# JanBeh/radiorust

Measured on NVIDIA B200. Metric: complex MS/s via FreqShift->Filter->Downsampler, higher is better.
Workload: dtype f32

## Files before the change

radiorust_b200/csrc/rr_chain.cu:

```cuda
#include <cuda_runtime.h>

#include <atomic>
#include <cmath>
#include <complex>
#include <algorithm>
#include <cstdio>
#include <cstdlib>
#include <cstring>
#include <deque>
#include <memory>
#include <mutex>
#include <numeric>
#include <string>
#include <unordered_map>
#include <vector>

#include "../../include/radiorust_b200.h"
#include "rr_design.h"
#include "rr_kernels.h"

namespace {

thread_local std::string g_err;
std::atomic<uint64_t> g_launches{0};

int fail(int code, const std::string& msg) {
    g_err = msg;
    return code;
}
int fail_cuda(cudaError_t e, const char* what) {
    g_err = std::string(what) + ": " + cudaGetErrorString(e);
    return RR_ERR_CUDA;
}
#define RR_CUDA(expr)                                     \
    do {                                                  \
        cudaError_t e__ = (expr);                         \
        if (e__ != cudaSuccess) return fail_cuda(e__, #expr); \
    } while (0)
#define RR_TRY(expr)              \
    do {                          \
        int r__ = (expr);         \
        if (r__ != RR_OK) return r__; \
    } while (0)
#define RR_LAUNCH(n_kernels, expr)                        \
    do {                                                  \
        cudaError_t e__ = (expr);                         \
        if (e__ != cudaSuccess) return fail_cuda(e__, #expr); \
        g_launches.fetch_add((n_kernels));                \
    } while (0)

struct DevBuf {
    void* p = nullptr;
    size_t bytes = 0;
    int ensure(size_t need, bool zero = false, cudaStream_t st = nullptr) {
        if (need <= bytes && p) {
            return RR_OK;
        }
        if (p) cudaFree(p);
        p = nullptr;
        bytes = 0;
        if (need == 0) need = 16;
        cudaError_t e = cudaMalloc(&p, need);
        if (e != cudaSuccess) {
            p = nullptr;
            g_err = std::string("cudaMalloc: ") + cudaGetErrorString(e);
            return e == cudaErrorMemoryAllocation ? RR_ERR_NOMEM : RR_ERR_CUDA;
        }
        bytes = need;
        if (zero) {
            e = cudaMemsetAsync(p, 0, need, st);
            if (e != cudaSuccess) return fail_cuda(e, "cudaMemsetAsync");
        }
        return RR_OK;
    }
    void release() {
        if (p) cudaFree(p);
        p = nullptr;
        bytes = 0;
    }
};

struct Shape {
    size_t chunk_len = 0, n_chunks = 0;
    double rate = 0.0;
    size_t len() const { return chunk_len * n_chunks; }
};

struct View {
    const void* p = nullptr;
    long long stride = 0;
    Shape sh;
};

struct NcoHost {
    int64_t numer = 0, denom = 1;
    uint64_t idx = 0;
    double start_phase = 0.0;
    bool has_table = false;
};

struct StageHost {
    double f_sr = NAN;
    size_t f_n = 0;
    int f_seg = 0;
    bool f_dirty = true;
    double r_in_rate = NAN;
    bool r_valid = false;
    int r_L = 0;
    long long P = 1, Q = 1, j0 = 0, m0 = 0;
    size_t r_pending = 0;
    bool r_indexed = false;
    double r_pos = 0.0;
    bool fm_has_prev = false;
    double n_sr = NAN;
    size_t rc_pending = 0;
    double rc_rate = NAN;
    size_t ov_hist = 0, ov_len = 0;
    double ov_rate = NAN;
};

struct StageAct {
    bool active = false;
    bool redesign = false;
    bool first_is_history = false;
    size_t n_new = 0;
    size_t pending_before = 0;
    long long j0 = 0, m0 = 0;
    double pos0 = 0.0;
    bool nco_recalc = false;
    int seg_before = 0;
    bool lost = false;
    Shape out;
};

inline long long floordiv128(long long a, long long b, long long c) { return (long long)(((__int128)a * b) / c); }
inline long long ceildiv128(long long a, long long b, long long c) { return (long long)(((__int128)a * b + (c - 1)) / c); }

bool integer_valued(double x) { return std::isfinite(x) && x >= 0.0 && x < 9.0e15 && std::floor(x) == x; }

}

struct rr_ctx {
    int device = 0;
    int sm_count = 0;
};


struct rr_pool {
    rr_ctx* ctx = nullptr;
    std::mutex mu;
    struct Buf {
        void* p;
        size_t cap;
    };
    std::deque<Buf> idle;
    std::unordered_map<void*, size_t> live;
    uint64_t n_alloc = 0, n_reuse = 0;
};

namespace {

struct Stage {
    rr_stage_desc d{};
    StageHost h;
    std::vector<double> shift;
    std::vector<uint8_t> shift_dirty;
    bool any_shift_dirty = true;
    std::vector<NcoHost> nco_h;
    std::vector<rr::NcoStream> nco_stage;
    DevBuf nco_d;
    DevBuf hperm, tw;
    DevBuf hist2[2];
    int hist_cur = 0;
    long long hist_fused_jlo = -1, hist_fused_jfirst = 0;
    DevBuf ztmp;
    size_t f_np = 0;
    DevBuf stg_in, stg_out, zero_chunk;
    DevBuf idx_a, idx_b;
    std::vector<std::complex<double>> taps;
    bool taps_valid = false;
    DevBuf big_h, big_twA, big_twB, big_twC, big_scratch;
    DevBuf ir, tail[2], obuf[2];
    int tail_cur = 0, obuf_cur = 0;
    std::vector<double> ir_host_flt;
    bool ztail_stale = false;
    DevBuf gtab, twK;
    bool poly_valid = false, poly_tried = false;
    int poly_K = 0, poly_G = 0, poly_Lmax = 0, poly_V = 0;
    DevBuf gtab2, twK2;
    bool poly2_tw_own = false;
    DevBuf acoef, gtab3, ubuf[2];
    long long ubuf_stride[2] = {-1, -1};
    int ubuf_cur = 0;
    bool ucache_valid = false;
    long long ucache_rows = 0;
    const void* ucache_ptr = nullptr;
    long long ucache_stride = 0;
    DevBuf ukeep[2];
    int ukeep_cur = 0;
    int fused_slot = -1;
    bool fused_valid = false;
    bool front_valid = false;
    int front_rank = 0;
    double front_discarded = 0.0;
    bool frontq_valid = false;
    bool frontq_wide = false;
    int frontq_cols = 0;
    int frontq_rank = 0;
    double frontq_discarded = 0.0;
    DevBuf acoef_q, gtab_q;
    bool poly2_valid = false;
    int poly2_G = 0, poly2_V = 0;
    size_t obuf_cap = 0;
    std::vector<double> ir_host;
    DevBuf fm_prev, fm_last;
    DevBuf fm_phase;
    size_t tail_cap = 0;
    DevBuf fwin, ftw;
    size_t fwin_n = 0;
    DevBuf out;
    size_t out_cap = 0;
};

}

struct rr_chain {
    rr_ctx* ctx = nullptr;
    int dtype = RR_C32;
    size_t esz = 8;
    int S = 1;
    std::vector<Stage> st;
    cudaStream_t stream = nullptr;
    cudaStream_t h2d_stream = nullptr, d2h_stream = nullptr;
    DevBuf stage_in[2], stage_out[2];
    cudaEvent_t ev_h2d[2] = {nullptr, nullptr}, ev_comp[2] = {nullptr, nullptr}, ev_d2h[2] = {nullptr, nullptr};
    cudaEvent_t ev_copy = nullptr;
    int slot = 0;
    std::string plan;
    uint64_t samples_lost = 0;
    bool push_mutated = false;
    bool allow_poly = true;
    bool allow_poly2 = true;
    size_t big_os_scratch_bytes = (size_t)2 << 30;
    bool allow_sab = true;
    bool allow_ucache = true;
    bool allow_front = true;
    bool allow_fused = true;
    int fused_min_streams = -1;
    long long fused_min_rows = 1;
    bool timing = false;
    std::vector<cudaEvent_t> evs;
    size_t ev_used = 0;
    std::vector<std::string> ev_names;
    std::string timed_kernel, breakdown;
    int timing_begin() {
        if (!timing) return 0;
        if (ev_used + 2 > evs.size()) {
            cudaEvent_t a = nullptr, b = nullptr;
            if (cudaEventCreate(&a) != cudaSuccess || cudaEventCreate(&b) != cudaSuccess) return 0;
            evs.push_back(a);
            evs.push_back(b);
        }
        cudaEventRecord(evs[ev_used], stream);
        return 1;
    }
    void timing_end(const char* name) {
        cudaEventRecord(evs[ev_used + 1], stream);
        ev_used += 2;
        if (ev_names.size() < ev_used / 2) ev_names.resize(ev_used / 2);
        ev_names[ev_used / 2 - 1] = name;
    }
};

namespace {
void chain_restart(rr_chain* c);
}

#define RR_TIMED_LAUNCH(c, name, n_kernels, expr)                        \
    do {                                                                 \
        const int t__ = (c)->timing_begin();                             \
        RR_LAUNCH(n_kernels, expr);                                      \
        if (t__) (c)->timing_end(name);                                  \
    } while (0)

namespace {

int advance_stage(const rr_stage_desc& d, StageHost& h, const Shape& in, StageAct* act) {
    StageAct a;
    a.out = in;
    if (in.n_chunks == 0 || in.chunk_len == 0) {
        a.out.n_chunks = 0;
        *act = a;
        return RR_OK;
    }
    a.active = true;
    switch (d.kind) {
        case RR_STAGE_FREQSHIFT:
            a.nco_recalc = !(h.n_sr == in.rate);
            h.n_sr = in.rate;
            break;
        case RR_STAGE_GAIN:
        case RR_STAGE_FOURIER:
        case RR_STAGE_FMMOD:
            break;
        case RR_STAGE_RECHUNK: {
            if (h.rc_pending > 0 && !(h.rc_rate == in.rate)) {
                h.rc_pending = 0;
                a.lost = true;
            }
            h.rc_rate = in.rate;
            const size_t ocl = (size_t)d.output_chunk_len;
            a.pending_before = h.rc_pending;
            a.n_new = in.len();
            const size_t total = h.rc_pending + a.n_new;
            a.out.chunk_len = ocl;
            a.out.n_chunks = total / ocl;
            h.rc_pending = total - a.out.n_chunks * ocl;
            break;
        }
        case RR_STAGE_OVERLAP: {
            const size_t k = (size_t)d.chunk_count;
            if (h.ov_hist > 0 && (h.ov_len != in.chunk_len || !(h.ov_rate == in.rate)))
                return fail(RR_ERR_UNSUPPORTED, "Overlapper: the chunks of one history must share length and sample rate");
            a.pending_before = h.ov_hist;
            const size_t tot = h.ov_hist + in.n_chunks;
            a.out.chunk_len = k * in.chunk_len;
            a.out.n_chunks = tot >= k ? tot - (k - 1) : 0;
            double acc = 0.0;
            for (size_t i = 0; i < k; ++i) acc += in.rate * (double)in.chunk_len;
            a.out.rate = acc / (double)(k * in.chunk_len);
            h.ov_hist = std::min(k - 1, tot);
            h.ov_len = in.chunk_len;
            h.ov_rate = in.rate;
            break;
        }
        case RR_STAGE_FMDEMOD:
            a.first_is_history = !h.fm_has_prev;
            h.fm_has_prev = true;
            break;
        case RR_STAGE_FILTER: {
            a.redesign = h.f_dirty || !(h.f_sr == in.rate) || h.f_n != in.chunk_len;
            if (a.redesign) {
                h.f_dirty = false;
                h.f_sr = in.rate;
                h.f_n = in.chunk_len;
                h.f_seg = 0;
            }
            a.seg_before = h.f_seg;
            a.first_is_history = (h.f_seg == 0);
            a.out.n_chunks = in.n_chunks - (a.first_is_history ? 1 : 0);
            h.f_seg = (int)std::min<size_t>(2, (size_t)h.f_seg + in.n_chunks);
            break;
        }
        case RR_STAGE_DOWNSAMPLE:
        case RR_STAGE_UPSAMPLE: {
            const bool down = d.kind == RR_STAGE_DOWNSAMPLE;
            if (!h.r_valid || !(h.r_in_rate == in.rate)) {
                const double in_rate = in.rate, out_rate = d.output_rate;
                if (!(in_rate >= 0.0)) return fail(RR_ERR_INVALID, "input sample rate must be positive");
                if (down && !(in_rate >= out_rate))
                    return fail(RR_ERR_INVALID, "input sample rate must be greater than or equal to output sample rate");
                if (!down && !(in_rate <= out_rate))
                    return fail(RR_ERR_INVALID, "input sample rate must be smaller than or equal to output sample rate");
                if (!down && !(d.bandwidth < in_rate))
                    return fail(RR_ERR_INVALID, "bandwidth must be smaller than input sample rate");
                const double margin = down ? (out_rate - d.bandwidth) / 2.0 : (in_rate - d.bandwidth) / 2.0;
                const double lf = std::ceil((down ? in_rate : out_rate) / margin * d.quality);
                if (!(lf > 0.0) || lf > 1.0e8) return fail(RR_ERR_INVALID, "resampler impulse response length out of range");
                if (in_rate == 0.0 || out_rate == 0.0) return fail(RR_ERR_INVALID, "resampler sample rates must be non-zero");
                h.r_indexed = !integer_valued(in_rate) || !integer_valued(out_rate);
                h.r_pos = 0.0;
                if (!h.r_indexed) {
                    long long Pn = (long long)in_rate, Qn = (long long)out_rate;
                    const long long g = std::gcd(Pn, Qn);
                    h.P = Pn / g;
                    h.Q = Qn / g;
                } else {
                    h.P = h.Q = 1;
                }
                h.j0 = 0;
                h.m0 = 0;
                h.r_L = (int)lf;
                h.r_in_rate = in_rate;
                h.r_valid = true;
                a.redesign = true;
            }
            const long long len = (long long)in.len();
            a.j0 = h.j0;
            a.m0 = h.m0;
            a.pos0 = h.r_pos;
            if (h.r_indexed) {
                const double in_rate = in.rate, out_rate = d.output_rate;
                double pos = h.r_pos;
                size_t cnt = 0;
                if (down) {
                    for (long long j = 0; j < len; ++j) {
                        pos += out_rate;
                        if (pos >= in_rate) {
                            pos -= in_rate;
                            ++cnt;
                        }
                    }
                } else {
                    for (long long p = 0; p < len; ++p) {
                        while (pos < out_rate) {
                            ++cnt;
                            pos += in_rate;
                        }
                        pos -= out_rate;
                    }
                }
                h.r_pos = pos;
                a.n_new = cnt;
            } else {
                long long total_after;
                if (down) total_after = floordiv128(h.j0 + len, h.Q, h.P);
                else total_after = ceildiv128(h.j0 + len, h.Q, h.P);
                a.n_new = (size_t)(total_after - h.m0);
                const long long j1 = (h.j0 + len) % h.P;
                h.j0 = j1;
                h.m0 = down ? floordiv128(j1, h.Q, h.P) : ceildiv128(j1, h.Q, h.P);
            }
            a.pending_before = h.r_pending;
            const size_t ocl = d.output_chunk_len ? (size_t)d.output_chunk_len : 1;
            const size_t total = h.r_pending + a.n_new;
            a.out.chunk_len = ocl;
            a.out.n_chunks = total / ocl;
            a.out.rate = d.output_rate;
            h.r_pending = total - a.out.n_chunks * ocl;
            break;
        }
        default:
            return fail(RR_ERR_INVALID, "unknown stage kind");
    }
    *act = a;
    return RR_OK;
}

int stage_event(const rr_stage_desc& d, StageHost& h, bool* interrupt) {
    int lost = 0;
    switch (d.kind) {
        case RR_STAGE_RECHUNK:
            if (h.rc_pending > 0) {
                h.rc_pending = 0;
                lost = 1;
                *interrupt = true;
            }
            break;
        case RR_STAGE_OVERLAP:
            h.ov_hist = 0;
            lost = 1;
            *interrupt = true;
            break;
        case RR_STAGE_FILTER:
            if (*interrupt) h.f_seg = 0;
            break;
        case RR_STAGE_FMDEMOD:
            if (*interrupt) h.fm_has_prev = false;
            break;
        default:
            break;
    }
    return lost;
}

inline size_t filter_padded_len(size_t n) {
    size_t np = 32;
    while (np < n) np <<= 1;
    return np;
}
template <typename T> bool filter_len_supported(size_t n) {
    if (n < 1 || n > ((size_t)1 << 23)) return false;
    const size_t np = filter_padded_len(n);
    return rr::chain_os_supported<T>((int)np, 0, 0) || rr::big_os_supported<T>((int)np);
}
inline bool is_pow2(size_t n) { return n >= 2 && (n & (n - 1)) == 0; }

int stage_supported(const rr_chain* c, const rr_stage_desc& d, const Shape& in) {
    if (in.n_chunks == 0 || in.chunk_len == 0) return RR_OK;
    const bool f32 = c->dtype == RR_C32;
    if (d.kind == RR_STAGE_FILTER) {
        const size_t n = in.chunk_len;
        if (!(f32 ? filter_len_supported<float>(n) : filter_len_supported<double>(n)))
            return fail(RR_ERR_UNSUPPORTED, "Filter: chunk length not supported by the device path");
    } else if (d.kind == RR_STAGE_FOURIER) {
        const int n = (int)std::min<size_t>(in.chunk_len, (size_t)1 << 30);
        const bool fft = f32 ? rr::fourier_fft_supported<float>(n) : rr::fourier_fft_supported<double>(n);
        if (!fft && in.chunk_len > (size_t)rr::kFourierDirectMax)
            return fail(RR_ERR_UNSUPPORTED, "Fourier: chunk lengths outside the FFT plans are limited to 4096 samples");
    }
    return RR_OK;
}

int dry_shape(const rr_chain* c, const Shape& in, Shape* out) {
    std::vector<StageHost> hs;
    hs.reserve(c->st.size());
    for (const auto& s : c->st) hs.push_back(s.h);
    Shape sh = in;
    for (size_t i = 0; i < hs.size(); ++i) {
        StageAct a;
        RR_TRY(stage_supported(c, c->st[i].d, sh));
        RR_TRY(advance_stage(c->st[i].d, hs[i], sh, &a));
        if (a.lost) {
            bool intr = true;
            for (size_t j = i + 1; j < hs.size(); ++j) stage_event(c->st[j].d, hs[j], &intr);
        }
        sh = a.out;
    }
    *out = sh;
    return RR_OK;
}

template <typename T> struct TypeTag { using type = T; };
#define RR_DISPATCH(chain, T, ...)                     \
    do {                                               \
        if ((chain)->dtype == RR_C32) {                \
            using T = float;                           \
            __VA_ARGS__;                               \
        } else {                                       \
            using T = double;                          \
            __VA_ARGS__;                               \
        }                                              \
    } while (0)

rr::WindowFn make_window(int kind, double beta, rr_window_fn fn, void* user) {
    switch (kind) {
        case RR_WINDOW_RECTANGULAR:
            return [](double) { return 1.0; };
        case RR_WINDOW_CUSTOM:
            return [fn, user](double x) { return fn ? fn(user, x) : 1.0; };
        default:
            return [beta](double x) { return rr::kaiser_rel_with_beta(beta, x); };
    }
}

template <typename T> int upload_complex(DevBuf& buf, const std::vector<std::complex<double>>& v, cudaStream_t st) {
    RR_TRY(buf.ensure(v.size() * 2 * sizeof(T)));
    std::vector<T> tmp(v.size() * 2);
    for (size_t i = 0; i < v.size(); ++i) {
        tmp[2 * i] = (T)v[i].real();
        tmp[2 * i + 1] = (T)v[i].imag();
    }
    RR_CUDA(cudaMemcpyAsync(buf.p, tmp.data(), tmp.size() * sizeof(T), cudaMemcpyHostToDevice, st));
    RR_CUDA(cudaStreamSynchronize(st));
    return RR_OK;
}
template <typename T> int upload_real(DevBuf& buf, const std::vector<double>& v, cudaStream_t st) {
    RR_TRY(buf.ensure(v.size() * sizeof(T)));
    std::vector<T> tmp(v.size());
    for (size_t i = 0; i < v.size(); ++i) tmp[i] = (T)v[i];
    RR_CUDA(cudaMemcpyAsync(buf.p, tmp.data(), tmp.size() * sizeof(T), cudaMemcpyHostToDevice, st));
    RR_CUDA(cudaStreamSynchronize(st));
// ... 421 lines not shown
    const size_t tab_bytes = (size_t)(Q * P) * (size_t)bestK * 2 * sizeof(T);
    if (tab_bytes > ((size_t)512 << 20)) return RR_OK;
    const double e8 = (double)P / (8.0 * (double)((P + 7) / 8)), e10 = (double)P / (10.0 * (double)((P + 9) / 10));
    int G = e10 > e8 + 1e-9 ? 10 : 8;
    if (const char* e = std::getenv("RR_POLY_G")) G = std::atoi(e) == 8 ? 8 : 10;
    if (!rr::poly_supported<T>(bestK, (int)Q, G)) return RR_OK;
    if (rr::poly_smem_bytes<T>(bestK, (int)Q, G, 1) > (size_t)220 * 1024) return RR_OK;
    std::vector<std::complex<double>> tab, perm;
    const int lm = rr::design_poly_tables(f.taps, ds.ir_host_flt, P, Q, bestK, &tab);
    if (lm != (int)Lmax) return fail(RR_ERR_INVALID, "internal: polyphase reach mismatch");
    const double scale = 2.0 * (double)n / (double)bestK;
    const long long NR = (P + G - 1) / G;
    perm.assign((size_t)(Q * NR) * (size_t)bestK * (size_t)G, std::complex<double>(0.0, 0.0));
    for (long long q = 0; q < Q; ++q)
        for (long long p = 0; p < P; ++p) {
            const long long r = p / G, gg = p % G;
            for (int k = 0; k < bestK; ++k) {
                const size_t pos = (size_t)rr::poly_hperm_index<T>(bestK, k);
                perm[(((size_t)(q * NR + r)) * bestK + pos) * G + gg] = tab[(size_t)(q * P + p) * bestK + k] * scale;
            }
        }
    RR_TRY(upload_complex<T>(ds.gtab, perm, c->stream));
    std::vector<std::complex<double>> tw;
    rr::make_twiddles((size_t)bestK, &tw);
    RR_TRY(upload_complex<T>(ds.twK, tw, c->stream));
    ds.poly_K = bestK;
    ds.poly_G = G;
    ds.poly_Lmax = (int)Lmax;
    ds.poly_V = (int)(bestK - 1 - Lmax);
    ds.poly_valid = true;

    if (std::is_same<T, float>::value && Q > 1 && c->allow_front && P > 2 * kFrontQRank && rr::poly_supported<T>(bestK, (int)Q, 8) &&
        Lmax + 2 <= bestK) {
        constexpr int RMAX = 2 * kFrontQRank;
        std::vector<double> acf;
        std::vector<std::complex<double>> bq;
        int rank = 0;
        double disc = 0.0;
        const int lmq = rr::design_rank_tables_q(f.taps, ds.ir_host_flt, P, Q, bestK, 2.0e-8, RMAX, &rank, &acf, &bq, &disc);
        const int cols = rank <= kFrontQRank ? kFrontQRank : RMAX;
        const bool narrow = cols == kFrontQRank && rr::front_supported(kFrontQRank, P);
        if (rank > 0 && lmq == (int)Lmax && (narrow || rr::front_wide_supported(cols, P))) {
            std::vector<float> ac((size_t)P * cols);
            for (long long p = 0; p < P; ++p)
                for (int cc = 0; cc < cols; ++cc) ac[(size_t)p * cols + cc] = (float)acf[(size_t)p * RMAX + cc];
            RR_TRY(ds.acoef_q.ensure(ac.size() * sizeof(float)));
            RR_CUDA(cudaMemcpyAsync(ds.acoef_q.p, ac.data(), ac.size() * sizeof(float), cudaMemcpyHostToDevice, c->stream));
            RR_CUDA(cudaStreamSynchronize(c->stream));
            constexpr int GQ = 8;
            const long long NRq = cols / GQ;
            perm.assign((size_t)(Q * NRq) * (size_t)bestK * (size_t)GQ, std::complex<double>(0.0, 0.0));
            for (long long q = 0; q < Q; ++q)
                for (int cc = 0; cc < cols; ++cc) {
                    const long long r = cc / GQ, gg = cc % GQ;
                    for (int k = 0; k < bestK; ++k) {
                        const size_t pos = (size_t)rr::poly_hperm_index<T>(bestK, k);
                        perm[(((size_t)(q * NRq + r)) * bestK + pos) * GQ + gg] = bq[((size_t)q * RMAX + cc) * bestK + k] * scale;
                    }
                }
            RR_TRY(upload_complex<T>(ds.gtab_q, perm, c->stream));
            ds.frontq_rank = rank;
            ds.frontq_cols = cols;
            ds.frontq_wide = !narrow;
            ds.frontq_discarded = disc;
            ds.frontq_valid = true;
        }
    }

    if (std::is_same<T, float>::value && c->allow_poly2 && rr::poly2_supported(512, P, Q) && 511 - Lmax >= 128) {
        const int K2 = 512, G2 = rr::poly2_pick_G(P);
        if (bestK != K2) rr::design_poly_tables(f.taps, ds.ir_host_flt, P, Q, K2, &tab);
        const double scale2 = 2.0 * (double)n / (double)K2;
        const long long NR2 = (P + G2 - 1) / G2;
        perm.assign((size_t)NR2 * (size_t)K2 * (size_t)G2, std::complex<double>(0.0, 0.0));
        for (long long p = 0; p < P; ++p)
            for (int k = 0; k < K2; ++k)
                perm[(size_t)rr::poly2_table_index(G2, (int)(p / G2), (int)(p % G2), k)] = tab[(size_t)p * K2 + k] * scale2;
        RR_TRY(upload_complex<T>(ds.gtab2, perm, c->stream));
        if (bestK != K2) {
            rr::make_twiddles((size_t)K2, &tw);
            RR_TRY(upload_complex<T>(ds.twK2, tw, c->stream));
        }
        ds.poly2_tw_own = bestK != K2;
        ds.poly2_G = G2;
        ds.poly2_V = (int)(K2 - 1 - Lmax);
        ds.poly2_valid = true;

        constexpr int RK = 10;
        if (c->allow_front && rr::front_supported(RK, P) && rr::poly2_supported(K2, RK, 1)) {
            std::vector<double> acf;
            std::vector<std::complex<double>> bfft;
            int rank = 0;
            double disc = 0.0;
            const int lm2 = rr::design_rank_tables(f.taps, ds.ir_host_flt, P, K2, 2.0e-8, RK, &rank, &acf, &bfft, &disc);
            if (rank > 0 && lm2 == (int)Lmax) {
                std::vector<float> ac((size_t)P * RK);
                for (long long p = 0; p < P; ++p)
                    for (int cc = 0; cc < RK; ++cc) ac[(size_t)(((p / 2) * 2 + (p & 1)) * RK + cc)] = (float)acf[(size_t)p * RK + cc];
                RR_TRY(ds.acoef.ensure(ac.size() * sizeof(float)));
                RR_CUDA(cudaMemcpyAsync(ds.acoef.p, ac.data(), ac.size() * sizeof(float), cudaMemcpyHostToDevice, c->stream));
                RR_CUDA(cudaStreamSynchronize(c->stream));
                perm.assign((size_t)K2 * (size_t)RK, std::complex<double>(0.0, 0.0));
                for (int cc = 0; cc < RK; ++cc)
                    for (int k = 0; k < K2; ++k) perm[(size_t)rr::poly2_table_index(RK, 0, cc, k)] = bfft[(size_t)cc * K2 + k] * scale2;
                RR_TRY(upload_complex<T>(ds.gtab3, perm, c->stream));
                ds.front_rank = rank;
                ds.front_discarded = disc;
                ds.front_valid = true;
                if (c->allow_fused && rr::fused_supported(RK, P, (int)Lmax)) {
                    const int slot = fused_slot_acquire(c->ctx->device, &ds);
                    if (slot >= 0) {
                        RR_CUDA(rr::fused_upload_coef(slot, ac.data(), (int)P, c->stream));
                        RR_CUDA(cudaStreamSynchronize(c->stream));
                        ds.fused_slot = slot;
                        ds.fused_valid = true;
                    }
                }
            }
        }
    }
    return RR_OK;
}

template <typename T>
int downsample_indexed(rr_chain* c, Stage& ds, const StageAct& a, const void* in, long long in_stride, long long len, void* out,
                       long long out_stride) {
    const double in_rate = ds.h.r_in_rate, out_rate = ds.d.output_rate;
    std::vector<int> fire;
    fire.reserve(a.n_new);
    double pos = a.pos0;
    for (long long j = 0; j < len; ++j) {
        pos += out_rate;
        if (pos >= in_rate) {
            pos -= in_rate;
            fire.push_back((int)j);
        }
    }
    if (fire.size() != a.n_new) return fail(RR_ERR_INVALID, "internal: indexed downsampler count mismatch");
    RR_TRY(ds.idx_a.ensure(std::max<size_t>(fire.size(), 1) * sizeof(int)));
    if (!fire.empty()) RR_CUDA(cudaMemcpyAsync(ds.idx_a.p, fire.data(), fire.size() * sizeof(int), cudaMemcpyHostToDevice, c->stream));
    RR_CUDA(cudaStreamSynchronize(c->stream));
    RR_LAUNCH(2, rr::launch_downsample_indexed<T>(in, in_stride, len, ds.tail[ds.tail_cur].p, ds.tail[ds.tail_cur ^ 1].p, (const T*)ds.ir.p,
                                                  ds.h.r_L, (const int*)ds.idx_a.p, (long long)fire.size(), out, out_stride, c->S, c->stream));
    ds.tail_cur ^= 1;
    return RR_OK;
}
template <typename T>
int upsample_indexed(rr_chain* c, Stage& us, const StageAct& a, const void* in, long long in_stride, long long len, void* out,
                     long long out_stride) {
    const double in_rate = us.h.r_in_rate, out_rate = us.d.output_rate;
    const int L = us.h.r_L;
    std::vector<int> qpos((size_t)len);
    double pos = a.pos0;
    long long q = 0;
    for (long long p = 0; p < len; ++p) {
        qpos[(size_t)p] = (int)q;
        while (pos < out_rate) {
            ++q;
            pos += in_rate;
        }
        pos -= out_rate;
    }
    if ((size_t)q != a.n_new) return fail(RR_ERR_INVALID, "internal: indexed upsampler count mismatch");
    std::vector<int> cnt((size_t)q + (size_t)L);
    {
        size_t p = 0;
        for (size_t i = 0; i < cnt.size(); ++i) {
            while (p < qpos.size() && (size_t)qpos[p] <= i) ++p;
            cnt[i] = (int)p;
        }
    }
    RR_TRY(us.idx_a.ensure(std::max<size_t>(qpos.size(), 1) * sizeof(int)));
    RR_TRY(us.idx_b.ensure(std::max<size_t>(cnt.size(), 1) * sizeof(int)));
    if (!qpos.empty()) RR_CUDA(cudaMemcpyAsync(us.idx_a.p, qpos.data(), qpos.size() * sizeof(int), cudaMemcpyHostToDevice, c->stream));
    if (!cnt.empty()) RR_CUDA(cudaMemcpyAsync(us.idx_b.p, cnt.data(), cnt.size() * sizeof(int), cudaMemcpyHostToDevice, c->stream));
    RR_CUDA(cudaStreamSynchronize(c->stream));
    RR_LAUNCH(1, rr::launch_upsample_indexed<T>(in, in_stride, len, us.tail[us.tail_cur].p, us.tail[us.tail_cur ^ 1].p, (const T*)us.ir.p, L,
                                                (const int*)us.idx_a.p, (const int*)us.idx_b.p, q, out, out_stride, c->S, c->stream));
    us.tail_cur ^= 1;
    return RR_OK;
}

struct DirectOut {
    void* user_out = nullptr;
    long long user_stride = 0;
    bool done = false;
};
template <typename T>
int run_filter_down(rr_chain* c, Stage& f, Stage& ds, const FilterIo& io, const StageAct& fa, const StageAct& da, std::string* plan,
                    DirectOut* direct = nullptr) {
    const size_t n = io.n;
    const int S = c->S;
    cudaStream_t st = c->stream;
    const int L = ds.h.r_L;
    void* obase = (char*)ds.obuf[ds.obuf_cur].p + da.pending_before * 2 * sizeof(T);
    const long long ostride = (long long)ds.obuf_cap;

    const bool rational = !ds.h.r_indexed && is_pow2(n);
    if (c->allow_poly && rational) RR_TRY(poly_prepare<T>(c, f, ds));
    const bool was_ucache_valid = ds.ucache_valid;
    ds.ucache_valid = false;
    size_t ca = io.n_chunks;
    if (c->allow_poly && rational && ds.poly_valid) {
        const size_t need = (size_t)(2 - std::min(2, fa.seg_before));
        ca = std::min(need, io.n_chunks);
    }
    const size_t fih = fa.first_is_history ? 1 : 0;

    long long j0 = da.j0, m0 = da.m0;
    if (ca > fih) {
        const long long zlen = (long long)((ca - fih) * n);
        if (ds.h.r_indexed) {
            RR_TRY(f.ztmp.ensure((size_t)S * (size_t)zlen * 2 * sizeof(T)));
            RR_TRY(run_os<T>(c, f, io, ca, fih != 0, f.ztmp.p, zlen));
            RR_TRY(downsample_indexed<T>(c, ds, da, f.ztmp.p, zlen, zlen, obase, ostride));
            *plan += "os|downsample(indexed)";
            return RR_OK;
        }
        const long long tot = floordiv128(j0 + zlen, ds.h.Q, ds.h.P);
        const long long n_out = tot - m0;
        if (rational && rr::chain_os_supported<T>((int)n, 1, L)) {
            rr::ChainOsArgs<T> a{};
            a.in = io.in;
            a.in_stride = io.in_stride;
            a.n_chunks = (int)ca;
            a.first_is_history = (int)fih;
            a.emit = 1;
            a.hist_in = (const char*)f.hist2[f.hist_cur].p + n * 2 * sizeof(T);
            a.hist_stride = (long long)(2 * n);
            a.hist_out = nullptr;
            a.hperm = f.hperm.p;
            a.twN = f.tw.p;
            a.nco = io.nco ? (const rr::NcoStream*)io.nco->nco_d.p : nullptr;
            a.nco_offset = 0;
            a.out = obase;
            a.out_stride = ostride;
            a.ir = (const T*)ds.ir.p;
            a.L = L;
            a.ztail_in = ds.tail[ds.tail_cur].p;
            a.ztail_out = ds.tail[ds.tail_cur ^ 1].p;
            a.rate.P = ds.h.P;
            a.rate.Q = ds.h.Q;
            a.rate.j0 = j0;
            a.rate.m0 = m0;
            RR_TIMED_LAUNCH(c, "k_chain_os<epi=down>", 1, rr::launch_chain_os<T>((int)n, 1, S, 1, a, st));
            ds.tail_cur ^= 1;
            *plan += "fused_os[filter+down]";
        } else {
            RR_TRY(f.ztmp.ensure((size_t)S * (size_t)zlen * 2 * sizeof(T)));
            RR_TRY(run_os<T>(c, f, io, ca, fih != 0, f.ztmp.p, zlen));
            rr::RateState rs;
            rs.P = ds.h.P;
            rs.Q = ds.h.Q;
            rs.j0 = j0;
            rs.m0 = m0;
            RR_LAUNCH(2, rr::launch_downsample<T>(f.ztmp.p, zlen, zlen, ds.tail[ds.tail_cur].p, ds.tail[ds.tail_cur ^ 1].p, (const T*)ds.ir.p,
                                                  L, rs, n_out, obase, ostride, S, st));
            ds.tail_cur ^= 1;
            *plan += !is_pow2(n) ? "padded_os[filter]|downsample" : (rr::chain_os_supported<T>((int)n, 0, 0) ? "fused_os[filter]|downsample" : "big_os|downsample");
        }
        obase = (char*)obase + (size_t)n_out * 2 * sizeof(T);
        j0 = (j0 + zlen) % ds.h.P;
        m0 = floordiv128(j0, ds.h.Q, ds.h.P);
    }

    if (ca < io.n_chunks) {
        const long long Pq = ds.h.P, Qq = ds.h.Q;
        const long long zlen = (long long)((io.n_chunks - ca) * n);
        const long long m_lo = m0 + 1;
        const long long m_hi = floordiv128(j0 + zlen, Qq, Pq);
        bool used_poly2 = false, used_front = false, used_fused = false, used_frontq = false;
        if (m_hi >= m_lo) {
            rr::PolyArgs<T> a{};
            a.in = io.in;
            a.in_stride = io.in_stride;
            a.len = (long long)(io.n_chunks * n);
            a.n = (long long)n;
            a.nco = io.nco ? (const rr::NcoStream*)io.nco->nco_d.p : nullptr;
            a.gtab = ds.gtab.p;
            a.twK = ds.twK.p;
            a.P = Pq;
            a.Q = Qq;
            a.Lmax = ds.poly_Lmax;
            a.V = ds.poly_V;
            a.J0 = j0 - (long long)(ca * n);
            a.m0 = m0;
            a.m_lo = m_lo;
            a.m_hi = m_hi;
            a.I_lo = m_lo / Qq;
            const long long I_hi = m_hi / Qq;
            bool done = false;
            if constexpr (std::is_same<T, float>::value) {
                const bool tma_ok = ((uintptr_t)a.in % 16 == 0) && (S == 1 || a.in_stride % 2 == 0) && a.len < (1LL << 31);
                if (ds.poly2_valid && ds.front_valid && ds.fused_valid && c->allow_fused && tma_ok && ca == 0 && was_ucache_valid &&
                    c->allow_ucache && ds.ucache_ptr && Qq == 1 && m0 == 0 && a.J0 >= 0 && a.J0 < Pq && S >= c->fused_min_streams &&
                    m_hi - m_lo + 1 >= c->fused_min_rows && a.len >= 33 * Pq) {
                    constexpr int RK = 10;
                    const long long n_out = m_hi - m_lo + 1;
                    const long long Lh = ds.poly_Lmax;
                    const size_t kbytes = (size_t)S * (size_t)Lh * RK * 2 * sizeof(float);
                    DevBuf& kb = ds.ukeep[ds.ukeep_cur];
                    RR_TRY(kb.ensure(kbytes));
                    rr::FusedArgs fu{};
                    fu.in = a.in;
                    fu.in_stride = a.in_stride;
                    fu.len = a.len;
                    fu.hist2 = f.hist2[f.hist_cur].p;
                    fu.n = a.n;
                    fu.nco = a.nco;
                    fu.P = (int)Pq;
                    fu.coef_slot = ds.fused_slot;
                    fu.J0 = a.J0;
                    fu.n_out = (int)n_out;
                    fu.Lmax = (int)Lh;
                    fu.V = ds.poly2_V;
                    fu.ukeep_in = ds.ucache_ptr;
                    fu.ukeep_in_stride = ds.ucache_stride;
                    fu.ukeep_out = kb.p;
                    fu.ukeep_out_stride = Lh * RK;
                    fu.gtab = ds.gtab3.p;
                    fu.twK = ds.poly2_tw_own ? ds.twK2.p : ds.twK.p;
                    fu.out = obase;
                    fu.out_stride = ostride;
                    const long long emit = (long long)da.out.len();
                    if (direct && direct->user_out && emit >= (long long)da.pending_before && emit > 0) {
                        fu.out = (char*)direct->user_out + da.pending_before * 2 * sizeof(T);
                        fu.out_stride = direct->user_stride;
                        fu.out2 = ds.obuf[ds.obuf_cur ^ 1].p;
                        fu.out2_stride = ostride;
                        fu.out_split = emit - (long long)da.pending_before;
                        direct->done = true;
                    }
                    const long long cover_hi = m_hi * Pq - a.J0;
                    f.hist_fused_jlo = -1;
                    f.hist_fused_jfirst = 0;
                    const long long hfrom = a.len - 2 * a.n, hstart = std::max<long long>(hfrom, 0);
                    if (cover_hi > hstart) {
                        fu.hist_out = f.hist2[f.hist_cur ^ 1].p;
                        fu.hist_from = hfrom;
                        fu.hist_stride = 2 * a.n;
                        f.hist_fused_jlo = cover_hi - hfrom;
                        f.hist_fused_jfirst = hstart - hfrom;
                    }
                    RR_TIMED_LAUNCH(c, "k_fused", 1, rr::launch_fused(S, fu, c->ctx->sm_count, st));
                    ds.ucache_valid = true;
                    ds.ucache_rows = n_out + Lh;
                    ds.ucache_ptr = kb.p;
                    ds.ucache_stride = Lh * RK;
                    ds.ukeep_cur ^= 1;
                    done = true;
                    used_fused = true;
                }
                if (!done && ds.poly2_valid && ds.front_valid && tma_ok) {
                    constexpr int RK = 10;
                    const int G2 = RK;
                    const long long n_out = m_hi - m_lo + 1;
                    const long long n_rows = n_out + ds.poly_Lmax;
                    const long long pad_rows = 512;
                    const long long u_stride = (((n_rows + 127) / 128 * 128 + pad_rows) * RK + 1) / 2 * 2;
                    if (n_rows < (1LL << 27)) {
                        const int n_blocks1 = (int)((n_out - 1) / ds.poly2_V + 1);
                        const int halves_total = 2 * c->ctx->sm_count;
                        const int sab_run = (c->allow_sab && n_blocks1 <= 3 && S > halves_total) ? (S + halves_total - 1) / halves_total : 0;
                        const int sab_nb = sab_run * n_blocks1;
                        const size_t S_alloc = sab_run ? (size_t)((S + sab_run - 1) / sab_run) * sab_run : (size_t)S;
                        const size_t ubytes = S_alloc * (size_t)u_stride * 2 * sizeof(float);
                        DevBuf& ub = ds.ubuf[ds.ubuf_cur];
                        if (ub.bytes < ubytes || ds.ubuf_stride[ds.ubuf_cur] != u_stride) {
                            RR_TRY(ub.ensure(ubytes));
                            RR_CUDA(cudaMemsetAsync(ub.p, 0, ubytes, st));
                            ds.ubuf_stride[ds.ubuf_cur] = u_stride;
                        }
                        const long long Lh = ds.poly_Lmax;
                        const bool cached = was_ucache_valid && c->allow_ucache && ca == 0 && ds.ucache_rows >= Lh && n_out > 0;
                        rr::FrontArgs fa{};
                        if (cached) {
                            fa.kept_src = ds.ucache_ptr;
                            fa.kept_stride = ds.ucache_stride;
                            fa.kept_rows = (int)Lh;
                        }
                        fa.in = a.in;
                        fa.in_stride = a.in_stride;
                        fa.len = a.len;
                        fa.hist2 = f.hist2[f.hist_cur].p;
                        fa.n = a.n;
                        fa.nco = a.nco;
                        fa.acoef = (const float*)ds.acoef.p;
                        fa.P = (int)Pq;
                        fa.J0 = a.J0;
                        fa.row_first = m_lo - 1 - (cached ? 0 : Lh);
                        fa.n_rows = (int)(cached ? n_out : n_rows);
                        fa.u = (char*)ub.p + (cached ? (size_t)Lh * RK * 2 * sizeof(float) : 0);
                        fa.u_stride = u_stride;
                        const long long cover_lo = fa.row_first * Pq - a.J0, cover_hi = m_hi * Pq - a.J0;
                        f.hist_fused_jlo = -1;
                        f.hist_fused_jfirst = 0;
                        const long long hfrom = a.len - 2 * a.n, hstart = std::max<long long>(hfrom, 0);
                        if (cover_lo <= hstart && cover_hi > hstart) {
                            fa.hist_out = f.hist2[f.hist_cur ^ 1].p;
                            fa.hist_from = hfrom;
                            fa.hist_stride = 2 * a.n;
                            fa.hist_staged = a.len < 4 * a.n ? 1 : 0;
                            f.hist_fused_jlo = cover_hi - hfrom;
                            f.hist_fused_jfirst = hstart - hfrom;
                        }
                        RR_TIMED_LAUNCH(c, "k_front", 1, rr::launch_front(RK, S, fa, st));
                        rr::PolyArgs<float> b{};
                        b.in = ub.p;
                        b.in_stride = u_stride;
                        b.len = (n_rows + pad_rows) * RK;
                        b.hist2 = ub.p;
                        b.n = 0;
                        b.nco = nullptr;
                        b.gtab = ds.gtab3.p;
                        b.twK = ds.poly2_tw_own ? ds.twK2.p : ds.twK.p;
                        b.P = RK;
                        b.Q = 1;
                        b.Lmax = ds.poly_Lmax;
                        b.V = ds.poly2_V;
                        b.J0 = 0;
                        b.m0 = ds.poly_Lmax;
                        b.m_lo = ds.poly_Lmax + 1;
                        b.m_hi = ds.poly_Lmax + n_out;
                        b.I_lo = b.m_lo;
                        b.n_blocks = (int)((b.m_hi - b.I_lo) / b.V + 1);
                        int nbpc = std::min(G2, b.n_blocks);
                        while (nbpc > 1 && rr::poly2_smem_bytes(G2, nbpc) > (size_t)226 * 1024) --nbpc;
                        const long long ctas_y = (S + 1) / 2;
                        while (nbpc > 1 && ctas_y * ((b.n_blocks + nbpc - 1) / nbpc) < 2LL * c->ctx->sm_count) --nbpc;
                        const int ngroups = (b.n_blocks + nbpc - 1) / nbpc;
                        nbpc = (b.n_blocks + ngroups - 1) / ngroups;
                        int ngrp = ngroups;
                        while (ngrp > 1 && ctas_y * ((ngroups + ngrp - 1) / ngrp) < 2LL * c->ctx->sm_count) --ngrp;
                        b.nbpc = nbpc;
                        b.ngrp = ngrp;
                        b.out = obase;
                        b.out_stride = ostride;
                        int S2 = S;
                        if (sab_nb) {
                            int nb2 = std::min(G2, sab_nb);
                            while (nb2 > 1 && rr::poly2_smem_bytes(G2, nb2) > (size_t)226 * 1024) --nb2;
                            const int groups2 = (sab_nb + nb2 - 1) / nb2;
                            b.n_blocks = sab_nb;
                            b.nbpc = (sab_nb + groups2 - 1) / groups2;
                            b.ngrp = groups2;
                            b.sab_blocks = sab_nb;
                            b.sab_rb = n_blocks1;
                            b.sab_streams = S;
                            b.sab_in_step = u_stride;
                            b.in_stride = (long long)sab_run * u_stride;
                            b.len = (long long)sab_run * u_stride;
                            S2 = (S + sab_run - 1) / sab_run;
                        }
                        const long long emit = (long long)da.out.len();
                        if (direct && direct->user_out && ca == 0 && emit >= (long long)da.pending_before && emit > 0) {
                            b.out = (char*)direct->user_out + da.pending_before * 2 * sizeof(T);
                            b.out_stride = direct->user_stride;
                            b.out2 = ds.obuf[ds.obuf_cur ^ 1].p;
                            b.out2_stride = ostride;
                            b.out_split = emit - (long long)da.pending_before;
                            direct->done = true;
                        }
                        if (sab_nb) {
                            b.sab_out_step = b.out_stride;
                            b.sab_out2_step = b.out2_stride;
                            b.out_stride *= sab_run;
                            b.out2_stride *= sab_run;
                        }
                        RR_TIMED_LAUNCH(c, "k_poly2", 1, rr::launch_poly2(G2, S2, b, st));
                        ds.ucache_valid = true;
                        ds.ucache_rows = n_rows;
                        ds.ucache_ptr = (const char*)ub.p + (size_t)(n_rows - Lh) * RK * 2 * sizeof(float);
                        ds.ucache_stride = u_stride;
                        ds.ubuf_cur ^= 1;
                        done = true;
                        used_front = true;
                    }
                }
                if (!done && ds.frontq_valid && (tma_ok || ds.frontq_wide) && Qq > 1) {
                    const int RQ = ds.frontq_cols;
                    constexpr int GQ = 8;
                    const long long Lh = ds.poly_Lmax;
                    const long long I_first = a.I_lo, I_last = I_hi;
                    const long long row_first = I_first - 1 - Lh;
                    const long long n_rows = I_last - I_first + 2 + Lh;
                    const long long u_stride = n_rows * RQ;
                    if (n_rows * Pq < (1LL << 31)) {
                        DevBuf& ub = ds.ubuf[0];
                        RR_TRY(ub.ensure((size_t)S * (size_t)u_stride * 2 * sizeof(float)));
                        ds.ubuf_stride[0] = -1;
                        rr::FrontArgs fa{};
                        fa.in = a.in;
                        fa.in_stride = a.in_stride;
                        fa.len = a.len;
                        fa.hist2 = f.hist2[f.hist_cur].p;
                        fa.n = a.n;
                        fa.nco = a.nco;
                        fa.acoef = (const float*)ds.acoef_q.p;
                        fa.P = (int)Pq;
                        fa.J0 = a.J0;
                        fa.row_first = row_first;
                        fa.n_rows = (int)n_rows;
                        fa.u = ub.p;
                        fa.u_stride = u_stride;
                        const long long cover_lo = row_first * Pq - a.J0, cover_hi = std::min<long long>((I_last + 1) * Pq - a.J0, a.len);
                        f.hist_fused_jlo = -1;
                        f.hist_fused_jfirst = 0;
                        const long long hfrom = a.len - 2 * a.n, hstart = std::max<long long>(hfrom, 0);
                        if (cover_lo <= hstart && cover_hi > hstart) {
                            fa.hist_out = f.hist2[f.hist_cur ^ 1].p;
                            fa.hist_from = hfrom;
                            fa.hist_stride = 2 * a.n;
                            fa.hist_staged = a.len < 4 * a.n ? 1 : 0;
                            f.hist_fused_jlo = cover_hi - hfrom;
                            f.hist_fused_jfirst = hstart - hfrom;
                        }
                        if (ds.frontq_wide) RR_TIMED_LAUNCH(c, "k_front_wide", 1, rr::launch_front_wide(RQ, S, fa, st));
                        else RR_TIMED_LAUNCH(c, "k_front", 1, rr::launch_front(RQ, S, fa, st));
                        rr::PolyArgs<float> b{};
                        b.in = ub.p;
                        b.in_stride = u_stride;
                        b.len = n_rows * RQ;
                        b.hist2 = ub.p;
                        b.n = 0;
                        b.nco = nullptr;
                        b.gtab = ds.gtab_q.p;
                        b.twK = ds.twK.p;
                        b.P = RQ;
                        b.Q = Qq;
                        b.Lmax = (int)Lh;
                        b.V = ds.poly_V;
                        b.J0 = row_first * RQ;
                        b.m0 = a.m0;
                        b.m_lo = a.m_lo;
                        b.m_hi = a.m_hi;
                        b.I_lo = I_first;
                        b.n_blocks = (int)((I_last - I_first) / b.V + 1);
                        int nbpc = b.n_blocks;
                        while (nbpc > 1 && rr::poly_smem_bytes<float>(ds.poly_K, (int)Qq, GQ, nbpc) > (size_t)200 * 1024) --nbpc;
                        while (nbpc > 1 && (long long)S * ((b.n_blocks + nbpc - 1) / nbpc) < 2LL * c->ctx->sm_count) --nbpc;
                        const int nsb = (b.n_blocks + nbpc - 1) / nbpc;
                        b.nbpc = (b.n_blocks + nsb - 1) / nsb;
                        b.out = obase;
                        b.out_stride = ostride;
                        RR_TIMED_LAUNCH(c, "k_poly(u)", 1, rr::launch_poly<float>(ds.poly_K, (int)Qq, GQ, S, b, st));
                        done = true;
                        used_frontq = true;
                    }
                }
                if (!done && ds.poly2_valid && tma_ok) {
                    a.gtab = ds.gtab2.p;
                    if (ds.poly2_tw_own) a.twK = ds.twK2.p;
                    a.V = ds.poly2_V;
                    a.n_blocks = (int)((I_hi - a.I_lo) / a.V + 1);
                    const int G2 = ds.poly2_G;
                    int nbpc = std::min(G2, a.n_blocks);
                    while (nbpc > 1 && rr::poly2_smem_bytes(G2, nbpc) > (size_t)226 * 1024) --nbpc;
                    const long long ctas_y = (S + 1) / 2;
                    while (nbpc > 1 && ctas_y * ((a.n_blocks + nbpc - 1) / nbpc) < 2LL * c->ctx->sm_count) --nbpc;
                    const int ngroups = (a.n_blocks + nbpc - 1) / nbpc;
                    nbpc = (a.n_blocks + ngroups - 1) / ngroups;
                    int ngrp = ngroups;
                    while (ngrp > 1 && ctas_y * ((ngroups + ngrp - 1) / ngrp) < 2LL * c->ctx->sm_count) --ngrp;
                    a.nbpc = nbpc;
                    a.ngrp = ngrp;
                    a.out = obase;
                    a.out_stride = ostride;
                    a.hist2 = f.hist2[f.hist_cur].p;
                    RR_TIMED_LAUNCH(c, "k_poly2", 1, rr::launch_poly2(G2, S, a, st));
                    done = true;
                    used_poly2 = true;
                }
            }
            if (!done) {
                a.n_blocks = (int)((I_hi - a.I_lo) / a.V + 1);
                int nbpc = std::max(1, ds.poly_G / (int)Qq);
                while (nbpc > 1 && rr::poly_smem_bytes<T>(ds.poly_K, (int)Qq, ds.poly_G, nbpc) > (size_t)200 * 1024) --nbpc;
                while (nbpc > 1 && (long long)S * ((a.n_blocks + nbpc - 1) / nbpc) < 2LL * c->ctx->sm_count) --nbpc;
                const int nsb = (a.n_blocks + nbpc - 1) / nbpc;
                nbpc = (a.n_blocks + nsb - 1) / nsb;
                a.nbpc = nbpc;
                a.out = obase;
                a.out_stride = ostride;
                a.hist2 = f.hist2[f.hist_cur].p;
                RR_TIMED_LAUNCH(c, "k_poly", 1, rr::launch_poly<T>(ds.poly_K, (int)Qq, ds.poly_G, S, a, st));
            }
        }
        ds.ztail_stale = true;
        if (!plan->empty() && plan->back() != '+' && plan->back() != '|' && ca > 0) *plan += "|";
        *plan += used_frontq ? "front+poly[filter+down]" : used_fused ? "fused[filter+down]" : (used_front ? "front+poly2[filter+down]" : (used_poly2 ? "poly2[filter+down]" : "poly[filter+down]"));
    }
    return RR_OK;
}

template <typename T>
int run_push(rr_chain* c, double sample_rate, size_t chunk_len, size_t n_chunks, const void* dev_in, size_t in_stride, void* dev_out,
             size_t out_capacity, size_t out_stride, size_t* out_count, double* out_rate) {
    const int S = c->S;
    const int ns = (int)c->st.size();
    cudaStream_t st = c->stream;
    Shape in;
    in.chunk_len = chunk_len;
    in.n_chunks = n_chunks;
    in.rate = sample_rate;
    if (chunk_len * n_chunks > in_stride && S > 1) return fail(RR_ERR_INVALID, "in_stride smaller than the pushed samples");

    {
        Shape sh;
        RR_TRY(dry_shape(c, in, &sh));
        if (sh.len() > out_capacity) return fail(RR_ERR_CAPACITY, "output buffer too small for this push");
        if (sh.len() > out_stride && S > 1) return fail(RR_ERR_INVALID, "out_stride smaller than the produced samples");
    }

    c->push_mutated = true;
    std::string plan;
    View cur;
    cur.p = dev_in;
    cur.stride = (long long)in_stride;
    cur.sh = in;
    Stage* pending_nco = nullptr;

    for (int i = 0; i < ns; ++i) {
        Stage& s = c->st[i];
        const bool last = (i == ns - 1);
        if (s.d.kind == RR_STAGE_FILTER && !last && c->st[i + 1].d.kind == RR_STAGE_DOWNSAMPLE && c->st[i + 1].ztail_stale &&
            cur.sh.n_chunks > 0) {
            StageHost probe = s.h;
            StageAct pa;
            RR_TRY(advance_stage(s.d, probe, cur.sh, &pa));
            StageHost dprobe = c->st[i + 1].h;
            StageAct dpa;
            int r = advance_stage(c->st[i + 1].d, dprobe, pa.out, &dpa);
            const bool ds_redesign = (r == RR_OK) && dpa.redesign;
            if (ds_redesign) c->st[i + 1].ztail_stale = false;
            else if (pa.redesign || pa.first_is_history || !c->allow_poly) RR_TRY(regen_ztail<T>(c, s, c->st[i + 1]));
        }
        StageAct a;
        RR_TRY(advance_stage(s.d, s.h, cur.sh, &a));
        if (a.lost) {
            ++c->samples_lost;
            bool intr = true;
            for (int j = i + 1; j < ns; ++j) c->samples_lost += (uint64_t)stage_event(c->st[j].d, c->st[j].h, &intr);
        }
        if (!a.active) {
            cur.sh = a.out;
            continue;
        }
// ... 445 lines not shown
    RR_CUDA(e);
    return RR_OK;
}
int rr_device_free(rr_ctx* ctx, void* p) {
    if (!ctx) return fail(RR_ERR_INVALID, "rr_device_free: null context");
    RR_CUDA(cudaSetDevice(ctx->device));
    if (p) RR_CUDA(cudaFree(p));
    return RR_OK;
}
int rr_ipc_export(rr_ctx* ctx, void* dev_ptr, void* handle_out_64_bytes) {
    if (!ctx || !dev_ptr || !handle_out_64_bytes) return fail(RR_ERR_INVALID, "rr_ipc_export: null argument");
    static_assert(sizeof(cudaIpcMemHandle_t) == 64, "the header promises a 64-byte handle");
    RR_CUDA(cudaSetDevice(ctx->device));
    cudaIpcMemHandle_t h;
    RR_CUDA(cudaIpcGetMemHandle(&h, dev_ptr));
    std::memcpy(handle_out_64_bytes, &h, sizeof h);
    return RR_OK;
}
int rr_ipc_open(rr_ctx* ctx, const void* handle_64_bytes, void** dev_ptr) {
    if (!ctx || !handle_64_bytes || !dev_ptr) return fail(RR_ERR_INVALID, "rr_ipc_open: null argument");
    *dev_ptr = nullptr;
    RR_CUDA(cudaSetDevice(ctx->device));
    cudaIpcMemHandle_t h;
    std::memcpy(&h, handle_64_bytes, sizeof h);
    RR_CUDA(cudaIpcOpenMemHandle(dev_ptr, h, cudaIpcMemLazyEnablePeerAccess));
    return RR_OK;
}
int rr_ipc_close(rr_ctx* ctx, void* dev_ptr) {
    if (!ctx) return fail(RR_ERR_INVALID, "rr_ipc_close: null context");
    RR_CUDA(cudaSetDevice(ctx->device));
    if (dev_ptr) RR_CUDA(cudaIpcCloseMemHandle(dev_ptr));
    return RR_OK;
}
int rr_memcpy_h2d(rr_ctx* ctx, void* dst_dev, const void* src_host, size_t bytes) {
    if (!ctx) return fail(RR_ERR_INVALID, "rr_memcpy_h2d: null context");
    RR_CUDA(cudaSetDevice(ctx->device));
    RR_CUDA(cudaDeviceSynchronize());
    RR_CUDA(cudaMemcpy(dst_dev, src_host, bytes, cudaMemcpyHostToDevice));
    return RR_OK;
}
int rr_memcpy_d2h(rr_ctx* ctx, void* dst_host, const void* src_dev, size_t bytes) {
    if (!ctx) return fail(RR_ERR_INVALID, "rr_memcpy_d2h: null context");
    RR_CUDA(cudaSetDevice(ctx->device));
    RR_CUDA(cudaDeviceSynchronize());
    RR_CUDA(cudaMemcpy(dst_host, src_dev, bytes, cudaMemcpyDeviceToHost));
    return RR_OK;
}

int rr_metering_level(rr_ctx* ctx, int32_t dtype, const void* dev_in, size_t in_stride, size_t chunk_len, size_t n_chunks, int n_streams,
                      double* host_out) {
    if (!ctx || !host_out || (!dev_in && n_chunks)) return fail(RR_ERR_INVALID, "rr_metering_level: null argument");
    if (dtype != RR_C32 && dtype != RR_C64) return fail(RR_ERR_INVALID, "rr_metering_level: bad dtype");
    if (n_streams < 1 || chunk_len == 0) return fail(RR_ERR_INVALID, "rr_metering_level: empty chunk (the reference divides by zero)");
    if (n_streams > 65535) return fail(RR_ERR_INVALID, "rr_metering_level: at most 65535 streams per call");
    if (n_chunks == 0) return RR_OK;
    RR_CUDA(cudaSetDevice(ctx->device));
    (void)cudaGetLastError();
    RR_CUDA(cudaDeviceSynchronize());
    DevBuf out;
    RR_TRY(out.ensure(sizeof(double) * n_chunks * (size_t)n_streams));
    cudaError_t e = dtype == RR_C32 ? rr::launch_level<float>(dev_in, (long long)in_stride, (long long)chunk_len, (long long)n_chunks, n_streams,
                                                              (double*)out.p, nullptr)
                                    : rr::launch_level<double>(dev_in, (long long)in_stride, (long long)chunk_len, (long long)n_chunks, n_streams,
                                                               (double*)out.p, nullptr);
    if (e == cudaSuccess) {
        g_launches.fetch_add(1);
        e = cudaMemcpy(host_out, out.p, sizeof(double) * n_chunks * (size_t)n_streams, cudaMemcpyDeviceToHost);
    }
    out.release();
    if (e != cudaSuccess) return fail_cuda(e, "rr_metering_level");
    return RR_OK;
}

int rr_metering_bandwidth(rr_ctx* ctx, int32_t dtype, const void* dev_bins, size_t in_stride, size_t chunk_len, size_t n_chunks,
                          int n_streams, double double_percentile, double sample_rate, double* host_out) {
    if (!ctx || !host_out || (!dev_bins && n_chunks)) return fail(RR_ERR_INVALID, "rr_metering_bandwidth: null argument");
    if (dtype != RR_C32 && dtype != RR_C64) return fail(RR_ERR_INVALID, "rr_metering_bandwidth: bad dtype");
    if (n_streams < 1 || n_streams > 65535 || chunk_len == 0) return fail(RR_ERR_INVALID, "rr_metering_bandwidth: empty chunk or bad stream count");
    if (n_chunks == 0) return RR_OK;
    RR_CUDA(cudaSetDevice(ctx->device));
    (void)cudaGetLastError();
    RR_CUDA(cudaDeviceSynchronize());
    DevBuf out;
    RR_TRY(out.ensure(sizeof(double) * n_chunks * (size_t)n_streams));
    cudaError_t e = dtype == RR_C32 ? rr::launch_bandwidth<float>(dev_bins, (long long)in_stride, (long long)chunk_len, (long long)n_chunks, n_streams,
                                                                  double_percentile, sample_rate, (double*)out.p, nullptr)
                                    : rr::launch_bandwidth<double>(dev_bins, (long long)in_stride, (long long)chunk_len, (long long)n_chunks, n_streams,
                                                                   double_percentile, sample_rate, (double*)out.p, nullptr);
    if (e == cudaSuccess) {
        g_launches.fetch_add(1);
        e = cudaMemcpy(host_out, out.p, sizeof(double) * n_chunks * (size_t)n_streams, cudaMemcpyDeviceToHost);
    }
    out.release();
    if (e != cudaSuccess) return fail_cuda(e, "rr_metering_bandwidth");
    return RR_OK;
}

int rr_metering_rescale_energy(rr_ctx* ctx, int32_t dtype, const void* dev_bins, size_t in_stride, size_t chunk_len, size_t n_chunks,
                               int n_streams, size_t resolution, void* host_out) {
    if (!ctx || !host_out || (!dev_bins && n_chunks)) return fail(RR_ERR_INVALID, "rr_metering_rescale_energy: null argument");
    if (dtype != RR_C32 && dtype != RR_C64) return fail(RR_ERR_INVALID, "rr_metering_rescale_energy: bad dtype");
    if (chunk_len == 0) return fail(RR_ERR_INVALID, "rr_metering_rescale_energy: empty input (metering.rs:98 asserts n > 0)");
    if (n_streams < 1 || n_streams > 65535 || n_chunks > 65535) return fail(RR_ERR_INVALID, "rr_metering_rescale_energy: at most 65535 streams and chunks per call");
    if (n_chunks == 0 || resolution == 0) return RR_OK;
    RR_CUDA(cudaSetDevice(ctx->device));
    (void)cudaGetLastError();
    RR_CUDA(cudaDeviceSynchronize());
    const size_t fsz = dtype == RR_C32 ? sizeof(float) : sizeof(double);
    const size_t bytes = fsz * n_chunks * (size_t)n_streams * resolution;
    DevBuf out;
    RR_TRY(out.ensure(bytes));
    cudaError_t e = dtype == RR_C32 ? rr::launch_rescale_energy<float>(dev_bins, (long long)in_stride, (long long)chunk_len, (long long)n_chunks,
                                                                       n_streams, (long long)resolution, out.p, nullptr)
                                    : rr::launch_rescale_energy<double>(dev_bins, (long long)in_stride, (long long)chunk_len, (long long)n_chunks,
                                                                        n_streams, (long long)resolution, out.p, nullptr);
    if (e == cudaSuccess) {
        g_launches.fetch_add(1);
        e = cudaMemcpy(host_out, out.p, bytes, cudaMemcpyDeviceToHost);
    }
    out.release();
    if (e != cudaSuccess) return fail_cuda(e, "rr_metering_rescale_energy");
    return RR_OK;
}

double rr_bessel_i0(double x) { return rr::bessel_i0(x); }
double rr_sinc(double x) { return rr::sinc(x); }
double rr_kaiser_rel_with_beta(double beta, double x) { return rr::kaiser_rel_with_beta(beta, x); }
double rr_kaiser_null_at_bin_to_beta(double n) { return rr::kaiser_null_at_bin_to_beta(n); }
void rr_deemphasis_factor(double tau, double frequency, double* out_re, double* out_im) {
    const std::complex<double> v = rr::deemphasis_factor(tau, frequency);
    if (out_re) *out_re = v.real();
    if (out_im) *out_im = v.imag();
}
int rr_freq_to_ratio(double sample_rate, double precision, double frequency, int64_t* numer, int64_t* denom) {
    int64_t n = 0, d = 1;
    if (!rr::freq_to_ratio(sample_rate, precision, frequency, &n, &d))
        return fail(RR_ERR_INVALID, "denominator == 0 (Ratio::new panics in the reference)");
    if (numer) *numer = n;
    if (denom) *denom = d;
    return RR_OK;
}
int rr_design_filter_response(rr_freq_resp_fn f, void* f_user, int32_t window_kind, double window_beta, rr_window_fn w, void* w_user,
                              double sample_rate, size_t n, int32_t dtype, double* out_2n_complex) {
    if (!f || !out_2n_complex) return fail(RR_ERR_INVALID, "rr_design_filter_response: null argument");
    rr::FreqResp fr = [f, f_user](int64_t bin, double freq) {
        double re = 0.0, im = 0.0;
        f(f_user, bin, freq, &re, &im);
        return std::complex<double>(re, im);
    };
    std::vector<std::complex<double>> H;
    if (!rr::design_filter_response(fr, make_window(window_kind, window_beta, w, w_user), sample_rate, n, dtype == RR_C32, &H))
        return fail(RR_ERR_INVALID, "rr_design_filter_response: n must be >= 1");
    for (size_t i = 0; i < H.size(); ++i) {
        out_2n_complex[2 * i] = H[i].real();
        out_2n_complex[2 * i + 1] = H[i].imag();
    }
    return RR_OK;
}
static int design_taps(bool down, double input_rate, double output_rate, double bandwidth, double quality, size_t* ir_len, double* ir) {
    if (!ir_len) return fail(RR_ERR_INVALID, "ir_len is null");
    if (!(output_rate >= 0.0) || !(bandwidth >= 0.0) || !(input_rate >= 0.0)) return fail(RR_ERR_INVALID, "rates must be positive");
    if (down && !(bandwidth < output_rate)) return fail(RR_ERR_INVALID, "bandwidth must be smaller than output sample rate");
    if (down && !(input_rate >= output_rate)) return fail(RR_ERR_INVALID, "input sample rate must be >= output sample rate");
    if (!down && !(input_rate <= output_rate)) return fail(RR_ERR_INVALID, "input sample rate must be <= output sample rate");
    if (!down && !(bandwidth < input_rate)) return fail(RR_ERR_INVALID, "bandwidth must be smaller than input sample rate");
    const double margin = down ? (output_rate - bandwidth) / 2.0 : (input_rate - bandwidth) / 2.0;
    const double lf = std::ceil((down ? input_rate : output_rate) / margin * quality);
    if (!(lf > 0.0) || lf > 1.0e8) return fail(RR_ERR_INVALID, "impulse response length out of range");
    const size_t L = (size_t)lf;
    const size_t cap = *ir_len;
    *ir_len = L;
    if (!ir) return RR_OK;
    if (cap < L) return fail(RR_ERR_CAPACITY, "ir buffer too small");
    std::vector<double> taps;
    const double ratio = down ? output_rate / input_rate : input_rate / output_rate;
    const double null_bin = (double)L * margin / (down ? input_rate : output_rate);
    rr::design_resampler_taps(L, ratio, null_bin, &taps);
    std::memcpy(ir, taps.data(), L * sizeof(double));
    return RR_OK;
}
int rr_design_downsampler_taps(double input_rate, double output_rate, double bandwidth, double quality, size_t* ir_len, double* ir) {
    return design_taps(true, input_rate, output_rate, bandwidth, quality, ir_len, ir);
}
int rr_design_upsampler_taps(double input_rate, double output_rate, double bandwidth, double quality, size_t* ir_len, double* ir) {
    return design_taps(false, input_rate, output_rate, bandwidth, quality, ir_len, ir);
}

int rr_design_fused_rank(rr_freq_resp_fn f, void* f_user, int32_t window_kind, double window_beta, rr_window_fn w, void* w_user,
                         double sample_rate, size_t n, double output_rate, double bandwidth, double quality, double tol, int max_rank,
                         int* rank, double* discarded, double* table_error) {
    if (!f || !rank) return fail(RR_ERR_INVALID, "rr_design_fused_rank: null argument");
    if (max_rank < 1 || max_rank > 64) return fail(RR_ERR_INVALID, "rr_design_fused_rank: max_rank out of range");
    rr::FreqResp fr = [f, f_user](int64_t bin, double freq) {
        double re = 0.0, im = 0.0;
        f(f_user, bin, freq, &re, &im);
        return std::complex<double>(re, im);
    };
    std::vector<std::complex<double>> resp, taps;
    if (!is_pow2(n)) return fail(RR_ERR_INVALID, "rr_design_fused_rank: the fused kernels run on power-of-two chunk lengths >= 2");
    if (!rr::design_filter_response(fr, make_window(window_kind, window_beta, w, w_user), sample_rate, n, true, &resp, &taps))
        return fail(RR_ERR_INVALID, "rr_design_fused_rank: filter design failed");
    if (!integer_valued(sample_rate) || !integer_valued(output_rate) || output_rate <= 0.0 || sample_rate < output_rate)
        return fail(RR_ERR_INVALID, "rr_design_fused_rank: rates must be integer valued, input >= output > 0");
    const long long g = std::gcd((long long)sample_rate, (long long)output_rate);
    const long long P = (long long)sample_rate / g, Q = (long long)output_rate / g;
    if (Q < 1 || Q > 4) return fail(RR_ERR_UNSUPPORTED, "rr_design_fused_rank: in/out = P/Q with Q <= 4 only");
    size_t L = 0;
    RR_TRY(design_taps(true, sample_rate, output_rate, bandwidth, quality, &L, nullptr));
    std::vector<double> ir(L);
    RR_TRY(design_taps(true, sample_rate, output_rate, bandwidth, quality, &L, ir.data()));
    for (auto& v : ir) v = (double)(float)v;
    const int K = 512;
    std::vector<double> a;
    std::vector<std::complex<double>> b, full;
    double disc = 0.0;
    const int lmax = Q == 1 ? rr::design_rank_tables(taps, ir, P, K, tol, max_rank, rank, &a, &b, &disc)
                            : rr::design_rank_tables_q(taps, ir, P, Q, K, tol, max_rank, rank, &a, &b, &disc);
    if (discarded) *discarded = disc;
    if (table_error) {
        *table_error = -1.0;
        if (*rank > 0 && lmax + 2 <= K) {
            rr::design_poly_tables(taps, ir, P, Q, K, &full);
            double num = 0.0, den = 0.0;
            for (long long q = 0; q < Q; ++q)
                for (long long p = 0; p < P; ++p)
                    for (int k = 0; k < K; ++k) {
                        std::complex<double> sum(0.0, 0.0);
                        for (int c = 0; c < *rank; ++c) sum += a[(size_t)p * max_rank + c] * b[((size_t)q * max_rank + c) * K + k];
                        const std::complex<double> want = full[(size_t)(q * P + p) * K + k];
                        num += std::norm(sum - want);
                        den += std::norm(want);
                    }
            *table_error = den > 0.0 ? std::sqrt(num / den) : 0.0;
        }
    }
    return RR_OK;
}

int rr_chain_create(rr_ctx* ctx, const rr_chain_desc* desc, rr_chain** out) {
    if (!ctx || !desc || !out) return fail(RR_ERR_INVALID, "rr_chain_create: null argument");
    *out = nullptr;
    if (desc->dtype != RR_C32 && desc->dtype != RR_C64) return fail(RR_ERR_INVALID, "rr_chain_create: bad dtype");
    if (desc->n_streams < 1) return fail(RR_ERR_INVALID, "rr_chain_create: n_streams must be >= 1");
    if (desc->n_streams > 65535) return fail(RR_ERR_INVALID, "rr_chain_create: at most 65535 streams per chain (streams map to a grid dimension)");
    if (desc->n_stages < 0 || (desc->n_stages > 0 && !desc->stages)) return fail(RR_ERR_INVALID, "rr_chain_create: bad stage list");
    for (int i = 0; i < desc->n_stages; ++i) {
        const rr_stage_desc& d = desc->stages[i];
        switch (d.kind) {
            case RR_STAGE_FREQSHIFT:
                if (!(d.precision > 0.0)) return fail(RR_ERR_INVALID, "FreqShifter: precision must be positive");
                break;
            case RR_STAGE_FILTER:
                if (!d.freq_resp) return fail(RR_ERR_INVALID, "Filter: freq_resp callback is null");
                break;
            case RR_STAGE_DOWNSAMPLE:
                if (!(d.output_rate >= 0.0)) return fail(RR_ERR_INVALID, "output sample rate must be positive");
                if (!(d.bandwidth >= 0.0)) return fail(RR_ERR_INVALID, "bandwidth must be positive");
                if (!(d.bandwidth < d.output_rate)) return fail(RR_ERR_INVALID, "bandwidth must be smaller than output sample rate");
                if (!(d.quality >= 1.0)) return fail(RR_ERR_INVALID, "quality must be >= 1.0");
                break;
            case RR_STAGE_UPSAMPLE:
                if (!(d.output_rate >= 0.0)) return fail(RR_ERR_INVALID, "output sample rate must be positive");
                if (!(d.bandwidth >= 0.0)) return fail(RR_ERR_INVALID, "bandwidth must be positive");
                if (!(d.quality >= 1.0)) return fail(RR_ERR_INVALID, "quality must be >= 1.0");
                break;
            case RR_STAGE_FMDEMOD:
            case RR_STAGE_FMMOD:
            case RR_STAGE_GAIN:
            case RR_STAGE_FOURIER:
                break;
            case RR_STAGE_RECHUNK:
                if (d.output_chunk_len == 0) return fail(RR_ERR_INVALID, "chunk length must be positive");
                break;
            case RR_STAGE_OVERLAP:
                if (d.chunk_count <= 0) return fail(RR_ERR_INVALID, "chunk count must be positive");
                break;
            default:
                return fail(RR_ERR_INVALID, "rr_chain_create: unknown stage kind");
        }
    }
    RR_CUDA(cudaSetDevice(ctx->device));
    std::unique_ptr<rr_chain> c(new rr_chain());
    c->ctx = ctx;
    c->dtype = desc->dtype;
    c->esz = desc->dtype == RR_C32 ? 8 : 16;
    c->S = desc->n_streams;
    c->st.resize((size_t)desc->n_stages);
    for (int i = 0; i < desc->n_stages; ++i) {
        Stage& s = c->st[(size_t)i];
        s.d = desc->stages[i];
        if (s.d.kind == RR_STAGE_FREQSHIFT) {
            s.shift.assign((size_t)c->S, s.d.shift);
            s.shift_dirty.assign((size_t)c->S, 1);
            s.any_shift_dirty = true;
        }
    }
    if (const char* e = std::getenv("RR_DISABLE_POLY")) c->allow_poly = !(e[0] == '1');
    if (const char* e = std::getenv("RR_DISABLE_POLY2")) c->allow_poly2 = !(e[0] == '1');
    if (const char* e = std::getenv("RR_DISABLE_FRONT")) c->allow_front = !(e[0] == '1');
    if (const char* e = std::getenv("RR_DISABLE_FUSED")) c->allow_fused = !(e[0] == '1');
    c->fused_min_streams = 2 * ctx->sm_count;
    if (const char* e = std::getenv("RR_FUSED_MIN_STREAMS")) c->fused_min_streams = std::max(1, std::atoi(e));
    if (const char* e = std::getenv("RR_FUSED_MIN_ROWS")) c->fused_min_rows = std::max(1, std::atoi(e));
    if (const char* e = std::getenv("RR_DISABLE_UCACHE")) c->allow_ucache = !(e[0] == '1');
    if (const char* e = std::getenv("RR_DISABLE_SAB")) c->allow_sab = !(e[0] == '1');
    if (const char* e = std::getenv("RR_BIG_OS_SCRATCH_MB")) c->big_os_scratch_bytes = (size_t)std::max(1, std::atoi(e)) << 20;
    RR_CUDA(cudaStreamCreateWithFlags(&c->stream, cudaStreamNonBlocking));
    *out = c.release();
    return RR_OK;
}

int rr_chain_destroy(rr_chain* c) {
    if (!c) return RR_OK;
    cudaSetDevice(c->ctx->device);
    if (c->stream) cudaStreamSynchronize(c->stream);
    for (auto& s : c->st) {
        DevBuf* bufs[] = {&s.nco_d, &s.hperm, &s.tw, &s.hist2[0], &s.hist2[1], &s.ztmp, &s.gtab, &s.twK, &s.big_h, &s.big_twA, &s.big_twB, &s.big_twC, &s.big_scratch,
                          &s.ir, &s.tail[0], &s.tail[1], &s.obuf[0], &s.obuf[1], &s.fm_prev, &s.fm_last, &s.out,
                          &s.gtab2, &s.twK2, &s.acoef, &s.gtab3, &s.acoef_q, &s.gtab_q, &s.ubuf[0], &s.ubuf[1], &s.fwin, &s.ftw, &s.fm_phase, &s.ukeep[0], &s.ukeep[1],
                          &s.stg_in, &s.stg_out, &s.zero_chunk, &s.idx_a, &s.idx_b};
        for (DevBuf* b : bufs) b->release();
        if (s.fused_slot >= 0) fused_slot_release(c->ctx->device, &s);
    }
    if (c->d2h_stream) cudaStreamSynchronize(c->d2h_stream);
    if (c->h2d_stream) cudaStreamSynchronize(c->h2d_stream);
    for (int k = 0; k < 2; ++k) {
        c->stage_in[k].release();
        c->stage_out[k].release();
        if (c->ev_h2d[k]) cudaEventDestroy(c->ev_h2d[k]);
        if (c->ev_comp[k]) cudaEventDestroy(c->ev_comp[k]);
        if (c->ev_d2h[k]) cudaEventDestroy(c->ev_d2h[k]);
    }
    for (cudaEvent_t e : c->evs) cudaEventDestroy(e);
    if (c->ev_copy) cudaEventDestroy(c->ev_copy);
    if (c->h2d_stream) cudaStreamDestroy(c->h2d_stream);
    if (c->d2h_stream) cudaStreamDestroy(c->d2h_stream);
    if (c->stream) cudaStreamDestroy(c->stream);
    delete c;
    return RR_OK;
}

static int stage_of(rr_chain* c, int stage, int kind, Stage** out) {
    if (!c) return fail(RR_ERR_INVALID, "null chain");
    if (stage < 0 || stage >= (int)c->st.size()) return fail(RR_ERR_INVALID, "stage index out of range");
    if (c->st[(size_t)stage].d.kind != kind) return fail(RR_ERR_INVALID, "stage is of a different kind");
    *out = &c->st[(size_t)stage];
    return RR_OK;
}

int rr_chain_set_shift(rr_chain* c, int stage, int stream, double shift_hz) {
    Stage* s = nullptr;
    RR_TRY(stage_of(c, stage, RR_STAGE_FREQSHIFT, &s));
    if (stream >= c->S) return fail(RR_ERR_INVALID, "stream index out of range");
    if (stream < 0) {
        for (int i = 0; i < c->S; ++i) {
            s->shift[(size_t)i] = shift_hz;
            s->shift_dirty[(size_t)i] = 1;
        }
    } else {
        s->shift[(size_t)stream] = shift_hz;
        s->shift_dirty[(size_t)stream] = 1;
    }
    s->any_shift_dirty = true;
    return RR_OK;
}
int rr_chain_set_shifts(rr_chain* c, int stage, const double* shifts_hz, int n) {
    Stage* s = nullptr;
    RR_TRY(stage_of(c, stage, RR_STAGE_FREQSHIFT, &s));
    if (!shifts_hz || n != c->S) return fail(RR_ERR_INVALID, "rr_chain_set_shifts: need one shift per stream");
    for (int i = 0; i < n; ++i) {
        s->shift[(size_t)i] = shifts_hz[i];
        s->shift_dirty[(size_t)i] = 1;
    }
    s->any_shift_dirty = true;
    return RR_OK;
}
int rr_chain_get_shift(rr_chain* c, int stage, int stream, double* shift_hz) {
    Stage* s = nullptr;
    RR_TRY(stage_of(c, stage, RR_STAGE_FREQSHIFT, &s));
    if (stream < 0 || stream >= c->S || !shift_hz) return fail(RR_ERR_INVALID, "bad stream index");
    *shift_hz = s->shift[(size_t)stream];
    return RR_OK;
}

int rr_chain_update_filter(rr_chain* c, int stage, rr_freq_resp_fn f, void* f_user, int32_t window_kind, double window_beta,
                           rr_window_fn w, void* w_user, int keep_window) {
    Stage* s = nullptr;
    RR_TRY(stage_of(c, stage, RR_STAGE_FILTER, &s));
    if (!f) return fail(RR_ERR_INVALID, "rr_chain_update_filter: freq_resp is null");
    s->d.freq_resp = f;
    s->d.freq_resp_user = f_user;
    if (!keep_window) {
        s->d.window_kind = window_kind;
        s->d.window_beta = window_beta;
        s->d.window_fn = w;
        s->d.window_user = w_user;
    }
    s->h.f_dirty = true;
    return RR_OK;
}
int rr_chain_set_deviation(rr_chain* c, int stage, double deviation) {
    Stage* s = nullptr;
    if (c && stage >= 0 && stage < (int)c->st.size() && c->st[(size_t)stage].d.kind == RR_STAGE_FMMOD) RR_TRY(stage_of(c, stage, RR_STAGE_FMMOD, &s));
    else RR_TRY(stage_of(c, stage, RR_STAGE_FMDEMOD, &s));
    s->d.deviation = deviation;
    return RR_OK;
}
int rr_chain_set_output_chunk_len(rr_chain* c, int stage, size_t output_chunk_len) {
    Stage* s = nullptr;
    RR_TRY(stage_of(c, stage, RR_STAGE_RECHUNK, &s));
    if (output_chunk_len == 0) return fail(RR_ERR_INVALID, "chunk length must be positive");
    s->d.output_chunk_len = output_chunk_len;
    return RR_OK;
}
int rr_chain_set_gain(rr_chain* c, int stage, double gain) {
    Stage* s = nullptr;
    RR_TRY(stage_of(c, stage, RR_STAGE_GAIN, &s));
    s->d.gain = gain;
    return RR_OK;
}

int rr_chain_event(rr_chain* c, int is_interrupt) {
    if (!c) return fail(RR_ERR_INVALID, "null chain");
    bool intr = is_interrupt != 0;
    for (auto& s : c->st) {
        c->samples_lost += (uint64_t)stage_event(s.d, s.h, &intr);
        if (intr) s.ucache_valid = false;
    }
    return RR_OK;
}
uint64_t rr_chain_samples_lost_count(rr_chain* c) { return c ? c->samples_lost : 0; }

size_t rr_chain_max_output(rr_chain* c, double sample_rate, size_t chunk_len, size_t n_chunks) {
    if (!c) return 0;
    Shape sh;
    sh.chunk_len = chunk_len;
    sh.n_chunks = n_chunks;
    sh.rate = sample_rate;
    Shape out;
    if (dry_shape(c, sh, &out) != RR_OK) return 0;
    return out.len();
}

int rr_chain_push_device(rr_chain* c, double sample_rate, size_t chunk_len, size_t n_chunks, const void* dev_in, size_t in_stride,
                         void* dev_out, size_t out_capacity, size_t out_stride, size_t* out_count, double* out_sample_rate) {
    if (!c) return fail(RR_ERR_INVALID, "null chain");
    if (out_count) *out_count = 0;
    if (n_chunks == 0 || chunk_len == 0) return RR_OK;
    if (!dev_in) return fail(RR_ERR_INVALID, "rr_chain_push_device: dev_in is null");
    if (chunk_len > (size_t)1 << 30 || n_chunks > (size_t)1 << 30) return fail(RR_ERR_INVALID, "push too large");
    RR_CUDA(cudaSetDevice(c->ctx->device));
    (void)cudaGetLastError();
    c->push_mutated = false;
    int r;
    if (c->dtype == RR_C32)
        r = run_push<float>(c, sample_rate, chunk_len, n_chunks, dev_in, in_stride, dev_out, out_capacity, out_stride, out_count,
                            out_sample_rate);
    else
        r = run_push<double>(c, sample_rate, chunk_len, n_chunks, dev_in, in_stride, dev_out, out_capacity, out_stride, out_count,
                             out_sample_rate);
    if (r != RR_OK && c->push_mutated) {
        const std::string msg = g_err;
        chain_restart(c);
        g_err = msg + " (the chain's streaming state was reset)";
        if (out_count) *out_count = 0;
    }
    c->push_mutated = false;
    return r;
}

int rr_chain_push(rr_chain* c, double sample_rate, size_t chunk_len, size_t n_chunks, const void* host_in, size_t in_stride,
                  void* host_out, size_t out_capacity, size_t out_stride, size_t* out_count, double* out_sample_rate) {
    if (!c) return fail(RR_ERR_INVALID, "null chain");
    if (out_count) *out_count = 0;
    if (n_chunks == 0 || chunk_len == 0) return RR_OK;
    if (!host_in) return fail(RR_ERR_INVALID, "rr_chain_push: host_in is null");
    RR_CUDA(cudaSetDevice(c->ctx->device));
    const size_t len = chunk_len * n_chunks;
    const size_t S = (size_t)c->S;
    if (S > 1 && in_stride < len) return fail(RR_ERR_INVALID, "in_stride smaller than the pushed samples");
    Shape sh_in, sh_out;
    sh_in.chunk_len = chunk_len;
    sh_in.n_chunks = n_chunks;
    sh_in.rate = sample_rate;
    RR_TRY(dry_shape(c, sh_in, &sh_out));
    const size_t max_out = sh_out.len();
    if (max_out > out_capacity) return fail(RR_ERR_CAPACITY, "output buffer too small for this push");
    if (max_out > 0 && !host_out) return fail(RR_ERR_INVALID, "rr_chain_push: host_out is null");
    if (max_out > out_stride && S > 1) return fail(RR_ERR_INVALID, "out_stride smaller than the produced samples");
    if (!c->h2d_stream) {
        RR_CUDA(cudaStreamCreateWithFlags(&c->h2d_stream, cudaStreamNonBlocking));
        RR_CUDA(cudaStreamCreateWithFlags(&c->d2h_stream, cudaStreamNonBlocking));
        for (int k = 0; k < 2; ++k) {
            RR_CUDA(cudaEventCreateWithFlags(&c->ev_h2d[k], cudaEventDisableTiming));
            RR_CUDA(cudaEventCreateWithFlags(&c->ev_comp[k], cudaEventDisableTiming));
            RR_CUDA(cudaEventCreateWithFlags(&c->ev_d2h[k], cudaEventDisableTiming));
        }
    }
    const int b = c->slot;
    const size_t ocap = max_out ? max_out : 1;
    RR_TRY(c->stage_in[b].ensure(S * len * c->esz));
    RR_TRY(c->stage_out[b].ensure(S * ocap * c->esz));
    RR_CUDA(cudaStreamWaitEvent(c->h2d_stream, c->ev_comp[b], 0));
    if (in_stride == len || S == 1)
        RR_CUDA(cudaMemcpyAsync(c->stage_in[b].p, host_in, S * len * c->esz, cudaMemcpyHostToDevice, c->h2d_stream));
    else
        RR_CUDA(cudaMemcpy2DAsync(c->stage_in[b].p, len * c->esz, host_in, in_stride * c->esz, len * c->esz, S, cudaMemcpyHostToDevice,
                                  c->h2d_stream));
    RR_CUDA(cudaEventRecord(c->ev_h2d[b], c->h2d_stream));
    RR_CUDA(cudaStreamWaitEvent(c->stream, c->ev_h2d[b], 0));
    RR_CUDA(cudaStreamWaitEvent(c->stream, c->ev_d2h[b], 0));
    size_t produced = 0;
    RR_TRY(rr_chain_push_device(c, sample_rate, chunk_len, n_chunks, c->stage_in[b].p, len, c->stage_out[b].p, max_out, ocap, &produced,
                                out_sample_rate));
    RR_CUDA(cudaEventRecord(c->ev_comp[b], c->stream));
    if (produced > 0) {
        RR_CUDA(cudaStreamWaitEvent(c->d2h_stream, c->ev_comp[b], 0));
        if ((out_stride == ocap && produced == ocap) || S == 1)
            RR_CUDA(cudaMemcpyAsync(host_out, c->stage_out[b].p, (S == 1 ? produced : S * ocap) * c->esz, cudaMemcpyDeviceToHost, c->d2h_stream));
        else
            RR_CUDA(cudaMemcpy2DAsync(host_out, out_stride * c->esz, c->stage_out[b].p, ocap * c->esz, produced * c->esz, S,
                                      cudaMemcpyDeviceToHost, c->d2h_stream));
        RR_CUDA(cudaEventRecord(c->ev_d2h[b], c->d2h_stream));
    }
    c->slot ^= 1;
    if (out_count) *out_count = produced;
    return RR_OK;
}

int rr_chain_copy_out_async(rr_chain* c, void* dst_dev, size_t dst_stride, const void* src_dev, size_t src_stride, size_t n_samples) {
    if (!c || (!dst_dev && n_samples) || (!src_dev && n_samples)) return fail(RR_ERR_INVALID, "rr_chain_copy_out_async: null argument");
    if (n_samples == 0) return RR_OK;
    RR_CUDA(cudaSetDevice(c->ctx->device));
    if (!c->d2h_stream) {
        RR_CUDA(cudaStreamCreateWithFlags(&c->h2d_stream, cudaStreamNonBlocking));
        RR_CUDA(cudaStreamCreateWithFlags(&c->d2h_stream, cudaStreamNonBlocking));
        for (int k = 0; k < 2; ++k) {
            RR_CUDA(cudaEventCreateWithFlags(&c->ev_h2d[k], cudaEventDisableTiming));
            RR_CUDA(cudaEventCreateWithFlags(&c->ev_comp[k], cudaEventDisableTiming));
            RR_CUDA(cudaEventCreateWithFlags(&c->ev_d2h[k], cudaEventDisableTiming));
        }
    }
    if (!c->ev_copy) RR_CUDA(cudaEventCreateWithFlags(&c->ev_copy, cudaEventDisableTiming));
    RR_CUDA(cudaEventRecord(c->ev_copy, c->stream));
    RR_CUDA(cudaStreamWaitEvent(c->d2h_stream, c->ev_copy, 0));
    RR_CUDA(cudaMemcpy2DAsync(dst_dev, dst_stride * c->esz, src_dev, src_stride * c->esz, n_samples * c->esz, (size_t)c->S, cudaMemcpyDeviceToDevice,
                              c->d2h_stream));
    return RR_OK;
}

int rr_chain_sync(rr_chain* c) {
    if (!c) return fail(RR_ERR_INVALID, "null chain");
    RR_CUDA(cudaSetDevice(c->ctx->device));
    RR_CUDA(cudaStreamSynchronize(c->stream));
    if (c->d2h_stream) RR_CUDA(cudaStreamSynchronize(c->d2h_stream));
    if (c->h2d_stream) RR_CUDA(cudaStreamSynchronize(c->h2d_stream));
    return RR_OK;
}
int rr_chain_set_fast_path(rr_chain* c, int enable) {
    if (!c) return fail(RR_ERR_INVALID, "null chain");
    c->allow_poly = enable != 0;
    return RR_OK;
}
int rr_chain_set_timing(rr_chain* c, int enable) {
    if (!c) return fail(RR_ERR_INVALID, "null chain");
    RR_CUDA(cudaSetDevice(c->ctx->device));
    c->timing = enable != 0;
    c->ev_used = 0;
    return RR_OK;
}
int rr_chain_kernel_time(rr_chain* c, double* total_ms, int* n_launches, const char** kernel_name) {
    if (!c || !total_ms) return fail(RR_ERR_INVALID, "null argument");
    RR_CUDA(cudaSetDevice(c->ctx->device));
    std::vector<std::string> names;
    std::vector<double> tot;
    std::vector<int> cnt;
    for (size_t i = 0; i + 1 < c->ev_used; i += 2) {
        float ms = 0.f;
        RR_CUDA(cudaEventSynchronize(c->evs[i + 1]));
        RR_CUDA(cudaEventElapsedTime(&ms, c->evs[i], c->evs[i + 1]));
        const std::string& nm = c->ev_names[i / 2];
        size_t k = 0;
        while (k < names.size() && names[k] != nm) ++k;
        if (k == names.size()) {
            names.push_back(nm);
            tot.push_back(0.0);
            cnt.push_back(0);
        }
        tot[k] += ms;
        cnt[k] += 1;
    }
    size_t best = 0;
    c->breakdown.clear();
    for (size_t k = 0; k < names.size(); ++k) {
        if (tot[k] > tot[best]) best = k;
        char buf[160];
        std::snprintf(buf, sizeof buf, "%s%s:%.6f:%d", k ? ";" : "", names[k].c_str(), tot[k], cnt[k]);
        c->breakdown += buf;
    }
    *total_ms = names.empty() ? 0.0 : tot[best];
    if (n_launches) *n_launches = names.empty() ? 0 : cnt[best];
    c->timed_kernel = names.empty() ? "" : names[best];
    if (kernel_name) *kernel_name = c->timed_kernel.c_str();
    return RR_OK;
}
const char* rr_chain_kernel_breakdown(rr_chain* c) { return c ? c->breakdown.c_str() : ""; }
// ... 5 lines not shown
```

radiorust_b200/csrc/rr_fused.cu:

```cuda
#include <cuda.h>
#include <cuda_runtime.h>

#include <algorithm>
#include <cstdio>
#include <cstdlib>
#include <mutex>

#include "rr_kernels.h"
#include "rr_poly.cuh"
#include "rr_pk.cuh"

namespace rr {

namespace {

constexpr int FK = 512;
constexpr int FRK = 10;
constexpr int T_WARPS = FRK / 2;
constexpr int T_THREADS = 32 * T_WARPS;
constexpr int F_ROWS = 32;
constexpr int PITCH = FRK * 8;
constexpr int STAGE_ROWS = 528;
constexpr int STAGE_BYTES = STAGE_ROWS * PITCH;
constexpr int TW_UNITS = 17;
constexpr int TW_BYTES = 16 * TW_UNITS * 16;
constexpr int YS_STRIDE = FK + 1;

constexpr int kFusedSlots = 6;
constexpr int kFusedSlotFloats = 2560;
__constant__ float4 c_fcoef[kFusedSlots * kFusedSlotFloats / 4];

__device__ __forceinline__ uint32_t s_u32(const void* p) { return (uint32_t)__cvta_generic_to_shared(p); }
__device__ __forceinline__ void mb_init(uint32_t bar, uint32_t count) {
    asm volatile("mbarrier.init.shared::cta.b64 [%0], %1;" ::"r"(bar), "r"(count) : "memory");
}
__device__ __forceinline__ void mb_expect_tx(uint32_t bar, uint32_t bytes) {
    asm volatile("mbarrier.arrive.expect_tx.shared::cta.b64 _, [%0], %1;" ::"r"(bar), "r"(bytes) : "memory");
}
__device__ __forceinline__ void mb_arrive(uint32_t bar) {
    asm volatile("mbarrier.arrive.release.cta.shared::cta.b64 _, [%0];" ::"r"(bar) : "memory");
}
__device__ __forceinline__ void mb_wait(uint32_t bar, uint32_t parity) {
    asm volatile(
        "{\n"
        ".reg .pred p;\n"
        "FWAIT_%=:\n"
        "mbarrier.try_wait.parity.acquire.cta.shared::cta.b64 p, [%0], %1;\n"
        "@p bra FDONE_%=;\n"
        "bra FWAIT_%=;\n"
        "FDONE_%=:\n"
        "}\n" ::"r"(bar),
        "r"(parity)
        : "memory");
}
__device__ __forceinline__ void mb_wait_long(uint32_t bar, uint32_t parity) {
    asm volatile(
        "{\n"
        ".reg .pred p;\n"
        "LWAIT_%=:\n"
        "mbarrier.try_wait.parity.acquire.cta.shared::cta.b64 p, [%0], %1, %2;\n"
        "@p bra LDONE_%=;\n"
        "bra LWAIT_%=;\n"
        "LDONE_%=:\n"
        "}\n" ::"r"(bar),
        "r"(parity), "r"(20000u)
        : "memory");
}
__device__ __forceinline__ pc f_lds(uint32_t addr) {
    pc r;
    asm volatile("ld.shared.v2.f32 {%0, %1}, [%2];" : "=f"(r.x), "=f"(r.y) : "r"(addr));
    return r;
}
__device__ __forceinline__ void f_lds2(uint32_t addr, pc& a, pc& b) {
    asm volatile("ld.shared.v4.f32 {%0, %1, %2, %3}, [%4];" : "=f"(a.x), "=f"(a.y), "=f"(b.x), "=f"(b.y) : "r"(addr));
}
__device__ __forceinline__ void f_sts(uint32_t addr, pc a) {
    asm volatile("st.shared.v2.f32 [%0], {%1, %2};" ::"r"(addr), "f"(a.x), "f"(a.y) : "memory");
}
__device__ __forceinline__ void f_sts2(uint32_t addr, pc a, pc b) {
    asm volatile("st.shared.v4.f32 [%0], {%1, %2, %3, %4};" ::"r"(addr), "f"(a.x), "f"(a.y), "f"(b.x), "f"(b.y) : "memory");
}
__device__ __forceinline__ void f_ldg2(const float4* p, pc& a, pc& b) {
    asm volatile("ld.global.nc.v4.f32 {%0, %1, %2, %3}, [%4];" : "=f"(a.x), "=f"(a.y), "=f"(b.x), "=f"(b.y) : "l"(p));
}

__device__ __forceinline__ pc f_rotation(uint32_t d, uint32_t numer_abs, uint32_t denom, double inv_m, int sign) {
    const uint32_t r = mulmod_fast(numer_abs, d % denom, denom, inv_m);
    double s, c;
    sincospi(2.0 * (double)r / (double)denom, &s, &c);
    return pc((float)c, (float)(sign < 0 ? -s : s));
}

__device__ __forceinline__ void f_pass1_store(pc (&v)[32], uint32_t tw_row, uint32_t xch_wr) {
    pdft_regs<32, +1>(v);
    pc w[3][2];
    f_lds2(tw_row, w[0][0], w[0][1]);
    f_lds2(tw_row + 16, w[1][0], w[1][1]);
#pragma unroll
    for (int m = 0; m < 16; ++m) {
        if (m + 2 < 16) f_lds2(tw_row + (m + 2) * 16, w[(m + 2) % 3][0], w[(m + 2) % 3][1]);
        f_sts(xch_wr + (2 * m) * PITCH, pcmul(v[2 * m], w[m % 3][0]));
        f_sts(xch_wr + (2 * m + 1) * PITCH, pcmul(v[2 * m + 1], w[m % 3][1]));
    }
}

#ifdef RR_FUSED_PROF
#define PROF(...) __VA_ARGS__
__device__ long long g_fused_prof[256 * 16];
#else
#define PROF(...)
#endif

struct FusedGeom {
    int steps, S0, hp, slot_bytes, slot_stride;
};
__host__ __device__ inline FusedGeom fused_geom(int P) {
    FusedGeom g;
    g.steps = P / 2;
    g.S0 = (g.steps + 1) / 2;
    g.hp = 2 * g.S0 + ((g.S0 & 1) ? 0 : 2);
    if (g.hp > P) g.hp = P;
    g.slot_bytes = F_ROWS * g.hp * 8;
    g.slot_stride = (g.slot_bytes + 127) / 128 * 128;
    return g;
}

template <int S_LO, int S_HI, bool HAS_NCO>
__device__ __forceinline__ void f_steps(pc (&acc)[FRK], const float4* __restrict__ xrow, const float4* __restrict__ crow, const float4* cf_base) {
#pragma unroll
    for (int st = S_LO; st < S_HI; ++st) {
        const float4 xv = xrow[st];
        pc x0(xv.x, xv.y), x1(xv.z, xv.w);
        if (HAS_NCO) {
            const float4 cv = crow[st];
            x0 = pcmul(x0, pc(cv.x, cv.y));
            x1 = pcmul(x1, pc(cv.z, cv.w));
        }
        const float4* cf = cf_base + st * 5;
        const float4 a0 = cf[0], a1 = cf[1], a2 = cf[2], a3 = cf[3], a4 = cf[4];
        const float k0[FRK] = {a0.x, a0.y, a0.z, a0.w, a1.x, a1.y, a1.z, a1.w, a2.x, a2.y};
        const float k1[FRK] = {a2.z, a2.w, a3.x, a3.y, a3.z, a3.w, a4.x, a4.y, a4.z, a4.w};
#pragma unroll
        for (int c = 0; c < FRK; ++c) {
            acc[c] = pfma_s(x0, k0[c], acc[c]);
            acc[c] = pfma_s(x1, k1[c], acc[c]);
        }
    }
}

}

template <int FW, int D, int NB, bool HAS_NCO, int PT>
__global__ void __launch_bounds__(T_THREADS + 32 * FW, 1)
k_fused(const __grid_constant__ CUtensorMap tmap, const FusedArgs a, const int n_streams) {
    extern __shared__ __align__(128) unsigned char smem[];
    const int warp = __shfl_sync(0xffffffffu, (int)(threadIdx.x >> 5), 0), lane = threadIdx.x & 31;
    const int P = PT > 0 ? PT : a.P;
    const FusedGeom geo = fused_geom(P);
    const int Lmax = a.Lmax, V = a.V, n_out = a.n_out;
    const int B = (n_out + V - 1) / V;
    const int n_tiles = (B * V + F_ROWS - 1) / F_ROWS;

    const int keep_bytes = ((Lmax * PITCH) + 127) / 128 * 128;
    unsigned char* const p_stage = smem;
    unsigned char* const p_tw = p_stage + 2 * STAGE_BYTES;
    unsigned char* const p_keep = p_tw + TW_BYTES;
    unsigned char* const p_ys = p_keep + keep_bytes;
    unsigned char* const p_ring = p_ys + (((size_t)NB * YS_STRIDE * 8 + 127) / 128 * 128);
    unsigned char* const p_colph = p_ring + (size_t)FW * D * geo.slot_stride;
    unsigned char* const p_bar = p_colph + (((size_t)FW * P * 8 + 127) / 128 * 128);
    const uint32_t bar_full = s_u32(p_bar), bar_empty = bar_full + 16, bar_ring = bar_full + 32;
    const uint32_t left_cnt = bar_ring + FW * D * 8;

    for (int e = threadIdx.x; e < 2 * STAGE_BYTES / 16; e += blockDim.x) reinterpret_cast<float4*>(p_stage)[e] = make_float4(0.f, 0.f, 0.f, 0.f);
    {
        const float2* __restrict__ twK = reinterpret_cast<const float2*>(a.twK);
        for (int e = threadIdx.x; e < FK; e += blockDim.x) {
            const int tr = e >> 5, k1 = e & 31;
            const float2 w = twK[(tr * k1) & (FK - 1)];
            const int off = (tr * TW_UNITS + (k1 >> 1)) * 16 + (k1 & 1) * 8;
            *reinterpret_cast<float2*>(p_tw + off) = w;
        }
    }
    if (threadIdx.x == 0) {
        asm volatile("prefetch.tensormap [%0];" ::"l"(&tmap) : "memory");
        mb_init(bar_full, FW);
        mb_init(bar_full + 8, FW);
        mb_init(bar_empty, T_WARPS);
        mb_init(bar_empty + 8, T_WARPS);
        for (int q = 0; q < FW * D; ++q) mb_init(bar_ring + q * 8, 1);
        asm volatile("st.shared.v2.u32 [%0], {%1, %1};" ::"r"(left_cnt), "r"(0u) : "memory");
        asm volatile("fence.mbarrier_init.release.cluster;" ::: "memory");
    }
    __syncthreads();

    const int n_my = (n_streams - (int)blockIdx.x + (int)gridDim.x - 1) / (int)gridDim.x;
    if (n_my <= 0) return;

    if (warp >= T_WARPS) {
        const int fw = warp - T_WARPS;
        const uint32_t ring_s = s_u32(p_ring) + fw * (D * geo.slot_stride);
        const uint32_t rbar = bar_ring + fw * (D * 8);
        float2* const colph = reinterpret_cast<float2*>(p_colph) + fw * P;
        const int steps = geo.steps, S0 = geo.S0, hp = geo.hp;
        const int half1_col0 = P - hp;
        const int J0 = (int)a.J0;
        const int hist_len = (int)(2 * a.n);
        const int hist_from = (int)a.hist_from;
        const int n_live = (n_out + F_ROWS - 1) / F_ROWS;
        const int rot_step = n_live % FW;
        auto tiles_from = [&](int j0) { return j0 < n_tiles ? (n_tiles - j0 + FW - 1) / FW : 0; };
        const int BV = B * V;
        const int tile_step = FW * F_ROWS;

        int i_so = 0, i_k = 0, i_half = 0, i_slot = 0;
        int i_j0 = fw, i_rot = 0, i_tw = tiles_from(fw);
        auto issue_next = [&]() {
            while (i_so < n_my) {
                if (i_k >= i_tw) {
                    ++i_so;
                    i_k = 0;
                    i_rot += rot_step;
                    if (i_rot >= FW) i_rot -= FW;
                    i_j0 = fw - i_rot + (fw < i_rot ? FW : 0);
                    i_tw = tiles_from(i_j0);
                    continue;
                }
                const int j = i_j0 + i_k * FW, half = i_half, so = i_so;
                i_half ^= 1;
                if (i_half == 0) ++i_k;
                const int rows_ok = min(F_ROWS, n_out - j * F_ROWS);
                if (rows_ok <= 0) continue;
                const int pos0 = j * (F_ROWS * P) - J0;
                const int coff = half ? half1_col0 : 0;
                const int sh = pos0 < 0 ? -1 : F_ROWS - rows_ok;
                if (lane == 0) {
                    mb_expect_tx(rbar + i_slot * 8, (uint32_t)geo.slot_bytes);
                    asm volatile("cp.async.bulk.tensor.3d.shared::cluster.global.mbarrier::complete_tx::bytes [%0], [%1, {%3, %4, %5}], [%2];" ::"r"(
                                     ring_s + i_slot * geo.slot_stride),
                                 "l"(&tmap), "r"(rbar + i_slot * 8), "r"(pos0 + coff - sh * P), "r"(sh), "r"((int)blockIdx.x + so * (int)gridDim.x)
                                 : "memory");
                }
                i_slot = (i_slot + 1 == D) ? 0 : i_slot + 1;
                return;
            }
        };
#pragma unroll 1
        for (int q = 0; q < D; ++q) issue_next();

        PROF(long long pr[8] = {0, 0, 0, 0, 0, 0, 0, 0}; const long long pr_t0 = clock64();)
        int c_slot = 0;
        uint32_t c_phase = 0;
        int gb_acq = -1;
        int gb_arr = -1;
        auto arrive_upto = [&](int gb_done) {
            for (int g2 = gb_arr + 1; g2 <= gb_done; ++g2) {
                while (gb_acq < g2) {
                    ++gb_acq;
                    mb_wait(bar_empty + (uint32_t)(gb_acq & 1) * 8, (uint32_t)(((gb_acq >> 1) & 1) ^ 1));
                }
                __syncwarp();
                if (lane == 0) mb_arrive(bar_full + (uint32_t)(g2 & 1) * 8);
            }
            if (gb_done > gb_arr) gb_arr = gb_done;
        };

        int rot = 0;
#pragma unroll 1
        for (int so = 0; so < n_my; ++so) {
            PROF(const long long pst0 = clock64();)
            const int s = (int)blockIdx.x + so * (int)gridDim.x;
            const int gb0 = so * B;
            const int j0 = fw - rot + (fw < rot ? FW : 0);
            const int tiles_w = tiles_from(j0);
            rot += rot_step;
            if (rot >= FW) rot -= FW;
            uint32_t denom = 1, numer_abs = 0, idx0 = 0;
            int sign = 0;
            float start = 0.f;
            pc rot_tile(1.f, 0.f);
            double inv_denom = 1.0;
            if (HAS_NCO && j0 < n_live) {
                const NcoStream ns = a.nco[s];
                denom = ns.denom;
                numer_abs = ns.numer_abs;
                sign = ns.sign;
                idx0 = ns.idx;
                start = (float)ns.start_phase;
                inv_denom = 1.0 / (double)denom;
                rot_tile = f_rotation((uint32_t)(tile_step * P), numer_abs, denom, inv_denom, sign);
                __syncwarp();
                for (int p = lane; p < P; p += 32) {
                    const pc c = f_rotation((uint32_t)p, numer_abs, denom, inv_denom, sign);
                    colph[p] = make_float2(c.x, c.y);
                }
                __syncwarp();
            }
            const float2* __restrict__ in = reinterpret_cast<const float2*>(a.in) + (long long)s * a.in_stride;
            const float2* __restrict__ hist_end = reinterpret_cast<const float2*>(a.hist2) + ((long long)s + 1) * hist_len;
            float2* __restrict__ hist_o = a.hist_out ? reinterpret_cast<float2*>(a.hist_out) + (long long)s * a.hist_stride : nullptr;
            float4* __restrict__ keep_o = reinterpret_cast<float4*>(reinterpret_cast<float2*>(a.ukeep_out) + (long long)s * a.ukeep_out_stride);
            const float4* cf_base = c_fcoef + a.coef_off4;
            const float4* __restrict__ crow = reinterpret_cast<const float4*>(colph);

            PROF(pr[7] += clock64() - pst0;)
            int blk = (j0 * F_ROWS) / V, off = (j0 * F_ROWS) - blk * V;
            pc rowph(1.f, 0.f);
#pragma unroll 1
            for (int k = 0; k < tiles_w; ++k) {
                const int r0 = (j0 + k * FW) * F_ROWS;
                const int row = r0 + lane;
                const int pos0 = r0 * P - J0;
                pc acc[FRK];
#pragma unroll
                for (int c = 0; c < FRK; ++c) acc[c] = pc(0.f, 0.f);
                PROF(long long pc0 = clock64();)
                if (r0 < n_out) {
                    if (HAS_NCO) {
                        if ((k & 15) == 0) {
                            const long long v = (long long)idx0 + pos0 + (long long)lane * P;
                            long long kk = v - (long long)floor((double)v * inv_denom) * (long long)denom;
                            if (kk < 0) kk += denom;
                            else if (kk >= (long long)denom) kk -= denom;
                            const cx<float> c = nco_phasor<float>(mulmod_fast(numer_abs, (uint32_t)kk, denom, inv_denom), denom, sign, start);
                            rowph = pc(c.x, c.y);
                        } else {
                            rowph = pcmul(rowph, rot_tile);
                        }
                    }
                    const int prow = pos0 + lane * P;
                    const bool to_hist = hist_o != nullptr && pos0 + F_ROWS * P > hist_from;
#pragma unroll 1
                    for (int half = 0; half < 2; ++half) {
                        const uint32_t slot_s = ring_s + c_slot * geo.slot_stride;
                        PROF(long long pw0 = clock64(); pr[0] += pw0 - pc0;)
                        mb_wait(rbar + c_slot * 8, c_phase);
                        PROF(long long pw1 = clock64(); pr[1] += pw1 - pw0;)
                        const int col0 = half ? half1_col0 : 0;
                        if (pos0 < 0) {
                            float2* dst = reinterpret_cast<float2*>(smem + (slot_s - s_u32(smem)));
                            const float r0x = __shfl_sync(0xffffffffu, rowph.x, 0), r0y = __shfl_sync(0xffffffffu, rowph.y, 0);
                            for (int cc = lane; cc < hp; cc += 32) {
                                const int p = col0 + cc;
                                const int pos = pos0 + p;
                                float2 q = make_float2(0.f, 0.f);
                                if (pos >= 0) {
                                    if (pos < (int)a.len) q = __ldg(in + pos);
                                } else if (pos >= -hist_len) {
                                    q = __ldg(hist_end + pos);
                                    if (HAS_NCO) {
                                        const float2 cph = colph[p];
                                        const pc y = pcmulc(pc(q.x, q.y), pcmul(pc(r0x, r0y), pc(cph.x, cph.y)));
                                        q = make_float2(y.x, y.y);
                                    }
                                }
                                dst[cc] = q;
                            }
                            __syncwarp();
                        }
                        const float4* __restrict__ xrow = reinterpret_cast<const float4*>(smem + (slot_s - s_u32(smem)) + lane * (hp * 8) - col0 * 8);
                        if (to_hist) {
                            const int st_lo = half ? S0 : 0, st_hi = half ? steps : S0;
#pragma unroll 2
                            for (int st = st_lo; st < st_hi; ++st) {
                                const float4 xv = xrow[st];
                                pc x0(xv.x, xv.y), x1(xv.z, xv.w);
                                if (HAS_NCO) {
                                    const float4 cv = crow[st];
                                    x0 = pcmul(x0, pc(cv.x, cv.y));
                                    x1 = pcmul(x1, pc(cv.z, cv.w));
                                }
                                const pc y0 = HAS_NCO ? pcmul(x0, rowph) : x0, y1 = HAS_NCO ? pcmul(x1, rowph) : x1;
                                const int jh = prow + 2 * st - hist_from;
                                if (row < n_out && jh >= -1) {
                                    if (jh >= 0) hist_o[jh] = make_float2(y0.x, y0.y);
                                    hist_o[jh + 1] = make_float2(y1.x, y1.y);
                                }
                                const float4* cf = cf_base + st * 5;
                                const float4 a0 = cf[0], a1 = cf[1], a2 = cf[2], a3 = cf[3], a4 = cf[4];
                                const float k0[FRK] = {a0.x, a0.y, a0.z, a0.w, a1.x, a1.y, a1.z, a1.w, a2.x, a2.y};
                                const float k1[FRK] = {a2.z, a2.w, a3.x, a3.y, a3.z, a3.w, a4.x, a4.y, a4.z, a4.w};
#pragma unroll
                                for (int c = 0; c < FRK; ++c) {
                                    acc[c] = pfma_s(x0, k0[c], acc[c]);
                                    acc[c] = pfma_s(x1, k1[c], acc[c]);
                                }
                            }
                        } else if constexpr (PT > 0) {
                            constexpr int STEPS_C = PT / 2, S0_C = (STEPS_C + 1) / 2;
                            if (half == 0) f_steps<0, S0_C, HAS_NCO>(acc, xrow, crow, cf_base);
                            else f_steps<S0_C, STEPS_C, HAS_NCO>(acc, xrow, crow, cf_base);
                        } else {
                            const int st_lo = half ? S0 : 0, st_hi = half ? steps : S0;
#pragma unroll 4
                            for (int st = st_lo; st < st_hi; ++st) {
                                const float4 xv = xrow[st];
                                pc x0(xv.x, xv.y), x1(xv.z, xv.w);
                                if (HAS_NCO) {
                                    const float4 cv = crow[st];
                                    x0 = pcmul(x0, pc(cv.x, cv.y));
                                    x1 = pcmul(x1, pc(cv.z, cv.w));
                                }
                                const float4* cf = cf_base + st * 5;
                                const float4 a0 = cf[0], a1 = cf[1], a2 = cf[2], a3 = cf[3], a4 = cf[4];
                                const float k0[FRK] = {a0.x, a0.y, a0.z, a0.w, a1.x, a1.y, a1.z, a1.w, a2.x, a2.y};
                                const float k1[FRK] = {a2.z, a2.w, a3.x, a3.y, a3.z, a3.w, a4.x, a4.y, a4.z, a4.w};
#pragma unroll
                                for (int c = 0; c < FRK; ++c) {
                                    acc[c] = pfma_s(x0, k0[c], acc[c]);
                                    acc[c] = pfma_s(x1, k1[c], acc[c]);
                                }
                            }
                        }
                        PROF(long long ps1 = clock64(); pr[2] += ps1 - pw1;)
                        asm volatile("fence.proxy.async.shared::cta;" ::: "memory");
                        __syncwarp();
                        PROF(long long ps2 = clock64(); pr[3] += ps2 - ps1;)
                        if (++c_slot == D) {
                            c_slot = 0;
                            c_phase ^= 1u;
                        }
                        issue_next();
                        PROF(pc0 = clock64(); pr[4] += pc0 - ps2;)
                    }
                }
                {
                    const int last_off = min(off + F_ROWS, BV - blk * V) - 1;
                    const int gb_hi = gb0 + blk + (last_off >= V ? 1 : 0);
                    PROF(long long pe0 = clock64(); pr[0] += pe0 - pc0;)
                    while (gb_acq < gb_hi) {
                        ++gb_acq;
                        mb_wait(bar_empty + (uint32_t)(gb_acq & 1) * 8, (uint32_t)(((gb_acq >> 1) & 1) ^ 1));
                    }
                    PROF(pc0 = clock64(); pr[5] += pc0 - pe0;)
                }
                if (row < BV) {
                    int b = blk, o = off + lane;
                    if (o >= V) {
                        o -= V;
                        ++b;
                    }
                    const uint32_t dst = s_u32(p_stage) + (uint32_t)((gb0 + b) & 1) * STAGE_BYTES + (Lmax + o) * PITCH;
                    const bool live = row < n_out;
                    const bool keep = live && row >= n_out - Lmax;
#pragma unroll
                    for (int c = 0; c < FRK; c += 2) {
                        pc y0 = acc[c], y1 = acc[c + 1];
                        if (HAS_NCO) {
                            y0 = pcmul(y0, rowph);
                            y1 = pcmul(y1, rowph);
                        }
                        if (!live) {
                            y0 = pc(0.f, 0.f);
                            y1 = pc(0.f, 0.f);
                        }
                        f_sts2(dst + c * 8, y0, y1);
                        if (keep) keep_o[((row - (n_out - Lmax)) * FRK + c) / 2] = make_float4(y0.x, y0.y, y1.x, y1.y);
                    }
                }
                __syncwarp();
                off += tile_step;
                while (off >= V) {
                    off -= V;
                    ++blk;
                }
                arrive_upto((k + 1 < tiles_w) ? gb0 + min(blk, B) - 1 : gb0 + B - 1);
                PROF(pr[6] += clock64() - pc0;)
            }
            if (tiles_w == 0) arrive_upto(gb0 + B - 1);
        }
        PROF(if (fw == 0 && lane == 0) {
            for (int q = 0; q < 7; ++q) g_fused_prof[blockIdx.x * 16 + q] = pr[q];
            g_fused_prof[blockIdx.x * 16 + 7] = pr[7];
            g_fused_prof[blockIdx.x * 16 + 8] = clock64() - pr_t0;
        })
        return;
    }

    const int tid = threadIdx.x;
    const int t = lane >> 1, gg = lane & 1;
    const int g = 2 * warp + gg;
    auto sync_t = [&]() { asm volatile("bar.sync 1, %0;" ::"n"(T_THREADS) : "memory"); };
    const uint32_t stage0 = s_u32(p_stage);
    const uint32_t tw_row = s_u32(p_tw) + t * (TW_UNITS * 16);
    const uint32_t tile_rd = t * PITCH + g * 8;
    const uint32_t xch_wr = 33 * t * PITCH + g * 8;
    const uint32_t xch_rd = t * PITCH + g * 8;
    const uint32_t keep_s = s_u32(p_keep) + warp * 16;
    float2* const ysave = reinterpret_cast<float2*>(p_ys);
    const float4* __restrict__ gtab = reinterpret_cast<const float4*>(a.gtab);
    const int hist_rows_per_lane = (Lmax + 31) / 32;

    const int n_blocks_total = n_my * B;
    auto copy_kept = [&](int so_k, int gb_k) {
        const uint32_t bytes = (uint32_t)(Lmax * PITCH), bar = bar_full + (uint32_t)(gb_k & 1) * 8;
        const float2* src = reinterpret_cast<const float2*>(a.ukeep_in) + (long long)((int)blockIdx.x + so_k * (int)gridDim.x) * a.ukeep_in_stride;
        asm volatile("fence.proxy.async.shared::cta;" ::: "memory");
        asm volatile("mbarrier.expect_tx.relaxed.cta.shared::cta.b64 [%0], %1;" ::"r"(bar), "r"(bytes) : "memory");
        asm volatile("cp.async.bulk.shared::cluster.global.mbarrier::complete_tx::bytes [%0], [%1], %2, [%3];" ::"r"(stage0 + (uint32_t)(gb_k & 1) * STAGE_BYTES),
                     "l"(src), "r"(bytes), "r"(bar)
                     : "memory");
    };
    if (tid == 0) {
        copy_kept(0, 0);
        if (B == 1 && n_my > 1) copy_kept(1, 1);
    }
    int parked = 0;
    int gb_first = 0;
    int so = 0, b = -1;
    PROF(long long tp[6] = {0, 0, 0, 0, 0, 0}; long long tc = clock64();)

#pragma unroll 1
    for (int gb = 0; gb < n_blocks_total; ++gb) {
        if (++b == B) {
            b = 0;
            ++so;
        }
        const int s = (int)blockIdx.x + so * (int)gridDim.x;
        const uint32_t stg = stage0 + (uint32_t)(gb & 1) * STAGE_BYTES;

        PROF({ long long n_ = clock64(); tp[0] += n_ - tc; tc = n_; })
        mb_wait_long(bar_full + (uint32_t)(gb & 1) * 8, (uint32_t)((gb >> 1) & 1));
        PROF({ long long n_ = clock64(); tp[1] += n_ - tc; tc = n_; })
#pragma unroll
        for (int q = 0; q < 12; ++q) {
            const int r = lane + 32 * q;
            if (q < hist_rows_per_lane && r < Lmax) {
                float4 nx;
                asm volatile("ld.shared.v4.f32 {%0, %1, %2, %3}, [%4];" : "=f"(nx.x), "=f"(nx.y), "=f"(nx.z), "=f"(nx.w) : "r"(stg + (V + r) * PITCH + warp * 16));
                if (b != 0) {
                    float4 h;
                    asm volatile("ld.shared.v4.f32 {%0, %1, %2, %3}, [%4];" : "=f"(h.x), "=f"(h.y), "=f"(h.z), "=f"(h.w) : "r"(keep_s + r * PITCH));
                    asm volatile("st.shared.v4.f32 [%0], {%1, %2, %3, %4};" ::"r"(stg + r * PITCH + warp * 16), "f"(h.x), "f"(h.y), "f"(h.z), "f"(h.w) : "memory");
                }
                asm volatile("st.shared.v4.f32 [%0], {%1, %2, %3, %4};" ::"r"(keep_s + r * PITCH), "f"(nx.x), "f"(nx.y), "f"(nx.z), "f"(nx.w) : "memory");
            }
        }
        if (b == 0 && n_out < Lmax) {
            float4* __restrict__ kout = reinterpret_cast<float4*>(reinterpret_cast<float2*>(a.ukeep_out) + (long long)s * a.ukeep_out_stride);
#pragma unroll 1
            for (int r = n_out + lane; r < Lmax; r += 32) {
                float4 h;
                asm volatile("ld.shared.v4.f32 {%0, %1, %2, %3}, [%4];" : "=f"(h.x), "=f"(h.y), "=f"(h.z), "=f"(h.w) : "r"(stg + r * PITCH + warp * 16));
                kout[((long long)(r - n_out) * FRK) / 2 + warp] = h;
            }
        }
        if (lane == 0) asm volatile("st.shared.v4.f32 [%0], {%1, %1, %1, %1};" ::"r"(stg + (FK - 1) * PITCH + warp * 16), "f"(0.f) : "memory");
        __syncwarp();

        pc acc[32];
        {
            pc v[32];
            const uint32_t src = stg + tile_rd;
#pragma unroll
            for (int m = 0; m < 32; ++m) v[m] = f_lds(src + m * (16 * PITCH));
            __syncwarp();
            f_pass1_store(v, tw_row, stg + xch_wr);
        }
        {
            const float4* gp = gtab + tid;
            pc h[16];
#pragma unroll
            for (int jj = 0; jj < 8; ++jj) f_ldg2(gp + jj * T_THREADS, h[2 * jj], h[2 * jj + 1]);
            __syncwarp();
#pragma unroll
            for (int which = 0; which < 2; ++which) {
                pc x[16];
#pragma unroll
                for (int tr = 0; tr < 16; ++tr) x[tr] = f_lds(stg + xch_rd + (33 * tr + 16 * which) * PITCH);
                pdft_regs<16, +1>(x);
#pragma unroll
                for (int k = 0; k < 16; ++k) acc[which * 16 + k] = pcmul(x[k], h[k]);
                if (which == 0) {
#pragma unroll
                    for (int jj = 0; jj < 8; ++jj) f_ldg2(gp + (8 + jj) * T_THREADS, h[2 * jj], h[2 * jj + 1]);
                }
            }
        }
        PROF({ long long n_ = clock64(); tp[2] += n_ - tc; tc = n_; })
        __syncwarp();
#pragma unroll
        for (int j = 0; j < 32; ++j) f_sts(stg + xch_rd + (16 * j) * PITCH, acc[j]);
        sync_t();
        if (parked == 0) gb_first = gb;
        {
            float2* ys = ysave + parked * YS_STRIDE;
            for (int o = tid; o < FK; o += T_THREADS) {
                const uint32_t src = stg + o * PITCH;
                pc sum(0.f, 0.f);
#pragma unroll
                for (int w = 0; w < T_WARPS; ++w) {
                    pc u0, u1;
                    f_lds2(src + w * 16, u0, u1);
                    sum = sum + u0;
                    sum = sum + u1;
                }
                const int j = o >> 4, tt = o & 15;
                ys[tt + 16 * (j >> 4) + 32 * (j & 15)] = make_float2(sum.x, sum.y);
            }
        }
        ++parked;
        PROF({ long long n_ = clock64(); tp[3] += n_ - tc; tc = n_; })

        if (parked == NB || gb + 1 == n_blocks_total) {
            sync_t();
#pragma unroll 1
            for (int j0 = 0; j0 < parked; j0 += FRK) {
                if (j0 + 2 * warp >= parked) continue;
                const int job = j0 + g;
                const bool active = job < parked;
                pc v[32];
                const float2* ys = ysave + (active ? job : 0) * YS_STRIDE;
#pragma unroll
                for (int i1 = 0; i1 < 32; ++i1) {
                    const float2 q = ys[t + 16 * i1];
                    v[i1] = active ? pc(q.x, -q.y) : pc(0.f, 0.f);
                }
                f_pass1_store(v, tw_row, stg + xch_wr);
                __syncwarp();
                const int gj = gb_first + (active ? job : 0);
                const int so_j = gj / B, b_j = gj - so_j * B;
                const int s_j = (int)blockIdx.x + so_j * (int)gridDim.x;
                float2* __restrict__ out = reinterpret_cast<float2*>(a.out) + (long long)s_j * a.out_stride;
                float2* __restrict__ out2 = a.out2 ? reinterpret_cast<float2*>(a.out2) + (long long)s_j * a.out2_stride : nullptr;
#pragma unroll
                for (int which = 0; which < 2; ++which) {
                    pc x[16];
#pragma unroll
                    for (int tr = 0; tr < 16; ++tr) x[tr] = f_lds(stg + xch_rd + (33 * tr + 16 * which) * PITCH);
                    pdft_regs<16, +1>(x);
                    if (active) {
#pragma unroll
                        for (int k2 = 0; k2 < 16; ++k2) {
                            const int i = t + 16 * which + 32 * k2;
                            if (i >= Lmax && i < Lmax + V) {
                                const long long o = (long long)b_j * V + (i - Lmax);
                                if (o < n_out) {
                                    float2* dst = (out2 != nullptr && o >= a.out_split) ? out2 + (o - a.out_split) : out + o;
                                    *dst = make_float2(x[k2].x, -x[k2].y);
                                }
                            }
                        }
                    }
                }
                __syncwarp();
            }
            parked = 0;
            sync_t();
        }
        PROF({ long long n_ = clock64(); tp[4] += n_ - tc; tc = n_; })
        __syncwarp();
        if (lane == 0) {
            uint32_t left;
            asm volatile("atom.acq_rel.cta.shared::cta.add.u32 %0, [%1], 1;" : "=r"(left) : "r"(left_cnt + (uint32_t)(gb & 1) * 4) : "memory");
            if (left % T_WARPS == T_WARPS - 1) {
                int b2 = b + 2, so2 = so;
                while (b2 >= B) {
                    b2 -= B;
                    ++so2;
                }
                if (b2 == 0 && so2 < n_my) copy_kept(so2, gb + 2);
            }
            mb_arrive(bar_empty + (uint32_t)(gb & 1) * 8);
        }
    }
    PROF(if (tid == 0) for (int q = 0; q < 5; ++q) g_fused_prof[blockIdx.x * 16 + 9 + q] = tp[q];)
}

namespace {

using EncodeFn = CUresult (*)(CUtensorMap*, CUtensorMapDataType, cuuint32_t, void*, const cuuint64_t*, const cuuint64_t*, const cuuint32_t*,
                              const cuuint32_t*, CUtensorMapInterleave, CUtensorMapSwizzle, CUtensorMapL2promotion, CUtensorMapFloatOOBfill);
EncodeFn fused_encode_fn() {
    static EncodeFn fn = nullptr;
    static std::once_flag once;
    std::call_once(once, [] {
        void* p = nullptr;
        cudaDriverEntryPointQueryResult q;
        if (cudaGetDriverEntryPoint("cuTensorMapEncodeTiled", &p, cudaEnableDefault, &q) == cudaSuccess && q == cudaDriverEntryPointSuccess)
            fn = reinterpret_cast<EncodeFn>(p);
    });
    return fn;
}

template <int FW, int D, int NB> size_t fused_smem(int P, int Lmax) {
    const FusedGeom geo = fused_geom(P);
    size_t b = 2 * (size_t)STAGE_BYTES + TW_BYTES;
    b += ((size_t)Lmax * PITCH + 127) / 128 * 128;
    b += ((size_t)NB * YS_STRIDE * 8 + 127) / 128 * 128;
    b += (size_t)FW * D * geo.slot_stride;
    b += ((size_t)FW * P * 8 + 127) / 128 * 128;
    b += 32 + (size_t)FW * D * 8 + 64;
    return b;
}

template <int FW, int D, int NB>
cudaError_t launch_cfg(int n_streams, const FusedArgs& a, const CUtensorMap& tm, int sm_count, cudaStream_t st) {
    const size_t smem = fused_smem<FW, D, NB>(a.P, a.Lmax);
    if (smem > (size_t)227 * 1024) return cudaErrorInvalidConfiguration;
    const int grid = std::min(n_streams, sm_count);
    void (*kern)(const CUtensorMap, const FusedArgs, const int);
    switch (a.P) {
        case 50: kern = a.nco ? k_fused<FW, D, NB, true, 50> : k_fused<FW, D, NB, false, 50>; break;
        case 40: kern = a.nco ? k_fused<FW, D, NB, true, 40> : k_fused<FW, D, NB, false, 40>; break;
        case 20: kern = a.nco ? k_fused<FW, D, NB, true, 20> : k_fused<FW, D, NB, false, 20>; break;
        default: return cudaErrorNotSupported;
    }
    const cudaError_t e = cudaFuncSetAttribute(kern, cudaFuncAttributeMaxDynamicSharedMemorySize, (int)smem);
    if (e != cudaSuccess) return e;
    kern<<<grid, T_THREADS + 32 * FW, smem, st>>>(tm, a, n_streams);
#ifdef RR_FUSED_PROF
    static int calls = 0;
    static int at = std::getenv("RR_FUSED_PROF_CALL") ? std::atoi(std::getenv("RR_FUSED_PROF_CALL")) : 12;
    if (++calls == at) {
        cudaDeviceSynchronize();
        long long h[256 * 16];
        cudaMemcpyFromSymbol(h, g_fused_prof, sizeof h);
        for (int c : {0, 100})
            fprintf(stderr,
                    "cta %d n_out %d F0: tile-head %lld ring-wait %lld steps %lld fence+sync %lld issue %lld empty-wait %lld finalize %lld stream-setup %lld | total %lld"
                    " || T0: pre %lld wait-full %lld fwd+prod %lld sum+park %lld inverse %lld\n",
                    c, a.n_out, h[c * 16], h[c * 16 + 1], h[c * 16 + 2], h[c * 16 + 3], h[c * 16 + 4], h[c * 16 + 5], h[c * 16 + 6], h[c * 16 + 7], h[c * 16 + 8], h[c * 16 + 9],
                    h[c * 16 + 10], h[c * 16 + 11], h[c * 16 + 12], h[c * 16 + 13]);
    }
#endif
    return cudaGetLastError();
}

}

int fused_coef_slots() { return kFusedSlots; }

bool fused_supported(int rank_pad, long long P, int Lmax) {
    if (rank_pad != FRK || !(P == 50 || P == 40 || P == 20) || fused_encode_fn() == nullptr) return false;
    if (Lmax < 1 || FK - 1 - Lmax < 128 || Lmax > 383) return false;
    if ((P / 2) * 2 * FRK > kFusedSlotFloats) return false;
    return fused_smem<7, 2, 5>((int)P, Lmax) <= (size_t)227 * 1024;
}

cudaError_t fused_upload_coef(int slot, const float* acoef, int P, cudaStream_t st) {
    if (slot < 0 || slot >= kFusedSlots) return cudaErrorInvalidValue;
    const size_t n = (size_t)(P / 2) * 2 * FRK;
    if (n > (size_t)kFusedSlotFloats) return cudaErrorInvalidValue;
    return cudaMemcpyToSymbolAsync(c_fcoef, acoef, n * sizeof(float), (size_t)slot * kFusedSlotFloats * sizeof(float), cudaMemcpyHostToDevice, st);
}

cudaError_t launch_fused(int n_streams, const FusedArgs& a0, int sm_count, cudaStream_t st) {
    EncodeFn enc = fused_encode_fn();
    if (!enc) return cudaErrorNotSupported;
    FusedArgs a = a0;
    a.coef_off4 = a.coef_slot * (kFusedSlotFloats / 4);
    if ((uintptr_t)a.ukeep_in % 16 != 0 || (n_streams > 1 && a.ukeep_in_stride % 2 != 0)) return cudaErrorInvalidValue;
    const FusedGeom geo = fused_geom(a.P);
    CUtensorMap tm;
    const cuuint64_t dims[3] = {(cuuint64_t)a.len, (cuuint64_t)F_ROWS, (cuuint64_t)n_streams};
    const cuuint64_t sstride = n_streams > 1 ? (cuuint64_t)a.in_stride * 8 : (((cuuint64_t)a.len * 8 + 15) / 16) * 16;
    const cuuint64_t strides[2] = {(cuuint64_t)a.P * 8, sstride};
    const cuuint32_t box[3] = {(cuuint32_t)geo.hp, (cuuint32_t)F_ROWS, 1};
    const cuuint32_t estr[3] = {1, 1, 1};
    const CUresult r = enc(&tm, CU_TENSOR_MAP_DATA_TYPE_UINT64, 3, const_cast<void*>(a.in), dims, strides, box, estr, CU_TENSOR_MAP_INTERLEAVE_NONE,
                           CU_TENSOR_MAP_SWIZZLE_NONE, CU_TENSOR_MAP_L2_PROMOTION_L2_128B, CU_TENSOR_MAP_FLOAT_OOB_FILL_NONE);
    if (r != CUDA_SUCCESS) return cudaErrorInvalidValue;
    static int cfg = -1;
    if (cfg < 0) {
        cfg = 0;
        if (const char* e = std::getenv("RR_FUSED_CFG")) cfg = std::atoi(e);
    }
    switch (cfg) {
        case 1: return launch_cfg<6, 2, 8>(n_streams, a, tm, sm_count, st);
        default: return launch_cfg<7, 2, 5>(n_streams, a, tm, sm_count, st);
    }
}

}
```

radiorust_b200/csrc/rr_kernels.h:

```cpp
#pragma once
#include <cuda_runtime.h>
#include <stdint.h>

namespace rr {

struct NcoStream {
    uint32_t numer_abs;
    uint32_t denom;
    uint32_t idx;
    int32_t sign;
    double start_phase;
};

struct RateState {
    long long P, Q, j0, m0;
};

template <typename T> struct ChainOsArgs {
    const void* in;
    long long in_stride;
    int n_chunks;
    int first_is_history;
    int emit;
    int reserved;
    const void* hist_in;
    long long hist_stride;
    void* hist_out;
    const void* hperm;
    const void* twN;
    const NcoStream* nco;
    long long nco_offset;
    void* out;
    long long out_stride;
    const T* ir;
    int L;
    const void* ztail_in;
    void* ztail_out;
    RateState rate;
};

template <typename T>
cudaError_t launch_chain_os(int n, int epi, int n_streams, int parts, const ChainOsArgs<T>& a, cudaStream_t st);
template <typename T> bool chain_os_supported(int n, int epi, int L);
template <typename T> int chain_os_threads(int n);
template <typename T> int chain_os_hperm_index(int n, int k);

template <typename T>
cudaError_t launch_freqshift(const void* in, long long in_stride, void* out, long long out_stride, long long len,
                             int n_streams, const NcoStream* nco, long long nco_offset, cudaStream_t st);

cudaError_t launch_nco_advance(NcoStream* nco, int n_streams, long long len, cudaStream_t st);

template <typename T>
cudaError_t launch_gain(const void* in, long long in_stride, void* out, long long out_stride, long long len,
                        int n_streams, double gain, cudaStream_t st);

template <typename T>
cudaError_t launch_downsample(const void* in, long long in_stride, long long len, const void* tail_in, void* tail_out,
                              const T* ir, int L, RateState rate, long long n_out, void* out, long long out_stride,
                              int n_streams, cudaStream_t st);

template <typename T>
cudaError_t launch_upsample(const void* in, long long in_stride, long long len, const void* acc_in, void* acc_out,
                            const T* ir, int L, RateState rate, long long n_out, void* out, long long out_stride,
                            int n_streams, cudaStream_t st, void* out2 = nullptr, long long out2_stride = 0, long long out_split = 0);
template <typename T> bool upsample_tiled_supported(RateState rate, int L);

template <typename T>
cudaError_t launch_downsample_indexed(const void* in, long long in_stride, long long len, const void* tail_in, void* tail_out, const T* ir, int L,
                                      const int* fire, long long n_out, void* out, long long out_stride, int n_streams, cudaStream_t st);
template <typename T>
cudaError_t launch_upsample_indexed(const void* in, long long in_stride, long long len, const void* acc_in, void* acc_out, const T* ir, int L,
                                    const int* qpos, const int* cnt, long long n_out, void* out, long long out_stride, int n_streams,
                                    cudaStream_t st);

template <typename T>
cudaError_t launch_fmdemod(const void* in, long long in_stride, void* out, long long out_stride, long long len,
                           int n_streams, void* prev_sample, void* last_output, int has_prev, double factor,
                           cudaStream_t st);

template <typename T>
cudaError_t launch_fmmod(const void* in, long long in_stride, void* out, long long out_stride, long long len, int n_streams, void* phase,
                         double factor, int sm_count, cudaStream_t st);

template <typename T>
cudaError_t launch_overlap(const void* a, long long a_stride, long long a_len, const void* b, long long b_stride, void* out,
                           long long out_stride, long long n_out, long long span, long long hop, long long base, int n_streams,
                           cudaStream_t st);

constexpr int kFourierDirectMax = 4096;
template <typename T> bool fourier_fft_supported(int n);
template <typename T>
cudaError_t launch_fourier(int n, const void* in, long long in_stride, void* out, long long out_stride, int n_chunks, int n_streams,
                           const T* window, const void* twN, int rot, cudaStream_t st);

template <typename T>
cudaError_t launch_level(const void* in, long long in_stride, long long chunk_len, long long n_chunks, int n_streams, double* out,
                         cudaStream_t st);

template <typename T>
cudaError_t launch_bandwidth(const void* in, long long in_stride, long long chunk_len, long long n_chunks, int n_streams,
                             double double_percentile, double sample_rate, double* out, cudaStream_t st);
template <typename T>
cudaError_t launch_rescale_energy(const void* in, long long in_stride, long long chunk_len, long long n_chunks, int n_streams,
                                  long long resolution, void* out, cudaStream_t st);

template <typename T>
cudaError_t launch_copy2d(const void* in, long long in_stride, void* out, long long out_stride, long long len,
                          int n_streams, cudaStream_t st);

template <typename T> struct BigOsArgs {
    const void* in;
    long long in_stride;
    const void* hist;
    long long hist_stride;
    int first_chunk;
    int n_blocks;
    void* scratch;
    const void* hbig;
    const void* twN;
    const void* twA;
    const void* twB;
    void* out;
    long long out_stride;
    const void* twC;
};
template <typename T> bool big_os_supported(int n);
template <typename T> void big_os_shape(int n, int* Na, int* Nb);
template <typename T> long long big_os_hperm_index(int n, long long k);
template <typename T>
cudaError_t launch_big_os(int n, int n_streams, const BigOsArgs<T>& a, cudaStream_t st);
bool long_os_supported(int n);
void long_os_shape(int n, int* Na, int* Nb);
long long long_os_hperm_index(int n, long long k);
template <typename T>
cudaError_t launch_long_os(int n, int n_streams, const BigOsArgs<T>& a, cudaStream_t st);
template <typename T> int long_os_twc_size(int n);
template <typename T> long long long_os_twc_exponent(int n, int i);

template <typename T> struct PolyArgs {
    const void* in;
    long long in_stride;
    long long len;
    const void* hist2;
    long long n;
    const NcoStream* nco;
    const void* gtab;
    const void* twK;
    long long P, Q;
    int Lmax, V;
    int n_blocks, nbpc;
    int ngrp;
    int halves;
    void* out2;
    long long out2_stride, out_split;
    int sab_blocks, sab_rb, sab_streams;
    long long sab_in_step, sab_out_step, sab_out2_step;
    long long J0, m0;
    long long m_lo, m_hi;
    long long I_lo;
    void* out;
    long long out_stride;
};
template <typename T> bool poly_supported(int K, int Q, int G);
template <typename T> int poly_hperm_index(int K, int k);
template <typename T> size_t poly_smem_bytes(int K, int Q, int G, int nbpc);
template <typename T> cudaError_t launch_poly(int K, int Q, int G, int n_streams, const PolyArgs<T>& a, cudaStream_t st);

bool poly2_supported(int K, long long P, long long Q);
int poly2_pick_G(long long P);
size_t poly2_smem_bytes(int G, int nbpc);
long long poly2_table_index(int G, int r, int g, int k);
cudaError_t launch_poly2(int G, int n_streams, const PolyArgs<float>& a, cudaStream_t st);

struct FrontArgs {
    const void* in;
    long long in_stride;
    long long len;
    const void* hist2;
    long long n;
    const NcoStream* nco;
    const float* acoef;
    int P;
    long long J0;
    long long row_first;
    int n_rows;
    void* u;
    long long u_stride;
    int tiles_per_warp;
    int has_hist_map;
    void* hist_out;
    long long hist_from, hist_stride;
    int hist_staged;
    const void* kept_src;
    long long kept_stride;
    int kept_rows;
};
bool front_supported(int rank_pad, long long P);
cudaError_t launch_front(int rank_pad, int n_streams, const FrontArgs& a, cudaStream_t st);
bool front_wide_supported(int rank_pad, long long P);
cudaError_t launch_front_wide(int rank_pad, int n_streams, const FrontArgs& a, cudaStream_t st);

struct FusedArgs {
    const void* in;
    long long in_stride;
    long long len;
    const void* hist2;
    long long n;
    const NcoStream* nco;
    int P;
    int coef_slot;
    int coef_off4;
    long long J0;
    int n_out;
    int Lmax, V;
    const void* ukeep_in;
    long long ukeep_in_stride;
    void* ukeep_out;
    long long ukeep_out_stride;
    const void* gtab;
    const void* twK;
    void* out;
    long long out_stride;
    void* out2;
    long long out2_stride, out_split;
    void* hist_out;
    long long hist_from, hist_stride;
};
bool fused_supported(int rank_pad, long long P, int Lmax);
int fused_coef_slots();
cudaError_t fused_upload_coef(int slot, const float* acoef, int P, cudaStream_t st);
cudaError_t launch_fused(int n_streams, const FusedArgs& a, int sm_count, cudaStream_t st);

template <typename T>
cudaError_t launch_hist2_update(const void* in, long long in_stride, long long len, const void* hist2_in, void* hist2_out,
                                long long n, const NcoStream* nco, int n_streams, cudaStream_t st, long long j_lo = 0, long long j_hi = -1);

}
```

Baseline: 528,900.

## Add tcgen05 tensor-core front end to fused FreqShift-Filter-Downsample kernel

Adds a new fused kernel variant whose polyphase front end runs on Blackwell tcgen05 MMA with a TMA-fed slot pipeline and split-TF32 hi/lo correction. The FFT transform role moves into a shared helper. The tensor path is selected by default when shared memory allows, and RR_FUSED_FRONT=simt restores the old SIMT path. The aim is to cut the FMA-bound front-end filtering cost, in exchange for more complexity, TF32-split precision risk, and heavier shared-memory use that may limit pipelining. An A/B profiling script is included.

```diff
diff --git a/profiles/fused_ab.py b/profiles/fused_ab.py
--- /dev/null
+++ b/profiles/fused_ab.py
@@ -0,0 +1,116 @@
+import argparse
+import json
+import os
+import subprocess
+import sys
+
+import numpy as np
+
+ROOT = os.path.dirname(os.path.dirname(os.path.abspath(__file__)))
+sys.path.insert(0, ROOT)
+
+import bench
+
+
+def make_chain(rr, ctx, S, front):
+    os.environ["RR_FUSED_FRONT"] = front
+    try:
+        stages = [rr.FreqShifter(0.0), rr.Filter.new(bench.lowpass(bench.CUTOFF)), rr.Downsampler(bench.OUT_CHUNK, bench.OUT_RATE, bench.BANDWIDTH)]
+        chain = rr.Chain(ctx, stages, "f32", n_streams=S)
+    finally:
+        del os.environ["RR_FUSED_FRONT"]
+    chain.set_shifts(0, [bench.stream_shift(g) for g in range(S)])
+    return chain
+
+
+def power_limit():
+    try:
+        r = subprocess.run(["nvidia-smi", "--query-gpu=power.limit", "--format=csv,noheader"], capture_output=True, text=True, timeout=30)
+        return r.stdout.strip().splitlines()[0] if r.returncode == 0 else "unknown"
+    except (OSError, subprocess.SubprocessError, IndexError):
+        return "unknown"
+
+
+def main():
+    ap = argparse.ArgumentParser(description=__doc__, formatter_class=argparse.RawDescriptionHelpFormatter)
+    ap.add_argument("--streams", type=int, default=4096)
+    ap.add_argument("--chunks", type=int, default=50)
+    ap.add_argument("--rounds", type=int, default=5)
+    ap.add_argument("--pushes", type=int, default=20)
+    ap.add_argument("--warmup", type=int, default=3)
+    args = ap.parse_args()
+
+    import torch
+    import radiorust_b200 as rr
+
+    if not torch.cuda.is_available():
+        raise SystemExit("fused_ab.py: no CUDA device")
+    S, C_ = args.streams, args.chunks
+    length = C_ * bench.CHUNK_LEN
+    ctx = rr.Context(0)
+    forms = {"simt": make_chain(rr, ctx, S, "simt"), "tensor": make_chain(rr, ctx, S, "tensor")}
+
+    gen = torch.Generator(device="cuda")
+    gen.manual_seed(20260000 + 3 * 100000)
+    x = torch.randn((S, length, 2), device="cuda", dtype=torch.float32, generator=gen)
+    cap = forms["simt"].max_output(bench.SAMPLE_RATE, bench.CHUNK_LEN, C_ + 1) + bench.OUT_CHUNK
+    ys = {k: torch.zeros((S, cap, 2), device="cuda", dtype=torch.float32) for k in forms}
+    torch.cuda.synchronize()
+
+    def push(k):
+        return forms[k].push_device(bench.SAMPLE_RATE, bench.CHUNK_LEN, C_, x.data_ptr(), length, ys[k].data_ptr(), cap, cap)
+
+    for k in forms:
+        for _ in range(args.warmup):
+            push(k)
+        forms[k].sync()
+    torch.cuda.synchronize()
+
+    times = {k: [] for k in forms}
+    kernel = {k: [] for k in forms}
+    cnt = {}
+    for _ in range(args.rounds):
+        for k, chain in forms.items():
+            ext = torch.cuda.ExternalStream(chain.cuda_stream)
+            e0, e1 = torch.cuda.Event(enable_timing=True), torch.cuda.Event(enable_timing=True)
+            chain.set_timing(True)
+            with torch.cuda.stream(ext):
+                e0.record(ext)
+                for _ in range(args.pushes):
+                    cnt[k], _ = push(k)
+                e1.record(ext)
+            chain.sync()
+            torch.cuda.synchronize()
+            times[k].append(e0.elapsed_time(e1) / args.pushes)
+            k_ms, k_n, k_name = chain.kernel_time()
+            kernel[k].append((k_ms / max(k_n, 1), k_name))
+            chain.set_timing(False)
+
+    assert cnt["simt"] == cnt["tensor"], cnt
+    n = cnt["simt"]
+    a = ys["tensor"][:, :n].double()
+    b = ys["simt"][:, :n].double()
+    d = (a - b).pow(2).sum(dim=(1, 2)).sqrt()
+    ref = b.pow(2).sum(dim=(1, 2)).sqrt()
+    rel = (d / ref).cpu().numpy()
+    rms = (ref / np.sqrt(n)).cpu().numpy()
+    maxd = (a - b).abs().amax(dim=(1, 2)).cpu().numpy() / rms
+    worst = int(np.argmax(rel))
+
+    samples = S * length
+    res = {"card": torch.cuda.get_device_name(0), "power_limit": power_limit(), "streams": S, "chunks": C_,
+           "rounds": args.rounds, "pushes_per_round": args.pushes}
+    for k in forms:
+        t = np.array(times[k])
+        kt = np.array([v for v, _ in kernel[k]])
+        res[k] = {"push_ms_median": float(np.median(t)), "push_ms_min": float(t.min()), "push_ms_max": float(t.max()),
+                  "spread_pct": float(100 * (t.max() - t.min()) / np.median(t)), "GS_per_s": float(samples / np.median(t) / 1e6),
+                  "kernel": kernel[k][-1][1], "kernel_ms_median": float(np.median(kt)), "plan": forms[k].plan}
+    res["speedup_tensor_over_simt"] = res["simt"]["push_ms_median"] / res["tensor"]["push_ms_median"]
+    res["outputs"] = {"per_stream_outputs": n, "worst_rel_l2": float(rel[worst]), "worst_stream": worst,
+                      "max_rel_l2_all": float(rel.max()), "worst_maxabs_over_rms": float(maxd.max())}
+    print(json.dumps(res, indent=1), flush=True)
+
+
+if __name__ == "__main__":
+    main()
diff --git a/radiorust_b200/csrc/rr_chain.cu b/radiorust_b200/csrc/rr_chain.cu
--- a/radiorust_b200/csrc/rr_chain.cu
+++ b/radiorust_b200/csrc/rr_chain.cu
@@ -248,6 +248,7 @@
     bool allow_fused = true;
     int fused_min_streams = -1;
     long long fused_min_rows = 1;
+    rr::FusedFront fused_front = rr::FusedFront::Tensor;
     bool timing = false;
     std::vector<cudaEvent_t> evs;
     size_t ev_used = 0;
@@ -1275,6 +1276,7 @@
                     DevBuf& kb = ds.ukeep[ds.ukeep_cur];
                     RR_TRY(kb.ensure(kbytes));
                     rr::FusedArgs fu{};
+                    fu.front = c->fused_front;
                     fu.in = a.in;
                     fu.in_stride = a.in_stride;
                     fu.len = a.len;
@@ -1315,7 +1317,7 @@
                         f.hist_fused_jlo = cover_hi - hfrom;
                         f.hist_fused_jfirst = hstart - hfrom;
                     }
-                    RR_TIMED_LAUNCH(c, "k_fused", 1, rr::launch_fused(S, fu, c->ctx->sm_count, st));
+                    RR_TIMED_LAUNCH(c, rr::fused_tc_selected(fu) ? "k_fused_tc" : "k_fused", 1, rr::launch_fused(S, fu, c->ctx->sm_count, st));
                     ds.ucache_valid = true;
                     ds.ucache_rows = n_out + Lh;
                     ds.ucache_ptr = kb.p;
@@ -2367,6 +2369,7 @@
     c->fused_min_streams = 2 * ctx->sm_count;
     if (const char* e = std::getenv("RR_FUSED_MIN_STREAMS")) c->fused_min_streams = std::max(1, std::atoi(e));
     if (const char* e = std::getenv("RR_FUSED_MIN_ROWS")) c->fused_min_rows = std::max(1, std::atoi(e));
+    if (const char* e = std::getenv("RR_FUSED_FRONT")) c->fused_front = std::strcmp(e, "simt") == 0 ? rr::FusedFront::Simt : rr::FusedFront::Tensor;
     if (const char* e = std::getenv("RR_DISABLE_UCACHE")) c->allow_ucache = !(e[0] == '1');
     if (const char* e = std::getenv("RR_DISABLE_SAB")) c->allow_sab = !(e[0] == '1');
     if (const char* e = std::getenv("RR_BIG_OS_SCRATCH_MB")) c->big_os_scratch_bytes = (size_t)std::max(1, std::atoi(e)) << 20;
diff --git a/radiorust_b200/csrc/rr_fused.cu b/radiorust_b200/csrc/rr_fused.cu
--- a/radiorust_b200/csrc/rr_fused.cu
+++ b/radiorust_b200/csrc/rr_fused.cu
@@ -148,6 +148,201 @@
     }
 }
 
+}
+
+template <int NB>
+__device__ __forceinline__ void transform_role(const FusedArgs& a, unsigned char* const p_stage, unsigned char* const p_tw, unsigned char* const p_keep,
+                                               unsigned char* const p_ys, const uint32_t bar_full, const uint32_t bar_empty, const uint32_t left_cnt,
+                                               const int n_my, const int B, const int warp, const int lane) {
+    const int Lmax = a.Lmax, V = a.V, n_out = a.n_out;
+    const int tid = threadIdx.x;
+    const int t = lane >> 1, gg = lane & 1;
+    const int g = 2 * warp + gg;
+    auto sync_t = [&]() { asm volatile("bar.sync 1, %0;" ::"n"(T_THREADS) : "memory"); };
+    const uint32_t stage0 = s_u32(p_stage);
+    const uint32_t tw_row = s_u32(p_tw) + t * (TW_UNITS * 16);
+    const uint32_t tile_rd = t * PITCH + g * 8;
+    const uint32_t xch_wr = 33 * t * PITCH + g * 8;
+    const uint32_t xch_rd = t * PITCH + g * 8;
+    const uint32_t keep_s = s_u32(p_keep) + warp * 16;
+    float2* const ysave = reinterpret_cast<float2*>(p_ys);
+    const float4* __restrict__ gtab = reinterpret_cast<const float4*>(a.gtab);
+    const int hist_rows_per_lane = (Lmax + 31) / 32;
+
+    const int n_blocks_total = n_my * B;
+    auto copy_kept = [&](int so_k, int gb_k) {
+        const uint32_t bytes = (uint32_t)(Lmax * PITCH), bar = bar_full + (uint32_t)(gb_k & 1) * 8;
+        const float2* src = reinterpret_cast<const float2*>(a.ukeep_in) + (long long)((int)blockIdx.x + so_k * (int)gridDim.x) * a.ukeep_in_stride;
+        asm volatile("fence.proxy.async.shared::cta;" ::: "memory");
+        asm volatile("mbarrier.expect_tx.relaxed.cta.shared::cta.b64 [%0], %1;" ::"r"(bar), "r"(bytes) : "memory");
+        asm volatile("cp.async.bulk.shared::cluster.global.mbarrier::complete_tx::bytes [%0], [%1], %2, [%3];" ::"r"(stage0 + (uint32_t)(gb_k & 1) * STAGE_BYTES),
+                     "l"(src), "r"(bytes), "r"(bar)
+                     : "memory");
+    };
+    if (tid == 0) {
+        copy_kept(0, 0);
+        if (B == 1 && n_my > 1) copy_kept(1, 1);
+    }
+    int parked = 0;
+    int gb_first = 0;
+    int so = 0, b = -1;
+    PROF(long long tp[6] = {0, 0, 0, 0, 0, 0}; long long tc = clock64();)
+
+#pragma unroll 1
+    for (int gb = 0; gb < n_blocks_total; ++gb) {
+        if (++b == B) {
+            b = 0;
+            ++so;
+        }
+        const int s = (int)blockIdx.x + so * (int)gridDim.x;
+        const uint32_t stg = stage0 + (uint32_t)(gb & 1) * STAGE_BYTES;
+
+        PROF({ long long n_ = clock64(); tp[0] += n_ - tc; tc = n_; })
+        mb_wait_long(bar_full + (uint32_t)(gb & 1) * 8, (uint32_t)((gb >> 1) & 1));
+        PROF({ long long n_ = clock64(); tp[1] += n_ - tc; tc = n_; })
+#pragma unroll
+        for (int q = 0; q < 12; ++q) {
+            const int r = lane + 32 * q;
+            if (q < hist_rows_per_lane && r < Lmax) {
+                float4 nx;
+                asm volatile("ld.shared.v4.f32 {%0, %1, %2, %3}, [%4];" : "=f"(nx.x), "=f"(nx.y), "=f"(nx.z), "=f"(nx.w) : "r"(stg + (V + r) * PITCH + warp * 16));
+                if (b != 0) {
+                    float4 h;
+                    asm volatile("ld.shared.v4.f32 {%0, %1, %2, %3}, [%4];" : "=f"(h.x), "=f"(h.y), "=f"(h.z), "=f"(h.w) : "r"(keep_s + r * PITCH));
+                    asm volatile("st.shared.v4.f32 [%0], {%1, %2, %3, %4};" ::"r"(stg + r * PITCH + warp * 16), "f"(h.x), "f"(h.y), "f"(h.z), "f"(h.w) : "memory");
+                }
+                asm volatile("st.shared.v4.f32 [%0], {%1, %2, %3, %4};" ::"r"(keep_s + r * PITCH), "f"(nx.x), "f"(nx.y), "f"(nx.z), "f"(nx.w) : "memory");
+            }
+        }
+        if (b == 0 && n_out < Lmax) {
+            float4* __restrict__ kout = reinterpret_cast<float4*>(reinterpret_cast<float2*>(a.ukeep_out) + (long long)s * a.ukeep_out_stride);
+#pragma unroll 1
+            for (int r = n_out + lane; r < Lmax; r += 32) {
+                float4 h;
+                asm volatile("ld.shared.v4.f32 {%0, %1, %2, %3}, [%4];" : "=f"(h.x), "=f"(h.y), "=f"(h.z), "=f"(h.w) : "r"(stg + r * PITCH + warp * 16));
+                kout[((long long)(r - n_out) * FRK) / 2 + warp] = h;
+            }
+        }
+        if (lane == 0) asm volatile("st.shared.v4.f32 [%0], {%1, %1, %1, %1};" ::"r"(stg + (FK - 1) * PITCH + warp * 16), "f"(0.f) : "memory");
+        __syncwarp();
+
+        pc acc[32];
+        {
+            pc v[32];
+            const uint32_t src = stg + tile_rd;
+#pragma unroll
+            for (int m = 0; m < 32; ++m) v[m] = f_lds(src + m * (16 * PITCH));
+            __syncwarp();
+            f_pass1_store(v, tw_row, stg + xch_wr);
+        }
+        {
+            const float4* gp = gtab + tid;
+            pc h[16];
+#pragma unroll
+            for (int jj = 0; jj < 8; ++jj) f_ldg2(gp + jj * T_THREADS, h[2 * jj], h[2 * jj + 1]);
+            __syncwarp();
+#pragma unroll
+            for (int which = 0; which < 2; ++which) {
+                pc x[16];
+#pragma unroll
+                for (int tr = 0; tr < 16; ++tr) x[tr] = f_lds(stg + xch_rd + (33 * tr + 16 * which) * PITCH);
+                pdft_regs<16, +1>(x);
+#pragma unroll
+                for (int k = 0; k < 16; ++k) acc[which * 16 + k] = pcmul(x[k], h[k]);
+                if (which == 0) {
+#pragma unroll
+                    for (int jj = 0; jj < 8; ++jj) f_ldg2(gp + (8 + jj) * T_THREADS, h[2 * jj], h[2 * jj + 1]);
+                }
+            }
+        }
+        PROF({ long long n_ = clock64(); tp[2] += n_ - tc; tc = n_; })
+        __syncwarp();
+#pragma unroll
+        for (int j = 0; j < 32; ++j) f_sts(stg + xch_rd + (16 * j) * PITCH, acc[j]);
+        sync_t();
+        if (parked == 0) gb_first = gb;
+        {
+            float2* ys = ysave + parked * YS_STRIDE;
+            for (int o = tid; o < FK; o += T_THREADS) {
+                const uint32_t src = stg + o * PITCH;
+                pc sum(0.f, 0.f);
+#pragma unroll
+                for (int w = 0; w < T_WARPS; ++w) {
+                    pc u0, u1;
+                    f_lds2(src + w * 16, u0, u1);
+                    sum = sum + u0;
+                    sum = sum + u1;
+                }
+                const int j = o >> 4, tt = o & 15;
+                ys[tt + 16 * (j >> 4) + 32 * (j & 15)] = make_float2(sum.x, sum.y);
+            }
+        }
+        ++parked;
+        PROF({ long long n_ = clock64(); tp[3] += n_ - tc; tc = n_; })
+
+        if (parked == NB || gb + 1 == n_blocks_total) {
+            sync_t();
+#pragma unroll 1
+            for (int j0 = 0; j0 < parked; j0 += FRK) {
+                if (j0 + 2 * warp >= parked) continue;
+                const int job = j0 + g;
+                const bool active = job < parked;
+                pc v[32];
+                const float2* ys = ysave + (active ? job : 0) * YS_STRIDE;
+#pragma unroll
+                for (int i1 = 0; i1 < 32; ++i1) {
+                    const float2 q = ys[t + 16 * i1];
+                    v[i1] = active ? pc(q.x, -q.y) : pc(0.f, 0.f);
+                }
+                f_pass1_store(v, tw_row, stg + xch_wr);
+                __syncwarp();
+                const int gj = gb_first + (active ? job : 0);
+                const int so_j = gj / B, b_j = gj - so_j * B;
+                const int s_j = (int)blockIdx.x + so_j * (int)gridDim.x;
+                float2* __restrict__ out = reinterpret_cast<float2*>(a.out) + (long long)s_j * a.out_stride;
+                float2* __restrict__ out2 = a.out2 ? reinterpret_cast<float2*>(a.out2) + (long long)s_j * a.out2_stride : nullptr;
+#pragma unroll
+                for (int which = 0; which < 2; ++which) {
+                    pc x[16];
+#pragma unroll
+                    for (int tr = 0; tr < 16; ++tr) x[tr] = f_lds(stg + xch_rd + (33 * tr + 16 * which) * PITCH);
+                    pdft_regs<16, +1>(x);
+                    if (active) {
+#pragma unroll
+                        for (int k2 = 0; k2 < 16; ++k2) {
+                            const int i = t + 16 * which + 32 * k2;
+                            if (i >= Lmax && i < Lmax + V) {
+                                const long long o = (long long)b_j * V + (i - Lmax);
+                                if (o < n_out) {
+                                    float2* dst = (out2 != nullptr && o >= a.out_split) ? out2 + (o - a.out_split) : out + o;
+                                    *dst = make_float2(x[k2].x, -x[k2].y);
+                                }
+                            }
+                        }
+                    }
+                }
+                __syncwarp();
+            }
+            parked = 0;
+            sync_t();
+        }
+        PROF({ long long n_ = clock64(); tp[4] += n_ - tc; tc = n_; })
+        __syncwarp();
+        if (lane == 0) {
+            uint32_t left;
+            asm volatile("atom.acq_rel.cta.shared::cta.add.u32 %0, [%1], 1;" : "=r"(left) : "r"(left_cnt + (uint32_t)(gb & 1) * 4) : "memory");
+            if (left % T_WARPS == T_WARPS - 1) {
+                int b2 = b + 2, so2 = so;
+                while (b2 >= B) {
+                    b2 -= B;
+                    ++so2;
+                }
+                if (b2 == 0 && so2 < n_my) copy_kept(so2, gb + 2);
+            }
+            mb_arrive(bar_empty + (uint32_t)(gb & 1) * 8);
+        }
+    }
+    PROF(if (tid == 0) for (int q = 0; q < 5; ++q) g_fused_prof[blockIdx.x * 16 + 9 + q] = tp[q];)
 }
 
 template <int FW, int D, int NB, bool HAS_NCO, int PT>
@@ -477,194 +672,454 @@
         return;
     }
 
-    const int tid = threadIdx.x;
-    const int t = lane >> 1, gg = lane & 1;
-    const int g = 2 * warp + gg;
-    auto sync_t = [&]() { asm volatile("bar.sync 1, %0;" ::"n"(T_THREADS) : "memory"); };
-    const uint32_t stage0 = s_u32(p_stage);
-    const uint32_t tw_row = s_u32(p_tw) + t * (TW_UNITS * 16);
-    const uint32_t tile_rd = t * PITCH + g * 8;
-    const uint32_t xch_wr = 33 * t * PITCH + g * 8;
-    const uint32_t xch_rd = t * PITCH + g * 8;
-    const uint32_t keep_s = s_u32(p_keep) + warp * 16;
-    float2* const ysave = reinterpret_cast<float2*>(p_ys);
-    const float4* __restrict__ gtab = reinterpret_cast<const float4*>(a.gtab);
-    const int hist_rows_per_lane = (Lmax + 31) / 32;
-
-    const int n_blocks_total = n_my * B;
-    auto copy_kept = [&](int so_k, int gb_k) {
-        const uint32_t bytes = (uint32_t)(Lmax * PITCH), bar = bar_full + (uint32_t)(gb_k & 1) * 8;
-        const float2* src = reinterpret_cast<const float2*>(a.ukeep_in) + (long long)((int)blockIdx.x + so_k * (int)gridDim.x) * a.ukeep_in_stride;
-        asm volatile("fence.proxy.async.shared::cta;" ::: "memory");
-        asm volatile("mbarrier.expect_tx.relaxed.cta.shared::cta.b64 [%0], %1;" ::"r"(bar), "r"(bytes) : "memory");
-        asm volatile("cp.async.bulk.shared::cluster.global.mbarrier::complete_tx::bytes [%0], [%1], %2, [%3];" ::"r"(stage0 + (uint32_t)(gb_k & 1) * STAGE_BYTES),
-                     "l"(src), "r"(bytes), "r"(bar)
-                     : "memory");
+    transform_role<NB>(a, p_stage, p_tw, p_keep, p_ys, bar_full, bar_empty, left_cnt, n_my, B, warp, lane);
+}
+
+namespace {
+constexpr int TC_M = 64;
+constexpr int TC_NH = 24;
+constexpr int TC_N = 2 * TC_NH;
+constexpr int TC_ACC = 4;
+constexpr int TC_ACC_COLS = 64;
+constexpr int TC_TMEM_COLS = TC_ACC * TC_ACC_COLS;
+constexpr int TC_MAX_SLOTS = 8;
+constexpr int TC_BAR_BYTES = 512;
+constexpr int E_WARPS = 4;
+constexpr int TC_THREADS = T_THREADS + 64 + 32 * E_WARPS;
+constexpr uint32_t TC_IDESC = (1u << 4) | (2u << 7) | (2u << 10) | ((uint32_t)(TC_N >> 3) << 17) | ((uint32_t)(TC_M >> 4) << 24);
+
+struct TcGeom {
+    int kc, ks, slot_bytes, b_bytes;
+};
+__host__ __device__ inline TcGeom tc_geom(int P) {
+    TcGeom g;
+    g.kc = P / 2;
+    g.ks = (g.kc + 1) / 2;
+    g.slot_bytes = 2 * g.ks * TC_M * 16;
+    g.b_bytes = 2 * g.ks * TC_N * 16;
+    return g;
+}
+
+__device__ __forceinline__ uint64_t tc_desc(uint32_t saddr, uint32_t lbo) {
+    return (uint64_t)((saddr >> 4) & 0x3FFFu) | ((uint64_t)((lbo >> 4) & 0x3FFFu) << 16) | ((uint64_t)(128u >> 4) << 32) | (1ull << 46);
+}
+__device__ __forceinline__ void tc_mma(uint32_t d, uint64_t adesc, uint64_t bdesc, uint32_t acc) {
+    asm volatile(
+        "{\n.reg .pred p;\nsetp.ne.b32 p, %4, 0;\n"
+        "tcgen05.mma.cta_group::1.kind::tf32 [%0], %1, %2, %3, p;\n}" ::"r"(d),
+        "l"(adesc), "l"(bdesc), "r"(TC_IDESC), "r"(acc)
+        : "memory");
+}
+__device__ __forceinline__ void tc_commit(uint32_t bar) {
+    asm volatile("tcgen05.commit.cta_group::1.mbarrier::arrive::one.shared::cluster.b64 [%0];" ::"r"(bar) : "memory");
+}
+__device__ __forceinline__ void tc_fence_before() { asm volatile("tcgen05.fence::before_thread_sync;" ::: "memory"); }
+__device__ __forceinline__ void tc_fence_after() { asm volatile("tcgen05.fence::after_thread_sync;" ::: "memory"); }
+__device__ __forceinline__ float tf32_hi(float v) { return __uint_as_float(__float_as_uint(v) & 0xffffe000u); }
+__device__ __forceinline__ float tf32_rn(float v) { return __uint_as_float((__float_as_uint(v) + 0x1000u) & 0xffffe000u); }
+
+__device__ __forceinline__ pc tc_rowph(long long pos, const NcoStream& ns) {
+    const uint32_t denom = ns.denom;
+    const double inv_denom = 1.0 / (double)denom;
+    const long long v = (long long)ns.idx + pos;
+    long long kk = v - (long long)floor((double)v * inv_denom) * (long long)denom;
+    if (kk < 0) kk += denom;
+    else if (kk >= (long long)denom) kk -= denom;
+    const cx<float> c = nco_phasor<float>(mulmod_fast(ns.numer_abs, (uint32_t)kk, denom, inv_denom), denom, ns.sign, (float)ns.start_phase);
+    return pc(c.x, c.y);
+}
+}
+
+template <int NB, bool HAS_NCO>
+__global__ void __launch_bounds__(TC_THREADS, 1)
+k_fused_tc(const __grid_constant__ CUtensorMap tmap, const FusedArgs a, const int n_streams, const int n_slots) {
+    extern __shared__ __align__(128) unsigned char smem[];
+    const int warp = __shfl_sync(0xffffffffu, (int)(threadIdx.x >> 5), 0), lane = threadIdx.x & 31;
+    const int P = a.P;
+    const TcGeom geo = tc_geom(P);
+    const int Lmax = a.Lmax, V = a.V, n_out = a.n_out;
+    const int B = (n_out + V - 1) / V;
+    const int n_tiles = (B * V + TC_M - 1) / TC_M;
+    const int n_live = (n_out + TC_M - 1) / TC_M;
+    const int S = n_slots;
+
+    const int keep_bytes = ((Lmax * PITCH) + 127) / 128 * 128;
+    unsigned char* const p_stage = smem;
+    unsigned char* const p_tw = p_stage + 2 * STAGE_BYTES;
+    unsigned char* const p_keep = p_tw + TW_BYTES;
+    unsigned char* const p_ys = p_keep + keep_bytes;
+    unsigned char* const p_bar = p_ys + (((size_t)NB * YS_STRIDE * 8 + 127) / 128 * 128);
+    unsigned char* const p_colph = p_bar + TC_BAR_BYTES;
+    unsigned char* const p_b = p_colph + (((size_t)P * 8 + 127) / 128 * 128);
+    unsigned char* const p_slots = p_b + geo.b_bytes;
+    const uint32_t bar_full = s_u32(p_bar), bar_empty = bar_full + 16, left_cnt = bar_full + 32, tmem_slot = bar_full + 40;
+    const uint32_t bar_load = bar_full + 48;
+    const uint32_t bar_ready1 = bar_load + 8 * TC_MAX_SLOTS;
+    const uint32_t bar_mma1 = bar_ready1 + 8 * TC_MAX_SLOTS;
+    const uint32_t bar_ready2 = bar_mma1 + 8 * TC_MAX_SLOTS;
+    const uint32_t bar_free = bar_ready2 + 8 * TC_MAX_SLOTS;
+    const uint32_t bar_accf = bar_free + 8 * TC_MAX_SLOTS;
+    const uint32_t bar_acce = bar_accf + 8 * TC_ACC;
+
+    for (int e = threadIdx.x; e < 2 * STAGE_BYTES / 16; e += blockDim.x) reinterpret_cast<float4*>(p_stage)[e] = make_float4(0.f, 0.f, 0.f, 0.f);
+    for (int e = threadIdx.x; e < geo.b_bytes / 16; e += blockDim.x) reinterpret_cast<float4*>(p_b)[e] = make_float4(0.f, 0.f, 0.f, 0.f);
+    {
+        const float2* __restrict__ twK = reinterpret_cast<const float2*>(a.twK);
+        for (int e = threadIdx.x; e < FK; e += blockDim.x) {
+            const int tr = e >> 5, k1 = e & 31;
+            const float2 w = twK[(tr * k1) & (FK - 1)];
+            const int off = (tr * TW_UNITS + (k1 >> 1)) * 16 + (k1 & 1) * 8;
+            *reinterpret_cast<float2*>(p_tw + off) = w;
+        }
+    }
+    if (threadIdx.x == 0) {
+        asm volatile("prefetch.tensormap [%0];" ::"l"(&tmap) : "memory");
+        mb_init(bar_full, E_WARPS);
+        mb_init(bar_full + 8, E_WARPS);
+        mb_init(bar_empty, T_WARPS);
+        mb_init(bar_empty + 8, T_WARPS);
+        for (int q = 0; q < S; ++q) {
+            mb_init(bar_load + q * 8, 1);
+            mb_init(bar_ready1 + q * 8, E_WARPS);
+            mb_init(bar_mma1 + q * 8, 1);
+            mb_init(bar_ready2 + q * 8, E_WARPS);
+            mb_init(bar_free + q * 8, 1);
+        }
+        for (int q = 0; q < TC_ACC; ++q) {
+            mb_init(bar_accf + q * 8, 1);
+            mb_init(bar_acce + q * 8, E_WARPS);
+        }
+        asm volatile("st.shared.v2.u32 [%0], {%1, %1};" ::"r"(left_cnt), "r"(0u) : "memory");
+        asm volatile("fence.mbarrier_init.release.cluster;" ::: "memory");
+    }
+    const int mma_warp = T_WARPS + 1;
+    if (warp == mma_warp) {
+        asm volatile("tcgen05.alloc.cta_group::1.sync.aligned.shared::cta.b32 [%0], %1;" ::"r"(tmem_slot), "n"(TC_TMEM_COLS) : "memory");
+        asm volatile("tcgen05.relinquish_alloc_permit.cta_group::1.sync.aligned;" ::: "memory");
+    }
+    tc_fence_before();
+    __syncthreads();
+    const int n_my = __shfl_sync(0xffffffffu, (n_streams - (int)blockIdx.x + (int)gridDim.x - 1) / (int)gridDim.x, 0);
+    if (warp < T_WARPS) {
+        transform_role<NB>(a, p_stage, p_tw, p_keep, p_ys, bar_full, bar_empty, left_cnt, n_my, B, warp, lane);
+        return;
+    }
+    tc_fence_after();
+    uint32_t tmem;
+    asm volatile("ld.shared.u32 %0, [%1];" : "=r"(tmem) : "r"(tmem_slot) : "memory");
+    const int J0 = (int)a.J0;
+
+    if (warp == T_WARPS) {
+        if (lane == 0) {
+            int L = 0, slot = 0;
+            uint32_t ph = 0;
+#pragma unroll 1
+            for (int so = 0; so < n_my; ++so) {
+                const int s = (int)blockIdx.x + so * (int)gridDim.x;
+#pragma unroll 1
+                for (int j = 0; j < n_live; ++j, ++L) {
+                    if (L >= S) mb_wait(bar_free + slot * 8, ph ^ 1u);
+                    const int pos0 = j * (TC_M * P) - J0;
+                    const int rows_ok = min(TC_M, n_out - j * TC_M);
+                    const int sh = pos0 < 0 ? -1 : TC_M - rows_ok;
+                    const uint32_t bar = bar_load + slot * 8;
+                    mb_expect_tx(bar, (uint32_t)geo.slot_bytes);
+                    asm volatile(
+                        "cp.async.bulk.tensor.4d.shared::cluster.global.mbarrier::complete_tx::bytes [%0], [%1, {%3, %4, %5, %6}], [%2];" ::"r"(
+                            s_u32(p_slots) + slot * geo.slot_bytes),
+                        "l"(&tmap), "r"(bar), "r"(pos0 - sh * P), "r"(sh), "r"(0), "r"(s)
+                        : "memory");
+                    if (++slot == S) {
+                        slot = 0;
+                        ph ^= 1u;
+                    }
+                }
+            }
+        }
+        return;
+    }
+
+    if (warp == mma_warp) {
+        if (lane == 0) {
+            const uint32_t a_lbo = TC_M * 16, b_lbo = TC_N * 16;
+            const uint64_t bd = tc_desc(s_u32(p_b), b_lbo);
+            const int n_live_total = n_my * n_live;
+            int slot = 0;
+            uint32_t ph = 0;
+#pragma unroll 1
+            for (int L = 0; L < n_live_total; ++L) {
+                const int acc = L & (TC_ACC - 1);
+                const uint32_t d = tmem + acc * TC_ACC_COLS;
+                const uint64_t ad = tc_desc(s_u32(p_slots) + slot * geo.slot_bytes, a_lbo);
+                mb_wait(bar_ready1 + slot * 8, ph);
+                mb_wait(bar_acce + acc * 8, ((L / TC_ACC) & 1) ^ 1u);
+                tc_fence_after();
+#pragma unroll 1
+                for (int k = 0; k < geo.ks; ++k) tc_mma(d, ad + (uint64_t)(k * 2 * TC_M), bd + (uint64_t)(k * 2 * TC_N), k > 0 ? 1u : 0u);
+                tc_commit(bar_mma1 + slot * 8);
+                mb_wait(bar_ready2 + slot * 8, ph);
+                tc_fence_after();
+#pragma unroll 1
+                for (int k = 0; k < geo.ks; ++k) tc_mma(d, ad + (uint64_t)(k * 2 * TC_M), bd + (uint64_t)(k * 2 * TC_N), 1u);
+                tc_commit(bar_free + slot * 8);
+                tc_commit(bar_accf + acc * 8);
+                if (++slot == S) {
+                    slot = 0;
+                    ph ^= 1u;
+                }
+            }
+        }
+        __syncwarp();
+        asm volatile("bar.sync 2, %0;" ::"n"(32 + 32 * E_WARPS) : "memory");
+        tc_fence_after();
+        asm volatile("tcgen05.dealloc.cta_group::1.sync.aligned.b32 %0, %1;" ::"r"(tmem), "n"(TC_TMEM_COLS) : "memory");
+        return;
+    }
+
+    const int et = threadIdx.x - (T_WARPS + 2) * 32;
+    const int sub = warp & 3;
+    const int er = 16 * sub + lane;
+    const bool e_row = lane < 16;
+    auto sync_e = [&]() { asm volatile("bar.sync 3, %0;" ::"n"(32 * E_WARPS) : "memory"); };
+    float2* const colph = reinterpret_cast<float2*>(p_colph);
+    const float* const cf = reinterpret_cast<const float*>(c_fcoef + a.coef_off4);
+    const int hist_len = (int)(2 * a.n);
+    const long long hist_from = a.hist_from;
+    const int BV = B * V;
+    const int G = n_my * n_tiles;
+
+    double2 rot_tile = make_double2(1.0, 0.0), rowph_d = make_double2(1.0, 0.0);
+    pc rowph(1.f, 0.f);
+    int gb0 = 0, blk = 0, off = 0;
+    int gb_acq = -1, gb_arr = -1;
+    auto arrive_upto = [&](int gb_done) {
+        for (int g2 = gb_arr + 1; g2 <= gb_done; ++g2) {
+            while (gb_acq < g2) {
+                ++gb_acq;
+                mb_wait(bar_empty + (uint32_t)(gb_acq & 1) * 8, (uint32_t)(((gb_acq >> 1) & 1) ^ 1));
+            }
+            __syncwarp();
+            if (lane == 0) mb_arrive(bar_full + (uint32_t)(g2 & 1) * 8);
+        }
+        if (gb_done > gb_arr) gb_arr = gb_done;
     };
-    if (tid == 0) {
-        copy_kept(0, 0);
-        if (B == 1 && n_my > 1) copy_kept(1, 1);
-    }
-    int parked = 0;
-    int gb_first = 0;
-    int so = 0, b = -1;
-    PROF(long long tp[6] = {0, 0, 0, 0, 0, 0}; long long tc = clock64();)
 
 #pragma unroll 1
-    for (int gb = 0; gb < n_blocks_total; ++gb) {
-        if (++b == B) {
-            b = 0;
-            ++so;
-        }
-        const int s = (int)blockIdx.x + so * (int)gridDim.x;
-        const uint32_t stg = stage0 + (uint32_t)(gb & 1) * STAGE_BYTES;
-
-        PROF({ long long n_ = clock64(); tp[0] += n_ - tc; tc = n_; })
-        mb_wait_long(bar_full + (uint32_t)(gb & 1) * 8, (uint32_t)((gb >> 1) & 1));
-        PROF({ long long n_ = clock64(); tp[1] += n_ - tc; tc = n_; })
-#pragma unroll
-        for (int q = 0; q < 12; ++q) {
-            const int r = lane + 32 * q;
-            if (q < hist_rows_per_lane && r < Lmax) {
-                float4 nx;
-                asm volatile("ld.shared.v4.f32 {%0, %1, %2, %3}, [%4];" : "=f"(nx.x), "=f"(nx.y), "=f"(nx.z), "=f"(nx.w) : "r"(stg + (V + r) * PITCH + warp * 16));
-                if (b != 0) {
-                    float4 h;
-                    asm volatile("ld.shared.v4.f32 {%0, %1, %2, %3}, [%4];" : "=f"(h.x), "=f"(h.y), "=f"(h.z), "=f"(h.w) : "r"(keep_s + r * PITCH));
-                    asm volatile("st.shared.v4.f32 [%0], {%1, %2, %3, %4};" ::"r"(stg + r * PITCH + warp * 16), "f"(h.x), "f"(h.y), "f"(h.z), "f"(h.w) : "memory");
-                }
-                asm volatile("st.shared.v4.f32 [%0], {%1, %2, %3, %4};" ::"r"(keep_s + r * PITCH), "f"(nx.x), "f"(nx.y), "f"(nx.z), "f"(nx.w) : "memory");
-            }
-        }
-        if (b == 0 && n_out < Lmax) {
-            float4* __restrict__ kout = reinterpret_cast<float4*>(reinterpret_cast<float2*>(a.ukeep_out) + (long long)s * a.ukeep_out_stride);
-#pragma unroll 1
-            for (int r = n_out + lane; r < Lmax; r += 32) {
-                float4 h;
-                asm volatile("ld.shared.v4.f32 {%0, %1, %2, %3}, [%4];" : "=f"(h.x), "=f"(h.y), "=f"(h.z), "=f"(h.w) : "r"(stg + r * PITCH + warp * 16));
-                kout[((long long)(r - n_out) * FRK) / 2 + warp] = h;
-            }
-        }
-        if (lane == 0) asm volatile("st.shared.v4.f32 [%0], {%1, %1, %1, %1};" ::"r"(stg + (FK - 1) * PITCH + warp * 16), "f"(0.f) : "memory");
-        __syncwarp();
-
-        pc acc[32];
-        {
-            pc v[32];
-            const uint32_t src = stg + tile_rd;
-#pragma unroll
-            for (int m = 0; m < 32; ++m) v[m] = f_lds(src + m * (16 * PITCH));
-            __syncwarp();
-            f_pass1_store(v, tw_row, stg + xch_wr);
-        }
-        {
-            const float4* gp = gtab + tid;
-            pc h[16];
-#pragma unroll
-            for (int jj = 0; jj < 8; ++jj) f_ldg2(gp + jj * T_THREADS, h[2 * jj], h[2 * jj + 1]);
-            __syncwarp();
-#pragma unroll
-            for (int which = 0; which < 2; ++which) {
-                pc x[16];
-#pragma unroll
-                for (int tr = 0; tr < 16; ++tr) x[tr] = f_lds(stg + xch_rd + (33 * tr + 16 * which) * PITCH);
-                pdft_regs<16, +1>(x);
-#pragma unroll
-                for (int k = 0; k < 16; ++k) acc[which * 16 + k] = pcmul(x[k], h[k]);
-                if (which == 0) {
-#pragma unroll
-                    for (int jj = 0; jj < 8; ++jj) f_ldg2(gp + (8 + jj) * T_THREADS, h[2 * jj], h[2 * jj + 1]);
-                }
-            }
-        }
-        PROF({ long long n_ = clock64(); tp[2] += n_ - tc; tc = n_; })
-        __syncwarp();
-#pragma unroll
-        for (int j = 0; j < 32; ++j) f_sts(stg + xch_rd + (16 * j) * PITCH, acc[j]);
-        sync_t();
-        if (parked == 0) gb_first = gb;
-        {
-            float2* ys = ysave + parked * YS_STRIDE;
-            for (int o = tid; o < FK; o += T_THREADS) {
-                const uint32_t src = stg + o * PITCH;
-                pc sum(0.f, 0.f);
-#pragma unroll
-                for (int w = 0; w < T_WARPS; ++w) {
-                    pc u0, u1;
-                    f_lds2(src + w * 16, u0, u1);
-                    sum = sum + u0;
-                    sum = sum + u1;
-                }
-                const int j = o >> 4, tt = o & 15;
-                ys[tt + 16 * (j >> 4) + 32 * (j & 15)] = make_float2(sum.x, sum.y);
-            }
-        }
-        ++parked;
-        PROF({ long long n_ = clock64(); tp[3] += n_ - tc; tc = n_; })
-
-        if (parked == NB || gb + 1 == n_blocks_total) {
-            sync_t();
-#pragma unroll 1
-            for (int j0 = 0; j0 < parked; j0 += FRK) {
-                if (j0 + 2 * warp >= parked) continue;
-                const int job = j0 + g;
-                const bool active = job < parked;
-                pc v[32];
-                const float2* ys = ysave + (active ? job : 0) * YS_STRIDE;
-#pragma unroll
-                for (int i1 = 0; i1 < 32; ++i1) {
-                    const float2 q = ys[t + 16 * i1];
-                    v[i1] = active ? pc(q.x, -q.y) : pc(0.f, 0.f);
-                }
-                f_pass1_store(v, tw_row, stg + xch_wr);
-                __syncwarp();
-                const int gj = gb_first + (active ? job : 0);
-                const int so_j = gj / B, b_j = gj - so_j * B;
-                const int s_j = (int)blockIdx.x + so_j * (int)gridDim.x;
-                float2* __restrict__ out = reinterpret_cast<float2*>(a.out) + (long long)s_j * a.out_stride;
-                float2* __restrict__ out2 = a.out2 ? reinterpret_cast<float2*>(a.out2) + (long long)s_j * a.out2_stride : nullptr;
-#pragma unroll
-                for (int which = 0; which < 2; ++which) {
-                    pc x[16];
-#pragma unroll
-                    for (int tr = 0; tr < 16; ++tr) x[tr] = f_lds(stg + xch_rd + (33 * tr + 16 * which) * PITCH);
-                    pdft_regs<16, +1>(x);
-                    if (active) {
-#pragma unroll
-                        for (int k2 = 0; k2 < 16; ++k2) {
-                            const int i = t + 16 * which + 32 * k2;
-                            if (i >= Lmax && i < Lmax + V) {
-                                const long long o = (long long)b_j * V + (i - Lmax);
-                                if (o < n_out) {
-                                    float2* dst = (out2 != nullptr && o >= a.out_split) ? out2 + (o - a.out_split) : out + o;
-                                    *dst = make_float2(x[k2].x, -x[k2].y);
-                                }
+    for (int g = 0; g < G + 2; ++g) {
+        int L = -1, slot = 0, pos0 = 0, j = 0, s = 0;
+        uint32_t ph = 0;
+        if (g < G) {
+            const int so = g / n_tiles;
+            s = (int)blockIdx.x + so * (int)gridDim.x;
+            j = g - so * n_tiles;
+            if (j < n_live) {
+                L = so * n_live + j;
+                slot = L % S;
+                ph = (uint32_t)((L / S) & 1);
+                pos0 = j * (TC_M * P) - J0;
+                if (j == 0) {
+                    if (L > 0) mb_wait(bar_accf + ((L - 1) & (TC_ACC - 1)) * 8, (uint32_t)(((L - 1) / TC_ACC) & 1));
+                    if (HAS_NCO) {
+                        const NcoStream ns = a.nco[s];
+                        const double inv_denom = 1.0 / (double)ns.denom;
+                        sync_e();
+                        for (int p = et; p < P; p += 32 * E_WARPS) {
+                            const pc c = f_rotation((uint32_t)p, ns.numer_abs, ns.denom, inv_denom, ns.sign);
+                            colph[p] = make_float2(c.x, c.y);
+                        }
+                        sync_e();
+                    }
+                    for (int e = et; e < P * FRK; e += 32 * E_WARPS) {
+                        const int p = e / FRK, c = e - p * FRK;
+                        const float ac = cf[(p >> 1) * (2 * FRK) + (p & 1) * FRK + c];
+                        float wr = ac, wi = 0.f;
+                        if (HAS_NCO) {
+                            const float2 cp = colph[p];
+                            wr = ac * cp.x;
+                            wi = ac * cp.y;
+                        }
+                        const int o = (p >> 1) * (TC_N * 16) + (2 * c) * 16 + (p & 1) * 8;
+                        const float v[4] = {wr, -wi, wi, wr};
+                        float h[4], l[4];
+#pragma unroll
+                        for (int q = 0; q < 4; ++q) {
+                            h[q] = tf32_rn(v[q]);
+                            l[q] = v[q] - h[q];
+                        }
+                        *reinterpret_cast<float2*>(p_b + o) = make_float2(h[0], h[1]);
+                        *reinterpret_cast<float2*>(p_b + o + 16) = make_float2(h[2], h[3]);
+                        *reinterpret_cast<float2*>(p_b + o + TC_NH * 16) = make_float2(l[0], l[1]);
+                        *reinterpret_cast<float2*>(p_b + o + TC_NH * 16 + 16) = make_float2(l[2], l[3]);
+                    }
+                }
+                mb_wait(bar_load + slot * 8, ph);
+                if (pos0 < 0) {
+                    unsigned char* const tile = p_slots + (size_t)slot * geo.slot_bytes;
+                    const float2* __restrict__ in = reinterpret_cast<const float2*>(a.in) + (long long)s * a.in_stride;
+                    const float2* __restrict__ hist_end = reinterpret_cast<const float2*>(a.hist2) + ((long long)s + 1) * hist_len;
+                    pc r0(1.f, 0.f);
+                    if (HAS_NCO) r0 = tc_rowph(pos0, a.nco[s]);
+                    for (int p = et; p < P; p += 32 * E_WARPS) {
+                        const int pos = pos0 + p;
+                        float2 q = make_float2(0.f, 0.f);
+                        if (pos >= 0) {
+                            if (pos < (int)a.len) q = __ldg(in + pos);
+                        } else if (pos >= -hist_len) {
+                            q = __ldg(hist_end + pos);
+                            if (HAS_NCO) {
+                                const float2 cph = colph[p];
+                                const pc y = pcmulc(pc(q.x, q.y), pcmul(r0, pc(cph.x, cph.y)));
+                                q = make_float2(y.x, y.y);
                             }
                         }
-                    }
-                }
+                        *reinterpret_cast<float2*>(tile + (p >> 1) * (TC_M * 16) + (p & 1) * 8) = q;
+                    }
+                }
+                asm volatile("fence.proxy.async.shared::cta;" ::: "memory");
                 __syncwarp();
-            }
-            parked = 0;
-            sync_t();
-        }
-        PROF({ long long n_ = clock64(); tp[4] += n_ - tc; tc = n_; })
-        __syncwarp();
-        if (lane == 0) {
-            uint32_t left;
-            asm volatile("atom.acq_rel.cta.shared::cta.add.u32 %0, [%1], 1;" : "=r"(left) : "r"(left_cnt + (uint32_t)(gb & 1) * 4) : "memory");
-            if (left % T_WARPS == T_WARPS - 1) {
-                int b2 = b + 2, so2 = so;
-                while (b2 >= B) {
-                    b2 -= B;
-                    ++so2;
-                }
-                if (b2 == 0 && so2 < n_my) copy_kept(so2, gb + 2);
-            }
-            mb_arrive(bar_empty + (uint32_t)(gb & 1) * 8);
-        }
-    }
-    PROF(if (tid == 0) for (int q = 0; q < 5; ++q) g_fused_prof[blockIdx.x * 16 + 9 + q] = tp[q];)
+                if (lane == 0) mb_arrive(bar_ready1 + slot * 8);
+            }
+        }
+
+        if (g >= 2) {
+            const int g2 = g - 2;
+            const int so2 = g2 / n_tiles, j2 = g2 - so2 * n_tiles;
+            const int s2 = (int)blockIdx.x + so2 * (int)gridDim.x;
+            if (j2 == 0) {
+                gb0 = so2 * B;
+                blk = 0;
+                off = 0;
+                if (HAS_NCO) {
+                    const NcoStream ns = a.nco[s2];
+                    const uint32_t r = mulmod_fast(ns.numer_abs, (uint32_t)(TC_M * P) % ns.denom, ns.denom, 1.0 / (double)ns.denom);
+                    double sn, cs;
+                    sincospi(2.0 * (double)r / (double)ns.denom, &sn, &cs);
+                    rot_tile = make_double2(cs, ns.sign < 0 ? -sn : sn);
+                }
+            }
+            const int r0 = j2 * TC_M;
+            const int row = r0 + er;
+            float u[2 * FRK];
+#pragma unroll
+            for (int c = 0; c < 2 * FRK; ++c) u[c] = 0.f;
+            if (j2 < n_live) {
+                const int L2 = so2 * n_live + j2, acc = L2 & (TC_ACC - 1);
+                mb_wait(bar_accf + acc * 8, (uint32_t)((L2 / TC_ACC) & 1));
+                tc_fence_after();
+                const uint32_t ta = tmem + ((uint32_t)(32 * sub) << 16) + acc * TC_ACC_COLS;
+                uint32_t r[20];
+                asm volatile(
+                    "tcgen05.ld.sync.aligned.32x32b.x16.b32 {%0, %1, %2, %3, %4, %5, %6, %7, %8, %9, %10, %11, %12, %13, %14, %15}, [%16];"
+                    : "=r"(r[0]), "=r"(r[1]), "=r"(r[2]), "=r"(r[3]), "=r"(r[4]), "=r"(r[5]), "=r"(r[6]), "=r"(r[7]), "=r"(r[8]), "=r"(r[9]), "=r"(r[10]),
+                      "=r"(r[11]), "=r"(r[12]), "=r"(r[13]), "=r"(r[14]), "=r"(r[15])
+                    : "r"(ta));
+                asm volatile("tcgen05.ld.sync.aligned.32x32b.x4.b32 {%0, %1, %2, %3}, [%4];"
+                             : "=r"(r[16]), "=r"(r[17]), "=r"(r[18]), "=r"(r[19])
+                             : "r"(ta + 16));
+                asm volatile("tcgen05.wait::ld.sync.aligned;" ::: "memory");
+#pragma unroll
+                for (int c = 0; c < 2 * FRK; ++c) u[c] = __uint_as_float(r[c]);
+                asm volatile(
+                    "tcgen05.ld.sync.aligned.32x32b.x16.b32 {%0, %1, %2, %3, %4, %5, %6, %7, %8, %9, %10, %11, %12, %13, %14, %15}, [%16];"
+                    : "=r"(r[0]), "=r"(r[1]), "=r"(r[2]), "=r"(r[3]), "=r"(r[4]), "=r"(r[5]), "=r"(r[6]), "=r"(r[7]), "=r"(r[8]), "=r"(r[9]), "=r"(r[10]),
+                      "=r"(r[11]), "=r"(r[12]), "=r"(r[13]), "=r"(r[14]), "=r"(r[15])
+                    : "r"(ta + TC_NH));
+                asm volatile("tcgen05.ld.sync.aligned.32x32b.x4.b32 {%0, %1, %2, %3}, [%4];"
+                             : "=r"(r[16]), "=r"(r[17]), "=r"(r[18]), "=r"(r[19])
+                             : "r"(ta + TC_NH + 16));
+                asm volatile("tcgen05.wait::ld.sync.aligned;" ::: "memory");
+                tc_fence_before();
+                __syncwarp();
+                if (lane == 0) mb_arrive(bar_acce + acc * 8);
+#pragma unroll
+                for (int c = 0; c < 2 * FRK; ++c) u[c] += __uint_as_float(r[c]);
+                if (HAS_NCO) {
+                    if ((j2 & 15) == 0) {
+                        rowph = tc_rowph((long long)r0 * P - J0 + (long long)er * P, a.nco[s2]);
+                        rowph_d = make_double2(rowph.x, rowph.y);
+                    } else {
+                        rowph_d = make_double2(rowph_d.x * rot_tile.x - rowph_d.y * rot_tile.y, rowph_d.x * rot_tile.y + rowph_d.y * rot_tile.x);
+                        rowph = pc((float)rowph_d.x, (float)rowph_d.y);
+                    }
+                }
+            }
+            {
+                const int last_off = min(off + TC_M, BV - blk * V) - 1;
+                const int gb_hi = gb0 + blk + (last_off >= V ? 1 : 0);
+                while (gb_acq < gb_hi) {
+                    ++gb_acq;
+                    mb_wait(bar_empty + (uint32_t)(gb_acq & 1) * 8, (uint32_t)(((gb_acq >> 1) & 1) ^ 1));
+                }
+            }
+            if (e_row && row < BV) {
+                int b = blk, o = off + er;
+                if (o >= V) {
+                    o -= V;
+                    ++b;
+                }
+                const uint32_t dst = s_u32(p_stage) + (uint32_t)((gb0 + b) & 1) * STAGE_BYTES + (Lmax + o) * PITCH;
+                const bool live = row < n_out;
+                const bool keep = live && row >= n_out - Lmax;
+                float4* __restrict__ keep_o = reinterpret_cast<float4*>(reinterpret_cast<float2*>(a.ukeep_out) + (long long)s2 * a.ukeep_out_stride);
+#pragma unroll
+                for (int c = 0; c < FRK; c += 2) {
+                    pc y0(u[2 * c], u[2 * c + 1]), y1(u[2 * c + 2], u[2 * c + 3]);
+                    if (HAS_NCO) {
+                        y0 = pcmul(y0, rowph);
+                        y1 = pcmul(y1, rowph);
+                    }
+                    if (!live) {
+                        y0 = pc(0.f, 0.f);
+                        y1 = pc(0.f, 0.f);
+                    }
+                    f_sts2(dst + c * 8, y0, y1);
+                    if (keep) keep_o[((row - (n_out - Lmax)) * FRK + c) / 2] = make_float4(y0.x, y0.y, y1.x, y1.y);
+                }
+            }
+            __syncwarp();
+            off += TC_M;
+            while (off >= V) {
+                off -= V;
+                ++blk;
+            }
+            arrive_upto((j2 + 1 < n_tiles) ? gb0 + min(blk, B) - 1 : gb0 + B - 1);
+        }
+
+        if (L >= 0) {
+            unsigned char* const tile = p_slots + (size_t)slot * geo.slot_bytes;
+            const int tr = et & (TC_M - 1);
+            const bool to_hist = a.hist_out != nullptr && (long long)pos0 + TC_M * P > hist_from && j * TC_M + tr < n_out;
+            float2* __restrict__ hist_o = reinterpret_cast<float2*>(a.hist_out) + (long long)s * a.hist_stride;
+            const long long prow = (long long)pos0 + (long long)tr * P;
+            pc rh(1.f, 0.f);
+            if (to_hist && HAS_NCO) rh = tc_rowph(prow, a.nco[s]);
+            mb_wait(bar_mma1 + slot * 8, ph);
+#pragma unroll 2
+            for (int ch = et >> 6; ch < geo.kc; ch += 2) {
+                float4* const q = reinterpret_cast<float4*>(tile + ch * (TC_M * 16) + tr * 16);
+                const float4 x = *q;
+                if (to_hist) {
+                    pc y0(x.x, x.y), y1(x.z, x.w);
+                    if (HAS_NCO) {
+                        const float4 cv = *reinterpret_cast<const float4*>(colph + 2 * ch);
+                        y0 = pcmul(pcmul(y0, pc(cv.x, cv.y)), rh);
+                        y1 = pcmul(pcmul(y1, pc(cv.z, cv.w)), rh);
+                    }
+                    const long long jh = prow + 2 * ch - hist_from;
+                    if (jh >= -1) {
+                        if (jh >= 0) hist_o[jh] = make_float2(y0.x, y0.y);
+                        hist_o[jh + 1] = make_float2(y1.x, y1.y);
+                    }
+                }
+                *q = make_float4(x.x - tf32_hi(x.x), x.y - tf32_hi(x.y), x.z - tf32_hi(x.z), x.w - tf32_hi(x.w));
+            }
+            asm volatile("fence.proxy.async.shared::cta;" ::: "memory");
+            __syncwarp();
+            if (lane == 0) mb_arrive(bar_ready2 + slot * 8);
+        }
+    }
+    tc_fence_before();
+    asm volatile("bar.arrive 2, %0;" ::"n"(32 + 32 * E_WARPS) : "memory");
 }
 
 namespace {
@@ -727,9 +1182,50 @@
     return cudaGetLastError();
 }
 
+constexpr int TC_NB = 5;
+size_t fused_tc_fixed_smem(int P, int Lmax) {
+    size_t b = (size_t)tc_geom(P).b_bytes + 2 * (size_t)STAGE_BYTES + TW_BYTES;
+    b += ((size_t)Lmax * PITCH + 127) / 128 * 128;
+    b += ((size_t)TC_NB * YS_STRIDE * 8 + 127) / 128 * 128;
+    b += ((size_t)P * 8 + 127) / 128 * 128;
+    b += TC_BAR_BYTES;
+    return b;
+}
+int fused_tc_slots(int P, int Lmax) {
+    const size_t fixed = fused_tc_fixed_smem(P, Lmax), cap = (size_t)227 * 1024;
+    if (fixed >= cap) return 0;
+    const int s = (int)std::min<size_t>(TC_MAX_SLOTS, (cap - fixed) / (size_t)tc_geom(P).slot_bytes);
+    return s >= 2 ? s : 0;
+}
+
+cudaError_t launch_tc(int n_streams, const FusedArgs& a, int sm_count, cudaStream_t st) {
+    EncodeFn enc = fused_encode_fn();
+    const TcGeom geo = tc_geom(a.P);
+    const int S = fused_tc_slots(a.P, a.Lmax);
+    const size_t smem = fused_tc_fixed_smem(a.P, a.Lmax) + (size_t)S * geo.slot_bytes;
+    CUtensorMap tm;
+    const cuuint64_t dims[4] = {(cuuint64_t)a.len, (cuuint64_t)TC_M, (cuuint64_t)geo.kc, (cuuint64_t)n_streams};
+    const cuuint64_t sstride = n_streams > 1 ? (cuuint64_t)a.in_stride * 8 : (((cuuint64_t)a.len * 8 + 15) / 16) * 16;
+    const cuuint64_t strides[3] = {(cuuint64_t)a.P * 8, 16, sstride};
+    const cuuint32_t box[4] = {2, (cuuint32_t)TC_M, (cuuint32_t)(2 * geo.ks), 1};
+    const cuuint32_t estr[4] = {1, 1, 1, 1};
+    const CUresult r = enc(&tm, CU_TENSOR_MAP_DATA_TYPE_UINT64, 4, const_cast<void*>(a.in), dims, strides, box, estr, CU_TENSOR_MAP_INTERLEAVE_NONE,
+                           CU_TENSOR_MAP_SWIZZLE_NONE, CU_TENSOR_MAP_L2_PROMOTION_L2_128B, CU_TENSOR_MAP_FLOAT_OOB_FILL_NONE);
+    if (r != CUDA_SUCCESS) return cudaErrorInvalidValue;
+    void (*kern)(const CUtensorMap, const FusedArgs, const int, const int) = a.nco ? k_fused_tc<TC_NB, true> : k_fused_tc<TC_NB, false>;
+    const cudaError_t e = cudaFuncSetAttribute(kern, cudaFuncAttributeMaxDynamicSharedMemorySize, (int)smem);
+    if (e != cudaSuccess) return e;
+    kern<<<std::min(n_streams, sm_count), TC_THREADS, smem, st>>>(tm, a, n_streams, S);
+    return cudaGetLastError();
+}
+
 }
 
 int fused_coef_slots() { return kFusedSlots; }
+
+bool fused_tc_selected(const FusedArgs& a) {
+    return a.front == FusedFront::Tensor && a.len >= (long long)(TC_M + 1) * a.P && fused_tc_slots(a.P, a.Lmax) > 0;
+}
 
 bool fused_supported(int rank_pad, long long P, int Lmax) {
     if (rank_pad != FRK || !(P == 50 || P == 40 || P == 20) || fused_encode_fn() == nullptr) return false;
@@ -751,6 +1247,7 @@
     FusedArgs a = a0;
     a.coef_off4 = a.coef_slot * (kFusedSlotFloats / 4);
     if ((uintptr_t)a.ukeep_in % 16 != 0 || (n_streams > 1 && a.ukeep_in_stride % 2 != 0)) return cudaErrorInvalidValue;
+    if (fused_tc_selected(a)) return launch_tc(n_streams, a, sm_count, st);
     const FusedGeom geo = fused_geom(a.P);
     CUtensorMap tm;
     const cuuint64_t dims[3] = {(cuuint64_t)a.len, (cuuint64_t)F_ROWS, (cuuint64_t)n_streams};
diff --git a/radiorust_b200/csrc/rr_kernels.h b/radiorust_b200/csrc/rr_kernels.h
--- a/radiorust_b200/csrc/rr_kernels.h
+++ b/radiorust_b200/csrc/rr_kernels.h
@@ -201,7 +201,9 @@
 bool front_wide_supported(int rank_pad, long long P);
 cudaError_t launch_front_wide(int rank_pad, int n_streams, const FrontArgs& a, cudaStream_t st);
 
+enum class FusedFront : int { Tensor = 0, Simt = 1 };
 struct FusedArgs {
+    FusedFront front;
     const void* in;
     long long in_stride;
     long long len;
@@ -231,6 +233,7 @@
 int fused_coef_slots();
 cudaError_t fused_upload_coef(int slot, const float* acoef, int P, cudaStream_t st);
 cudaError_t launch_fused(int n_streams, const FusedArgs& a, int sm_count, cudaStream_t st);
+bool fused_tc_selected(const FusedArgs& a);
 
 template <typename T>
 cudaError_t launch_hist2_update(const void* in, long long in_stride, long long len, const void* hist2_in, void* hist2_out,
```

Measured after the change: 185,300 (median of 6 runs). 65.0% lower.
